# robertknight/ocrs

Hardware: AMD Instinct MI355X
Metric: pages/sec end-to-end (1024x1024) (higher is better)
Workload: dtype f32

## Files before the change

ocrs_amd/csrc/common.cpp:

```cpp
#include "common.hpp"

#include <chrono>
#include <climits>
#include <cstdint>
#include <cstdlib>
#include <cstring>

#include <algorithm>
#include <atomic>
#include <condition_variable>
#include <deque>
#include <system_error>

namespace ocrs {

static thread_local std::string g_last_error;

void set_last_error(const std::string& msg) { g_last_error = msg; }
const std::string& last_error() { return g_last_error; }

namespace {
std::atomic<int> g_default_device{0};
thread_local DeviceContext* t_ctx = nullptr;
constexpr int kMaxDevices = 64;
// ... 240 lines not shown
            cached_ -= got;
            live_[p] = got;
            live_bytes_ += got;
            peak_live_ = std::max(peak_live_, live_bytes_);
            return p;
        }
    }
    void* p = nullptr;
    OCRS_HIP(hipHostMalloc(&p, sz, hipHostMallocPortable));
    std::lock_guard<std::mutex> g(mu_);
    live_[p] = sz;
    live_bytes_ += sz;
    peak_live_ = std::max(peak_live_, live_bytes_);
    allocs_++;
    return p;
}

void HostPool::release(void* p) {
    if (!p) return;
    std::vector<void*> drop;
    {
        std::lock_guard<std::mutex> g(mu_);
        auto it = live_.find(p);
        if (it == live_.end()) return;
        free_.emplace(it->second, p);
        cached_ += it->second;
        live_bytes_ -= it->second;
        live_.erase(it);
        while (cached_ > cap_ && !free_.empty()) {
            auto big = std::prev(free_.end());
            drop.push_back(big->second);
            cached_ -= big->first;
            free_.erase(big);
        }
    }
    for (void* q : drop) trimmer().give(-1, q, &frees_);
}

void HostPool::set_cap(uint64_t bytes) {
    std::lock_guard<std::mutex> g(mu_);
    cap_ = bytes;
}

PoolStats HostPool::stats() {
    std::lock_guard<std::mutex> g(mu_);
    PoolStats st;
    st.live = live_bytes_; st.cached = cached_; st.cap = cap_; st.peak_live = peak_live_; st.driver_allocs = allocs_; st.driver_frees = frees_;
    return st;
}

hipStream_t DeviceContext::heavy_stream() {
    std::lock_guard<std::mutex> g(lazy_mu_);
    if (!heavy_) {
        DeviceScope bind(device);
        int least = 0, greatest = 0;
        OCRS_HIP(hipDeviceGetStreamPriorityRange(&least, &greatest));
        OCRS_HIP(hipStreamCreateWithPriority(&heavy_, hipStreamNonBlocking, greatest));
    }
    return heavy_;
}

hipStream_t DeviceContext::recurrent_stream(int mode) {
    if (mode == MODE_SERIAL) return heavy_stream();
    std::lock_guard<std::mutex> g(lazy_mu_);
    if (!recurrent_) {
        DeviceScope bind(device);
        int least = 0, greatest = 0;
        OCRS_HIP(hipDeviceGetStreamPriorityRange(&least, &greatest));
        OCRS_HIP(hipStreamCreateWithPriority(&recurrent_, hipStreamNonBlocking, greatest));
    }
    return recurrent_;
}

static thread_local int t_lease_depth[kMaxDevices] = {0};

template <class F> void DeviceContext::switch_isolation(F&& change) {
    if (t_lease_depth[device] > 0) fail(OCRS_ERR_INVALID_ARGUMENT, "the isolation regime of device %d cannot change from inside one of its requests", device);
    std::unique_lock<std::mutex> lk(iso_mu_);
    iso_cv_.wait(lk, [&] { return !switching_; });
    const Mode before = mode_locked();
    switching_ = true;
    struct Done { DeviceContext* c; ~Done() { c->switching_ = false; c->iso_cv_.notify_all(); } } done{this};
    const Isolation p0 = policy_;
    const int r0 = relaxed_;
    change();
    if (mode_locked() == before) return;
    const Isolation p1 = policy_;
    const int r1 = relaxed_;
    policy_ = p0; relaxed_ = r0;
    iso_cv_.wait(lk, [&] { return leases_ == 0; });
    {
        DeviceScope bind(device);
        if (hipDeviceSynchronize() != hipSuccess) (void)hipGetLastError();
    }
    policy_ = p1; relaxed_ = r1;
}

DeviceContext::Mode DeviceContext::lease_begin() {
    std::unique_lock<std::mutex> lk(iso_mu_);
    if (t_lease_depth[device] == 0) iso_cv_.wait(lk, [&] { return !switching_; });
    t_lease_depth[device]++;
    leases_++;
    return mode_locked();
}

void DeviceContext::lease_end() {
    std::lock_guard<std::mutex> lk(iso_mu_);
    t_lease_depth[device]--;
    if (--leases_ == 0) iso_cv_.notify_all();
}

void DeviceContext::add_relaxed_engine(int delta) {
    switch_isolation([&] { relaxed_ += delta; });
}

void DeviceContext::set_isolation(Isolation policy) {
    switch_isolation([&] { policy_ = policy; });
}

DeviceContext::Mode DeviceContext::current_mode() {
    std::lock_guard<std::mutex> lk(iso_mu_);
    return mode_locked();
}

int DeviceContext::relaxed_engine_count() {
    std::lock_guard<std::mutex> lk(iso_mu_);
    return relaxed_;
}

int DeviceContext::cu_count() {
    std::lock_guard<std::mutex> g(lazy_mu_);
    if (!cus_) {
        hipDeviceProp_t prop;
        OCRS_HIP(hipGetDeviceProperties(&prop, device));
        cus_ = prop.multiProcessorCount;
    }
    return cus_;
}

namespace {
struct OptDef { const char* name; const char* env; long def; };
const OptDef kOptDefs[OPT_COUNT] = {
    {"gru_mode", "OCRS_GRU_MODE", GRU_PERSISTENT},
    {"gru_gates", "OCRS_GRU_GATES", 1},
    {"gru_local", "OCRS_GRU_LOCAL", 1},
    {"det_fuse", "OCRS_DET_FUSE", 1},
    {"det_stream", "OCRS_DET_STREAM", 1},
    {"det_rows", "OCRS_DET_ROWS", 1},
    {"ccl_quad", "OCRS_CCL_QUAD", 1},
    {"conv12_fuse", "OCRS_CONV12_FUSE", 1},
    {"conv_flat", "OCRS_CONV_FLAT", 1},
    {"beam_gpu", "OCRS_BEAM_GPU", 1},
    {"det_tile_batch", "OCRS_DET_TILE_BATCH", 16},
    {"numerics", nullptr, 0},
    {"coalesce", nullptr, 2},
    {"coalesce_pages", nullptr, 16},
    {"coalesce_window_us", nullptr, 300},
    {"layout_threads", nullptr, 0},
    {"rec_max_pixels", nullptr, 0},
};
struct OptRange { long lo, hi; long also[4]; };
const OptRange kOptRanges[OPT_COUNT] = {
    {0, 1, {}}, {0, 1, {}}, {0, 1, {}}, {0, 2, {}}, {0, 1, {8, 14, 32}}, {0, 1, {8, 14, 20, 32}}, {0, 1, {}}, {0, 1, {}}, {0, 1, {}}, {0, 1, {}},
    {1, 1024, {}},
    {0, 2, {}}, {0, 64, {}}, {1, 4096, {}}, {0, 10000000, {}}, {0, 4096, {}}, {0, INT64_MAX, {}},
};
bool in_range(int i, long v) {
    const OptRange& r = kOptRanges[i];
    if (v >= r.lo && v <= r.hi) return true;
    for (long a : r.also) if (a && v == a) return true;
    return false;
}
const char* const kRetired[] = {"det_heavy", "det_tail", "gru_waves", "gru_background", "gru_scatter", "gru_gates_pack", "conv_occupancy",
                                "gx_heavy", "gemm_nfast", "conv_a_lds", "gru_heavy", "heavy_priority", "det_mfma"};
std::atomic<long> g_opts[OPT_COUNT];
std::once_flag g_opts_once;
void init_options() {
    for (int i = 0; i < OPT_COUNT; i++) {
        const char* e = kOptDefs[i].env ? getenv(kOptDefs[i].env) : nullptr;
        const long v = e && *e ? strtol(e, nullptr, 10) : kOptDefs[i].def;
        g_opts[i].store(in_range(i, v) ? v : kOptDefs[i].def);
    }
}
int find_option(const char* name, int count = OPT_PUBLIC_COUNT) {
    for (int i = 0; i < count; i++)
        if (name && i != OPT_NUMERICS && strcmp(name, kOptDefs[i].name) == 0) return i;
    return -1;
}
thread_local const Tuning* t_tuning = nullptr;
}

TuningScope::TuningScope(const Tuning* t) : prev_(t_tuning) { t_tuning = t; }
TuningScope::~TuningScope() { t_tuning = prev_; }
const Tuning* current_tuning() { return t_tuning; }

long option_long(Option o) {
    if (t_tuning) return __atomic_load_n(&t_tuning->v[o], __ATOMIC_RELAXED);
    std::call_once(g_opts_once, init_options);
    return g_opts[o].load(std::memory_order_relaxed);
}
int option(Option o) { return (int)option_long(o); }

Tuning default_tuning() {
    std::call_once(g_opts_once, init_options);
    Tuning t;
    for (int i = 0; i < OPT_COUNT; i++) t.v[i] = g_opts[i].load(std::memory_order_relaxed);
    return t;
}

const char* option_name(int i) { return i >= 0 && i < OPT_PUBLIC_COUNT ? kOptDefs[i].name : nullptr; }

int set_option(const char* name, long value) {
    std::call_once(g_opts_once, init_options);
    const int i = find_option(name);
    if (i < 0) {
        for (const char* r : kRetired) if (name && strcmp(name, r) == 0) return 0;
        return 1;
    }
    if (!in_range(i, value)) return 2;
    g_opts[i].store(value);
    return 0;
}

int set_option(Tuning& t, const char* name, long value) {
    const int i = find_option(name, OPT_COUNT);
    if (i < 0) return 1;
    if (!in_range(i, value)) return 2;
    __atomic_store_n(&t.v[i], value, __ATOMIC_RELAXED);
    return 0;
}

bool get_option(const Tuning& t, const char* name, long* value) {
    const int i = name && strcmp(name, "numerics") == 0 ? (int)OPT_NUMERICS : find_option(name, OPT_COUNT);
    if (i < 0) return false;
    *value = __atomic_load_n(&t.v[i], __ATOMIC_RELAXED);
    return true;
}

StreamLease::StreamLease(bool high_priority) : ctx_(&ctx()), high_(high_priority) {
    high_ = true;
    mode_ = ctx_->lease_begin();
    try {
        if (mode_ == DeviceContext::MODE_SERIAL) {
            s_ = ctx_->heavy_stream();
            shared_ = true;
            OCRS_HIP(hipEventCreateWithFlags(&done_, hipEventBlockingSync | hipEventDisableTiming));
            return;
        }
        {
            std::lock_guard<std::mutex> g(ctx_->stream_mu);
            auto& v = ctx_->streams;
            if (!v.empty()) {
                s_ = v.back().first;
                done_ = v.back().second;
                v.pop_back();
                return;
            }
        }
        int least = 0, greatest = 0;
        OCRS_HIP(hipDeviceGetStreamPriorityRange(&least, &greatest));
        OCRS_HIP(hipStreamCreateWithPriority(&s_, hipStreamNonBlocking, greatest));
        OCRS_HIP(hipEventCreateWithFlags(&done_, hipEventBlockingSync | hipEventDisableTiming));
    } catch (...) {
        ctx_->lease_end();
        throw;
    }
}

StreamLease::~StreamLease() {
    if (shared_) {
        (void)hipEventDestroy(done_);
    } else {
        std::lock_guard<std::mutex> g(ctx_->stream_mu);
        ctx_->streams.emplace_back(s_, done_);
    }
    ctx_->lease_end();
}

std::vector<StageTimers::Pending>& StageTimers::pending() {
    static thread_local std::vector<Pending> p;
    return p;
}
std::map<int, std::vector<hipEvent_t>>& StageTimers::thread_events() {
    static thread_local std::map<int, std::vector<hipEvent_t>> f;
    return f;
}
std::vector<hipEvent_t>& StageTimers::free_events() { return thread_events()[ctx().device]; }

hipEvent_t StageTimers::get_event() {
    auto& fe = free_events();
    if (!fe.empty()) {
        hipEvent_t e = fe.back();
        fe.pop_back();
        return e;
    }
    hipEvent_t e;
    OCRS_HIP(hipEventCreate(&e));
    return e;
}

int StageTimers::begin(int stage, hipStream_t s, uint64_t n_launches) {
    if (!enabled) return -1;
    Pending p{stage, get_event(), get_event(), n_launches, false, 0.0, 0.0, 0.0};
    OCRS_HIP(hipEventRecord(p.a, s));
    pending().push_back(p);
    return (int)pending().size() - 1;
}

int StageTimers::kbegin(int cls, hipStream_t s, double flops, double bytes, double mfma_flops) {
    if (!enabled || !kernels_enabled || !((kernel_mask >> cls) & 1u)) return -1;
    if (mfma_flops < 0.0) mfma_flops = cls <= KC_GEMM_LINEAR ? flops : 0.0;
    Pending p{cls, get_event(), get_event(), 1, true, flops, bytes, mfma_flops};
    OCRS_HIP(hipEventRecord(p.a, s));
    pending().push_back(p);
    return (int)pending().size() - 1;
}

// ... 43 lines not shown
```

ocrs_amd/csrc/common.hpp:

```cpp
#pragma once
#include <atomic>
#include <hip/hip_runtime.h>

#include <cstdarg>
#include <cstdint>
#include <cstdio>
#include <cstdlib>
#include <chrono>
#include <condition_variable>
#include <cstring>
#include <map>
#include <mutex>
#include <stdexcept>
#include <string>
#include <thread>
#include <vector>

#include "../../include/ocrs_amd.h"

namespace ocrs {

struct Error : std::runtime_error {
    ocrs_status status;
    Error(ocrs_status s, const std::string& msg) : std::runtime_error(msg), status(s) {}
};

[[noreturn]] inline void fail(ocrs_status s, const char* fmt, ...) {
    char buf[512];
    va_list ap;
    va_start(ap, fmt);
    vsnprintf(buf, sizeof buf, fmt, ap);
    va_end(ap);
    throw Error(s, buf);
}

#define OCRS_HIP(expr)                                                                              \
    do {                                                                                            \
        hipError_t _e = (expr);                                                                     \
        if (_e != hipSuccess)                                                                       \
            ::ocrs::fail(OCRS_ERR_DEVICE, "HIP error %s at %s:%d (%s)", hipGetErrorString(_e), __FILE__, \
                         __LINE__, #expr);                                                          \
    } while (0)

void set_last_error(const std::string& msg);


struct PoolStats { uint64_t live = 0, cached = 0, cap = 0, peak_live = 0, driver_allocs = 0, driver_frees = 0; };
class DevicePool {
  public:
    explicit DevicePool(int device) : device_(device) {}
    ~DevicePool();
    void* alloc(size_t bytes);
    void release(void* p);
    void trim();
    void set_cap(uint64_t bytes);
    PoolStats stats();
    int device() const { return device_; }

  private:
    uint64_t cap_locked();
    const int device_;
    std::mutex mu_;
    std::multimap<size_t, void*> free_;
    std::map<void*, size_t> live_;
    uint64_t cached_ = 0, live_bytes_ = 0, peak_live_ = 0, cap_ = 0, allocs_ = 0;
    std::atomic<uint64_t> frees_{0};
};

class HostPool {
  public:
    void* alloc(size_t bytes);
    void release(void* p);
    void set_cap(uint64_t bytes);
    PoolStats stats();

  private:
    std::mutex mu_;
    std::multimap<size_t, void*> free_;
    std::map<void*, size_t> live_;
    uint64_t cached_ = 0, live_bytes_ = 0, peak_live_ = 0, cap_ = uint64_t(1) << 30, allocs_ = 0;
    std::atomic<uint64_t> frees_{0};
};

struct DeviceContext {
    const int device;
    DevicePool pool;
    HostPool host_pool;
    std::mutex heavy_phase, rec_phase;
    hipStream_t heavy_stream();
    hipStream_t recurrent_stream(int mode = 0);
    enum Isolation { ISO_AUTO = 0, ISO_NONE = 1 };
    enum Mode { MODE_FREE = 0, MODE_SERIAL = 1 };
    Mode lease_begin();
    void lease_end();
    void add_relaxed_engine(int delta);
    void set_isolation(Isolation policy);
    Mode current_mode();
    int relaxed_engine_count();
    int cu_count();
    std::vector<struct DevBuf> heavy_arena;
    std::mutex stream_mu;
    std::vector<std::pair<hipStream_t, hipEvent_t>> streams;

    explicit DeviceContext(int d) : device(d), pool(d) {}

  private:
    Mode mode_locked() const { return policy_ == ISO_NONE || relaxed_ <= 0 ? MODE_FREE : MODE_SERIAL; }
    template <class F> void switch_isolation(F&& change);
    std::mutex lazy_mu_;
    hipStream_t heavy_ = nullptr, recurrent_ = nullptr;
    int cus_ = 0;
    std::mutex iso_mu_;
    std::condition_variable iso_cv_;
    int leases_ = 0, relaxed_ = 0;
    bool switching_ = false;
    Isolation policy_ = ISO_AUTO;
    friend class StreamLease;
};

DeviceContext& device_context(int device);
int default_device();
void select_device(int device);
DeviceContext& ctx();

class DeviceScope {
  public:
    explicit DeviceScope(int device);
    ~DeviceScope();
    DeviceScope(const DeviceScope&) = delete;
    DeviceScope& operator=(const DeviceScope&) = delete;

  private:
    DeviceContext* prev_;
    int restore_ = -1;
};

inline DevicePool& pool() { return ctx().pool; }
inline HostPool& host_pool() { return ctx().host_pool; }
inline hipStream_t heavy_stream() { return ctx().heavy_stream(); }

enum Option { OPT_GRU_MODE = 0, OPT_GRU_GATES, OPT_GRU_LOCAL, OPT_DET_FUSE, OPT_DET_STREAM, OPT_DET_ROWS, OPT_CCL_QUAD,
              OPT_CONV12_FUSE, OPT_CONV_FLAT, OPT_BEAM_GPU, OPT_DET_TILE_BATCH, OPT_PUBLIC_COUNT,
              OPT_NUMERICS = OPT_PUBLIC_COUNT,
              OPT_COALESCE, OPT_COALESCE_PAGES, OPT_COALESCE_WINDOW_US,
              OPT_LAYOUT_THREADS, OPT_REC_MAX_PIXELS,
              OPT_COUNT };
struct Tuning { long v[OPT_COUNT]; };
Tuning default_tuning();
int set_option(const char* name, long value);
int set_option(Tuning& t, const char* name, long value);
bool get_option(const Tuning& t, const char* name, long* value);
const char* option_name(int i);
class TuningScope {
  public:
    explicit TuningScope(const Tuning* t);
    ~TuningScope();
    TuningScope(const TuningScope&) = delete;
    TuningScope& operator=(const TuningScope&) = delete;
  private:
    const Tuning* prev_;
};
const Tuning* current_tuning();
enum { GRU_PERSISTENT = 0, GRU_STEP = 1 };
int option(Option o);

inline void allow_dynamic_lds(const void* kernel, std::atomic<uint64_t>& done) {
    int dev = 0;
    (void)hipGetDevice(&dev);
    const uint64_t bit = 1ull << (dev & 63);
    if (done.load(std::memory_order_relaxed) & bit) return;
    (void)hipFuncSetAttribute(kernel, hipFuncAttributeMaxDynamicSharedMemorySize, 160 * 1024);
    done.fetch_or(bit, std::memory_order_relaxed);
}
long option_long(Option o);
inline int gru_mode() { return option(OPT_GRU_MODE); }

struct DevBuf {
    void* p = nullptr;
    size_t bytes = 0;
    DevicePool* owner = nullptr;
    DevBuf() = default;
    explicit DevBuf(size_t n) : bytes(n), owner(n ? &pool() : nullptr) { p = n ? owner->alloc(n) : nullptr; }
    DevBuf(const DevBuf&) = delete;
    DevBuf& operator=(const DevBuf&) = delete;
    DevBuf(DevBuf&& o) noexcept : p(o.p), bytes(o.bytes), owner(o.owner) { o.p = nullptr; o.bytes = 0; o.owner = nullptr; }
    DevBuf& operator=(DevBuf&& o) noexcept {
        if (this != &o) { reset(); p = o.p; bytes = o.bytes; owner = o.owner; o.p = nullptr; o.bytes = 0; o.owner = nullptr; }
        return *this;
    }
    ~DevBuf() { reset(); }
    void reset() { if (p && owner) owner->release(p); p = nullptr; bytes = 0; owner = nullptr; }
    int device() const { return owner ? owner->device() : -1; }
    template <class T> T* as() const { return static_cast<T*>(p); }
};

struct PinnedBuf {
    void* p = nullptr;
    size_t bytes = 0;
    PinnedBuf() = default;
    explicit PinnedBuf(size_t n) : bytes(n) { if (n) OCRS_HIP(hipHostMalloc(&p, n, hipHostMallocPortable)); }
    PinnedBuf(const PinnedBuf&) = delete;
    PinnedBuf& operator=(const PinnedBuf&) = delete;
    ~PinnedBuf() { if (p) (void)hipHostFree(p); }
    template <class T> T* as() const { return static_cast<T*>(p); }
};

class StreamLease {
  public:
    explicit StreamLease(bool high_priority = false);
    ~StreamLease();
    hipStream_t get() const { return s_; }
    hipError_t wait_done() const noexcept {
        hipError_t e = hipEventRecord(done_, s_);
        if (e != hipSuccess) return e;
        for (int i = 0;; i++) {
            e = hipEventQuery(done_);
            if (e != hipErrorNotReady) return e;
            if (i < 64) std::this_thread::yield();
            else std::this_thread::sleep_for(std::chrono::microseconds(i < 256 ? 20 : 100));
        }
    }
    void sync() const { OCRS_HIP(wait_done()); }
    hipError_t sync_noexcept() const noexcept { return wait_done(); }
    DeviceContext::Mode mode() const { return mode_; }
    bool serial() const { return mode_ == DeviceContext::MODE_SERIAL; }
    hipStream_t conv_stream() const { return ctx_->heavy_stream(); }
    hipStream_t recurrent_stream() const { return ctx_->recurrent_stream((int)mode_); }

  private:
    DeviceContext* ctx_;
    DeviceContext::Mode mode_ = DeviceContext::MODE_FREE;
    bool shared_ = false;
    hipStream_t s_;
    hipEvent_t done_;
    bool high_;
};

enum Stage {
    ST_PREPARE = 0,
    ST_RESIZE_IN,
    ST_DET_CNN,
    ST_RESIZE_THRESH,
    ST_CCL,
    ST_CONTOUR_RECTS,
    ST_LINE_CROP,
    ST_REC_CONV,
    ST_REC_GRU,
    ST_REC_HEAD,
    ST_CTC,
    ST_COUNT
};
extern const char* const kStageNames[ST_COUNT];

enum KernelClass {
    KC_GEMM_CONV3X3 = 0, KC_GEMM_POINTWISE, KC_GEMM_CONVT, KC_GEMM_GRU_INPUT, KC_GEMM_GRU_HIDDEN, KC_GEMM_LINEAR,
    KC_DWCONV3X3, KC_CONV_DIRECT, KC_POOL, KC_PADCAT, KC_CONV1X1_SIGMOID, KC_GRU_GATES, KC_LOGSOFTMAX_ARGMAX,
    KC_OTHER, KC_DET_BLOCK, KC_DET_STREAM_WAVE, KC_DET_STREAM_ROWS, KC_COUNT
};
extern const char* const kKernelClassNames[KC_COUNT];

struct StageTimers {
    bool enabled = false;
    bool kernels_enabled = false;
    uint32_t kernel_mask = 0xffffffffu;
    std::mutex mu;
    double ms[ST_COUNT] = {0};
    uint64_t launches[ST_COUNT] = {0};
    double kms[KC_COUNT] = {0};
    uint64_t klaunches[KC_COUNT] = {0};
    double kflops[KC_COUNT] = {0};
    double kbytes[KC_COUNT] = {0};
    double kmfma[KC_COUNT] = {0};
    struct Pending { int stage; hipEvent_t a, b; uint64_t n; bool kernel; double flops, bytes, mfma; };
    static std::vector<Pending>& pending();
    int begin(int stage, hipStream_t s, uint64_t n_launches);
    int kbegin(int cls, hipStream_t s, double flops, double bytes, double mfma_flops = -1.0);
    void end(int token, hipStream_t s);
    void collect();
    void reset();
    static void release_thread_events();
  private:
    static std::vector<hipEvent_t>& free_events();
    static std::map<int, std::vector<hipEvent_t>>& thread_events();
    hipEvent_t get_event();
};

inline int ceil_div(int64_t a, int64_t b) { return (int)((a + b - 1) / b); }

struct StageScope {
    StageTimers* t; int token; hipStream_t s;
    StageScope(StageTimers* timers, int stage, hipStream_t stream, uint64_t n_launches = 1)
        : t(timers), token(timers ? timers->begin(stage, stream, n_launches) : -1), s(stream) {}
    ~StageScope() { if (t && token >= 0) t->end(token, s); }
};

struct Workspace {
    StreamLease stream;
    HostPool& hpool = host_pool();
    std::vector<DevBuf> bufs;
    std::vector<hipEvent_t> events;
    hipEvent_t make_event() {
        hipEvent_t e;
        OCRS_HIP(hipEventCreateWithFlags(&e, hipEventDisableTiming));
        events.push_back(e);
        return e;
    }
    Workspace() = default;
    explicit Workspace(bool high_priority) : stream(high_priority) {}
    std::vector<void*> upload_staging;
    void upload(void* d_dst, const void* h_src, size_t bytes) {
        if (!bytes) return;
        void* pin = hpool.alloc(bytes);
        memcpy(pin, h_src, bytes);
        upload_staging.push_back(pin);
        OCRS_HIP(hipMemcpyAsync(d_dst, pin, bytes, hipMemcpyHostToDevice, stream.get()));
    }
// ... 41 lines not shown
```

ocrs_amd/csrc/kernels.hpp:

```cpp
#pragma once
#include <vector>
#include <hip/hip_runtime.h>

#include <cstdint>

namespace ocrs {
namespace jpeg { struct Coefficients; }
namespace k {

void prepare_image(const void* d_pixels, bool is_u8, bool chans_last, int h, int w, int chans, float* d_out,
                   hipStream_t s);
void resize_pages_to_model(const float* const* d_src_ptrs, int n, int sh, int sw, int vh, int vw, float* d_dst,
                           int dh, int dw, hipStream_t s);
bool resize_threshold(const float* d_prob, int n, int mh, int mw, int sh, int sw, float thr, uint8_t* d_mask,
                      float* d_map, int h, int w, hipStream_t s, int32_t* d_labels = nullptr, int32_t* d_zero_a = nullptr,
                      int32_t* d_zero_b = nullptr);
void threshold_only(const float* d_prob, float thr, uint8_t* d_mask, int64_t count, hipStream_t s);

struct CclBuffers {
    int32_t* labels;
    int32_t* row_counts;
    int32_t* row_offsets;
    int32_t* n_roots;
    int32_t* roots;
    int32_t* lengths;
    int32_t* offsets;
    int32_t* overflow;
    uint32_t* pts;
    uint32_t* tmp;
    uint8_t* keep;
    float* rects;
    uint8_t* valid;
    uint32_t* score_pixels;
    unsigned long long* score_sums;
};
void ccl_label(const uint8_t* d_mask, int n, int h, int w, const CclBuffers& b, int max_comp, hipStream_t s, bool prepared = false);
void contour_rects(const uint8_t* d_mask, int n, int h, int w, const CclBuffers& b, int max_comp, int64_t arena,
                   float expand, float min_area, float eps, hipStream_t s, bool prepared = false);

void component_scores(const uint8_t* d_mask, const float* d_map, int n, int h, int w, const CclBuffers& b, int max_comp,
                      hipStream_t s);

struct TileDesc {
    const float* page;
    uint8_t* mask;
    float* map;
    int32_t h, w;
    int32_t oy, ox;
    int32_t y0, y1, x0, x1;
};
void gather_tiles(const TileDesc* d_tiles, int n_tiles, float* d_dst, int mh, int mw, hipStream_t s);
void stitch_threshold(const TileDesc* d_tiles, int n_tiles, const float* d_prob, int mh, int mw, float thr, hipStream_t s);

struct GemmDesc {
    const float* A; int lda;
    const float* B; int ldb;
    const float* bias;
    float* C; int ldc;
    int M, N, K;
    int relu;
    int im2col; int H, W, Cin;
    int convt; int Cout;
    int batch; int64_t strideA, strideB, strideBias, strideC;
    int nfast = 0, nx = 0, ny = 0;
    const uint16_t* Bsplit = nullptr; int64_t strideBsplit = 0;
};
void gemm(const GemmDesc& d, hipStream_t s);
void conv_direct(const float* x, int n, int h, int w, int cin, const float* wt, const float* bias, int kh, int kw,
                 int cout, int relu, float* y, hipStream_t s);
void dwconv3x3(const float* x, int n, int h, int w, int c, const float* wt, const float* bias, int relu, float* y,
               hipStream_t s);
bool dwpw_fused_supported(int cin, int cout);
void dwpw_fused(const float* x, int n, int h, int w, int cin, const float* wdw, const float* bdw, int relu_dw, int cout,
                const float* wpw, const float* bpw, int relu_pw, float* y, hipStream_t s);
bool dwconv3x3_cat(const float* skip, int n, int h, int w, int cs, const float* up, int uh, int uw, int cu, const float* wt,
                   const float* bias, int relu, float* y, hipStream_t s);
struct DoubleConvArgs {
    const float* skip;
    const float* x1;
    const float *wt, *bt;
    const float *wd1, *bd1;
    const float *wp1, *bp1;
    const float *wd2, *bd2;
    const float *wp2, *bp2;
    const float *wf, *bf;
    float* y;
    float* ypool;
    int n, h, w, h1, w1;
    int relu_d1, relu_p1, relu_d2, relu_p2, sigmoid;
    int tiles_x, tiles_y;
    const float* tape = nullptr;
    int tape_len = 0;
    const float* rtape = nullptr;
    int rtape_len = 0;
};
struct StreamWeights {
    const float *wt, *bt, *wd1, *bd1, *wp1, *bp1, *wd2, *bd2, *wp2, *bp2, *wf, *bf;
};
bool double_conv_fused(const DoubleConvArgs& a, int cs, int cx, int cmid, int cout, bool pool, bool final_conv,
                       bool launch, hipStream_t s, bool* on_mfma = nullptr, int* path = nullptr);
bool double_conv_stream(const DoubleConvArgs& a, int cs, int cx, int cmid, int cout, bool pool, bool final_conv, bool launch, hipStream_t s,
                        const StreamWeights* hw = nullptr, std::vector<float>* tape_out = nullptr, int* tape_len = nullptr);
bool double_conv_rows(const DoubleConvArgs& a, int cs, int cx, int cmid, int cout, bool pool, bool final_conv, bool launch, hipStream_t s,
                      const StreamWeights* hw = nullptr, std::vector<float>* tape_out = nullptr, int* tape_len = nullptr);
bool double_conv_rows_takes(const DoubleConvArgs& a, int cx);
void maxpool(const float* x, int n, int h, int w, int c, int kh, int kw, float* y, hipStream_t s);
void avgpool(const float* x, int n, int h, int w, int c, int kh, int kw, float* y, hipStream_t s);
void padcat(const float* skip, int n, int sh, int sw, int cs, const float* x, int h, int w, int cx, float* y,
            hipStream_t s);
void sigmoid(const float* x, float* y, int64_t count, hipStream_t s);
void conv1x1_cout1(const float* x, int64_t pixels, int cin, const float* wt, const float* bias, int relu, int do_sigmoid,
                   float* y, hipStream_t s);
void to_seq(const float* x, int n, int w, int c, float* y, hipStream_t s);
void gru_gates(const float* gx, const float* gh, float* h, float* y, int T, int N, int H, int step, hipStream_t s);
bool log_softmax_argmax(const float* logits, int64_t rows, int c, const uint8_t* d_excluded ,
                        float* logp, int32_t* labels, hipStream_t s, float* maxlp = nullptr);
void to_seq_packed(const float* x, int n, int T, int c, const int32_t* d_pos, const int32_t* d_off, float* y,
                   hipStream_t s);
void gru_gates_packed(const float* gx, const float* gh, float* h, float* y, const int32_t* d_Tm, const int32_t* d_off,
                      int64_t R, int Mcap, int active, int H, int step, hipStream_t s);
bool gru_step_fused(const float* gx, const float* wh, const float* bh, const float* hT_in, float* hT_out, float* y,
                    const int32_t* d_Tm, const int32_t* d_off, int64_t R, int Mcap, int active, int H, int step,
                    hipStream_t s);
size_t gru_persistent_sync_words(int M);
size_t gru_persistent_exchange_bytes(const int32_t* h_Tm, int M, int H);
bool gru_persistent_supported(const int32_t* h_Tm, int M, int Tmax, int64_t R, int H);
bool gru_tile_plan(const int32_t* h_Tm, int M, int H, int* ncl, int* waves, int16_t* tiles );
hipError_t gru_persistent_prepare(float* hx, const int32_t* h_Tm, int M, int H, hipStream_t s);
bool gru_persistent(const float* gx, const float* wh, const float* bh, float* y, float* hx, const int32_t* d_Tm, const int32_t* d_off,
                    const int32_t* h_Tm, int64_t R, int M, int Tmax, int H, uint32_t* d_sync, hipStream_t s);
bool gru_general_tile_plan(const int32_t* h_Tm, int M, int Tmax, int H, int cap, int* ncl, int16_t* tiles , int kernel );
size_t gru_split_exchange_bytes(const int32_t* h_Tm, int M, int H, int np);
bool gru_split_supported(const int32_t* h_Tm, int M, int Tmax, int64_t R, int H, int np);
hipError_t gru_split_prepare(uint16_t* hx, const int32_t* h_Tm, int M, int H, int np, hipStream_t s);
bool gru_persistent_split(const float* gx, const float* wh, const float* bh, float* y, uint16_t* hx, const int32_t* d_Tm, const int32_t* d_off,
                          const int32_t* h_Tm, int64_t R, int M, int Tmax, int H, int np, uint32_t* d_sync, hipStream_t s);
void ctc_collapse_packed(const int32_t* labels, const int32_t* d_Tm, const int32_t* d_off, int M, int Tmax,
                         uint32_t* out_labels, uint32_t* out_pos, int32_t* out_count, hipStream_t s);
void ctc_collapse_scored_packed(const int32_t* labels, const float* maxlp, const int32_t* d_Tm, const int32_t* d_off, int M,
                                int Tmax, uint32_t* out_labels, uint32_t* out_pos, float* out_logp, int32_t* out_count,
                                double* out_score, hipStream_t s);
void argmax_rows(const float* x, int64_t rows, int c, const uint8_t* d_excluded, int32_t* labels, hipStream_t s);
bool ctc_beam_supported(int C, int width);
size_t ctc_beam_arena_entries(int Tmax, int width);
bool ctc_beam_packed(const float* logp, const int32_t* d_Tm, const int32_t* d_off, int M, int Tmax, int C, int width,
                     const uint8_t* d_excluded, int2* d_nodes, int2* d_posn, uint32_t* out_labels, uint32_t* out_pos,
                     int32_t* out_count, hipStream_t s, double* out_score = nullptr, float* out_logp = nullptr);
void ctc_collapse(const int32_t* labels, int T, int N, uint32_t* out_labels, uint32_t* out_pos, int32_t* out_count,
                  hipStream_t s);

struct RaggedView {
    int G;
    int H;
    const int32_t* W;
    const int32_t* n;
    const int64_t* poff;
    const int32_t* toff128;
    const int32_t* toff256;
    const int32_t* loff;
    int ntiles128, ntiles256;
    const int32_t* toff2d;
    int ntiles2d, tw;
    const int32_t* toff2d_flat;
    const int32_t* toff2d_flat2;
    int ntiles2d_flat, ntiles2d_flat2;
    const int32_t* toff2d_gap;
    int ntiles2d_gap;
    int64_t max_tile_px_;
    int min_w;
    int64_t pixels;
    int max_w;
};
void conv1_relu_pool_ragged(const float* x, const RaggedView& in, const float* wt, const float* bias, int cout,
                            float* y, const RaggedView& out, hipStream_t s);
void pool_ragged(const float* x, const RaggedView& in, int c, int kh, int kw, bool avg, float* y, const RaggedView& out,
                 hipStream_t s);
void to_seq_packed_ragged(const float* x, const RaggedView& in, int c, const int32_t* d_pos, const int32_t* d_off,
                          float* y, hipStream_t s);
void avgpool_to_seq_ragged(const float* x, const RaggedView& in, const RaggedView& seq, int c, const int32_t* d_pos,
                           const int32_t* d_off, float* y, hipStream_t s);
bool conv12_fused_ragged(const float* x, const RaggedView& in0, const RaggedView& mid, const float* w1, const float* b1,
                         int c1, const float* w2, const float* b2, int c2, float* y, const RaggedView& out, hipStream_t s,
                         const uint16_t* w2split = nullptr);
void conv12_split_weights(const float* w2_host , std::vector<uint16_t>* out);
bool conv3x3_ragged(const float* x, const RaggedView& rv, int cin, const float* wt, const float* bias, int cout, int relu,
                    int ph, int pw, float* y, const RaggedView& out, hipStream_t s, const uint16_t* wsplit = nullptr);
void split_weights(const float* w_host, int K, int N, int ldw, std::vector<uint16_t>* out);

struct LineDesc {
    int32_t page;
    int32_t poly_off;
    int32_t poly_n;
    int32_t top, left, bh, bw;
    int32_t resized_w;
    int32_t out_w;
    int64_t out_off;
};
void crop_lines(const float* const* d_pages, const int32_t* d_page_hw , const LineDesc* d_lines,
                const int32_t* d_poly , int n_lines, int out_h, float* d_out, hipStream_t s);

struct RectLineDesc {
    int32_t page;
    int32_t mode;
    int32_t range_off;
    int32_t range_n;
    int32_t resized_w;
    int32_t out_w;
    int64_t out_off;
    float x0, ax, bx, y0, ay, by;
};
void rectify_lines(const float* const* d_pages, const int32_t* d_page_hw , const RectLineDesc* d_lines,
                   const int32_t* d_ranges, int n_lines, int max_out_w, int out_h, float* d_out, hipStream_t s);

void measure_peaks(double* mfma_tflops, double* copy_gbps);


size_t jpeg_sample_bytes(const jpeg::Coefficients& c);
void jpeg_decode(const jpeg::Coefficients& c, const uint64_t* d_mask, const uint32_t* d_offset, const int16_t* d_values,
                 const uint16_t* d_quant, uint8_t* d_samples, uint8_t* d_rgb, hipStream_t s);

}
}
```

ocrs_amd/csrc/kernels_lines.hip:

```cpp
#include "kernels.hpp"

namespace ocrs {
namespace k {

constexpr int MAX_LDS_EDGES = 512;

__device__ __forceinline__ void resize_axis(int o, int in_len, int out_len, int& i0, int& i1, float& wgt) {
    float scale = (float)in_len / (float)out_len;
    float c = ((float)o + 0.5f) * scale - 0.5f;
    float hi = (float)(in_len - 1);
    c = c < 0.0f ? 0.0f : c;
    c = c > hi ? hi : c;
    int a = (int)c;
    i0 = a;
    i1 = a + 1 < in_len ? a + 1 : in_len - 1;
    wgt = c - (float)a;
}

__device__ __forceinline__ int edge_x_at(int xa, int ya, int xb, int yb, int y) {
    float t = (float)(y - ya) * ((float)(xb - xa) / (float)(yb - ya));
    return xa + (int)roundf(t);
}

__global__ void __launch_bounds__(256)
crop_lines_kernel(const float* const* __restrict__ pages, const int32_t* __restrict__ page_hw,
                  const LineDesc* __restrict__ lines, const int32_t* __restrict__ poly, int out_h,
                  float* __restrict__ batch) {
    __shared__ int xs[2][MAX_LDS_EDGES];
    __shared__ int cnt[2];
    const LineDesc ln = lines[blockIdx.y];
    const int oy = blockIdx.x;
    const int out_w = ln.out_w;
    float* __restrict__ dst = batch + ln.out_off + (int64_t)oy * out_w;
    const float fill = -0.5f;
    if (ln.bh <= 0 || ln.bw <= 0) {
        for (int ox = threadIdx.x; ox < out_w; ox += blockDim.x) dst[ox] = fill;
        return;
    }
    const float* __restrict__ page = pages[ln.page];
    const int ph = page_hw[2 * ln.page], pw = page_hw[2 * ln.page + 1];
    int r0, r1;
    float wy;
    resize_axis(oy, ln.bh, out_h, r0, r1, wy);
    if (threadIdx.x < 2) cnt[threadIdx.x] = 0;
    __syncthreads();
    const int32_t* pv = poly + 2 * (int64_t)ln.poly_off;
    for (int i = threadIdx.x; i < 2 * ln.poly_n; i += blockDim.x) {
        const int which = i / ln.poly_n, e = i - which * ln.poly_n;
        const int y = ln.top + (which ? r1 : r0);
        int ya = pv[2 * e], xa = pv[2 * e + 1];
        const int e2 = e + 1 == ln.poly_n ? 0 : e + 1;
        int yb = pv[2 * e2], xb = pv[2 * e2 + 1];
        if (ya == yb) continue;
        if (ya > yb) { int t = ya; ya = yb; yb = t; t = xa; xa = xb; xb = t; }
        if (y < ya || y >= yb) continue;
        int slot = atomicAdd(&cnt[which], 1);
        if (slot < MAX_LDS_EDGES) xs[which][slot] = edge_x_at(xa, ya, xb, yb, y);
    }
    __syncthreads();
    const int m0 = cnt[0], m1 = cnt[1];
    auto crossings_direct = [&](int which, int x) {
        const int y = ln.top + (which ? r1 : r0);
        int c = 0;
        for (int e = 0; e < ln.poly_n; e++) {
            int ya = pv[2 * e], xa = pv[2 * e + 1];
            const int e2 = e + 1 == ln.poly_n ? 0 : e + 1;
            int yb = pv[2 * e2], xb = pv[2 * e2 + 1];
            if (ya == yb) continue;
            if (ya > yb) { int t = ya; ya = yb; yb = t; t = xa; xa = xb; xb = t; }
            if (y < ya || y >= yb) continue;
            c += edge_x_at(xa, ya, xb, yb, y) <= x ? 1 : 0;
        }
        return c;
    };
    for (int ox = threadIdx.x; ox < out_w; ox += blockDim.x) {
        float v = fill;
        if (ox < ln.resized_w) {
            int c0, c1;
            float wx;
            resize_axis(ox, ln.bw, ln.resized_w, c0, c1, wx);
            float tap[4];
#pragma unroll
            for (int q = 0; q < 4; q++) {
                const int which = q >> 1;
                const int r = which ? r1 : r0;
                const int c = (q & 1) ? c1 : c0;
                const int y = ln.top + r, x = ln.left + c;
                const int m = which ? m1 : m0;
                int crossings = 0;
                if (m <= MAX_LDS_EDGES)
                    for (int kk = 0; kk < m; kk++) crossings += xs[which][kk] <= x ? 1 : 0;
                else
                    crossings = crossings_direct(which, x);
                float t = fill;
                if ((crossings & 1) && y >= 0 && y <= ph - 1 && x >= 0 && x <= pw - 1 && r <= ph - 1 && c <= pw - 1)
                    t = page[(int64_t)y * pw + x];
                tap[q] = t;
            }
            float top = (1.0f - wx) * tap[0] + wx * tap[1];
            float bot = (1.0f - wx) * tap[2] + wx * tap[3];
            v = (1.0f - wy) * top + wy * bot;
        }
        dst[ox] = v;
    }
}

void crop_lines(const float* const* d_pages, const int32_t* d_page_hw, const LineDesc* d_lines, const int32_t* d_poly,
                int n_lines, int out_h, float* d_out, hipStream_t s) {
    if (n_lines <= 0) return;
    hipLaunchKernelGGL(crop_lines_kernel, dim3(out_h, n_lines), dim3(256), 0, s, d_pages, d_page_hw, d_lines, d_poly,
                       out_h, d_out);
}

}
}
```

ocrs_amd/csrc/kernels_nn.hip:

```cpp
#include "common.hpp"
#include "kernels.hpp"
#include "split_mfma.hpp"
#include "spec_math.hpp"

namespace ocrs {
namespace k {

typedef float f32x16 __attribute__((ext_vector_type(16)));

constexpr int GEMM_BK = 32;

template <int NT, bool IM2COL, bool CONVT>
__global__ void __launch_bounds__(256) gemm_mfma_kernel(GemmDesc d) {
    extern __shared__ __attribute__((aligned(16))) float lds_b[];
    constexpr int BN = 32 * NT;
    const int tid = threadIdx.x;
    const int lane = tid & 63;
    const int wave = tid >> 6;
    const int half = lane >> 5;
    const int l31 = lane & 31;
    const int z = blockIdx.z;
    const float* __restrict__ A = d.A + (int64_t)z * d.strideA;
    const float* __restrict__ B = d.B + (int64_t)z * d.strideB;
    const float* __restrict__ bias = d.bias ? d.bias + (int64_t)z * d.strideBias : nullptr;
    float* __restrict__ C = d.C + (int64_t)z * d.strideC;

    const int n0 = blockIdx.y * BN;
    const int64_t row = (int64_t)blockIdx.x * 128 + wave * 32 + l31;
    const bool row_ok = row < d.M;
    const int64_t rowc = row_ok ? row : (int64_t)d.M - 1;

    int py = 0, px = 0;
    int64_t img_base = 0;
    if (IM2COL) {
        int64_t hw = (int64_t)d.H * d.W;
        int64_t img = rowc / hw;
        int rem = (int)(rowc - img * hw);
        py = rem / d.W;
        px = rem - py * d.W;
        img_base = img * hw * d.Cin;
    }

    f32x16 acc[NT];
#pragma unroll
    for (int t = 0; t < NT; t++) {
        int col = n0 + t * 32 + l31;
        float bv = (bias && col < d.N) ? bias[col] : 0.0f;
#pragma unroll
        for (int r = 0; r < 16; r++) acc[t][r] = bv;
    }

    for (int k0 = 0; k0 < d.K; k0 += GEMM_BK) {
        const int kc = min(GEMM_BK, d.K - k0);
        __syncthreads();
        for (int i = tid; i < GEMM_BK * BN / 4; i += 256) {
            int kk = (i * 4) / BN;
            int nn = (i * 4) % BN;
            float4 v = make_float4(0.f, 0.f, 0.f, 0.f);
            if (kk < kc) {
                const float* src = B + (int64_t)(k0 + kk) * d.ldb + n0 + nn;
                if (n0 + nn + 3 < d.N && ((d.ldb & 3) == 0) && (((uintptr_t)B & 15) == 0)) {
                    v = *reinterpret_cast<const float4*>(src);
                } else {
                    if (n0 + nn + 0 < d.N) v.x = src[0];
                    if (n0 + nn + 1 < d.N) v.y = src[1];
                    if (n0 + nn + 2 < d.N) v.z = src[2];
                    if (n0 + nn + 3 < d.N) v.w = src[3];
                }
            }
            *reinterpret_cast<float4*>(&lds_b[kk * BN + nn]) = v;
        }
        __syncthreads();

        const float* arow;
        bool a_ok = true;
        if (IM2COL) {
            int tap = k0 / d.Cin;
            int ci0 = k0 - tap * d.Cin;
            int ky = tap / 3, kx = tap - ky * 3;
            int iy = py + ky - 1, ix = px + kx - 1;
            a_ok = (unsigned)iy < (unsigned)d.H && (unsigned)ix < (unsigned)d.W;
            arow = A + img_base + ((int64_t)(a_ok ? iy : 0) * d.W + (a_ok ? ix : 0)) * d.Cin + ci0;
        } else {
            arow = A + rowc * d.lda + k0;
        }

        for (int kk = 0; kk < kc; kk += 4) {
            float4 av = make_float4(0.f, 0.f, 0.f, 0.f);
            if (a_ok) {
                if (kk + 4 <= kc) {
                    av = *reinterpret_cast<const float4*>(arow + kk);
                } else {
                    av.x = arow[kk];
                    if (kk + 1 < kc) av.y = arow[kk + 1];
                    if (kk + 2 < kc) av.z = arow[kk + 2];
                }
            }
            const float a0 = half ? av.y : av.x;
            const float a1 = half ? av.w : av.z;
            const float* b0p = &lds_b[(kk + half) * BN + l31];
            const float* b1p = &lds_b[(kk + 2 + half) * BN + l31];
#pragma unroll
            for (int t = 0; t < NT; t++)
                acc[t] = __builtin_amdgcn_mfma_f32_32x32x2f32(a0, b0p[t * 32], acc[t], 0, 0, 0);
#pragma unroll
            for (int t = 0; t < NT; t++)
                acc[t] = __builtin_amdgcn_mfma_f32_32x32x2f32(a1, b1p[t * 32], acc[t], 0, 0, 0);
        }
    }

    const int64_t row_base = (int64_t)blockIdx.x * 128 + wave * 32;
#pragma unroll
    for (int t = 0; t < NT; t++) {
        const int col = n0 + t * 32 + l31;
        if (col >= d.N) continue;
#pragma unroll
        for (int r = 0; r < 16; r++) {
            const int64_t rr = row_base + (r & 3) + 8 * (r >> 2) + 4 * half;
            if (rr >= d.M) continue;
            float v = acc[t][r];
            if (d.relu) v = v > 0.0f ? v : 0.0f;
            if (CONVT) {
                int64_t hw = (int64_t)d.H * d.W;
                int64_t img = rr / hw;
                int rem = (int)(rr - img * hw);
                int y = rem / d.W, x = rem - y * d.W;
                int q = col / d.Cout, co = col - q * d.Cout;
                int dy = q >> 1, dx = q & 1;
                C[((img * 2 * d.H + 2 * y + dy) * (2 * (int64_t)d.W) + 2 * x + dx) * d.Cout + co] = v;
            } else {
                C[rr * d.ldc + col] = v;
            }
        }
    }
}

constexpr int TG_BM = 128, TG_BK = 16, TG_LDA = TG_BM + 1;

typedef float f32x4v __attribute__((ext_vector_type(4)));

template <int NTW, class Acc>
__device__ __forceinline__ void store_tile_rows(const Acc (&acc)[2][NTW], float* stage, int lane, bool relu, float* __restrict__ C,
                                                int64_t row0, int64_t M, int ldc) {
    constexpr int WN = 32 * NTW, LPR = WN / 4, RPI = 64 / LPR;
    const int half = lane >> 5, l31 = lane & 31;
    const int srow = lane / LPR, sc4 = (lane % LPR) * 4;
#pragma unroll
    for (int i = 0; i < 2; i++) {
#pragma unroll
        for (int t = 0; t < NTW; t++)
#pragma unroll
            for (int r = 0; r < 16; r++) {
                float v = acc[i][t][r];
                if (relu) v = v > 0.0f ? v : 0.0f;
                stage[((r & 3) + 8 * (r >> 2) + 4 * half) * WN + t * 32 + l31] = v;
            }
        asm volatile("s_waitcnt lgkmcnt(0)" ::: "memory");
#pragma unroll
        for (int it = 0; it < 32 / RPI; it++) {
            const int row = it * RPI + srow;
            const f32x4v v = *reinterpret_cast<const f32x4v*>(&stage[row * WN + sc4]);
            const int64_t rr = row0 + i * 32 + row;
            if (rr < M) *reinterpret_cast<f32x4v*>(&C[rr * ldc + sc4]) = v;
        }
        asm volatile("s_waitcnt lgkmcnt(0)" ::: "memory");
    }
}

template <int BN, bool IM2COL, bool PAIR>
__global__ void __launch_bounds__(256, 4) gemm_tiled_kernel(GemmDesc d) {
    extern __shared__ __attribute__((aligned(16))) float lds[];
    constexpr int NTW = BN / 64;
    float* As = lds;
    float* Bs = lds + 2 * TG_BK * TG_LDA;
    const int tid = threadIdx.x, lane = tid & 63, wave = tid >> 6;
    const int half = lane >> 5, l31 = lane & 31;
    const int wm = wave >> 1, wn = wave & 1;
    const int z = blockIdx.z;
    const float* __restrict__ A = d.A + (int64_t)z * d.strideA;
    const float* __restrict__ B = d.B + (int64_t)z * d.strideB;
    const float* __restrict__ bias = d.bias ? d.bias + (int64_t)z * d.strideBias : nullptr;
    float* __restrict__ C = d.C + (int64_t)z * d.strideC;
    int mblk, nblk;
    if (d.nfast) {
        const int xcd = blockIdx.x & 7, q = blockIdx.x >> 3;
        nblk = q % d.ny;
        mblk = (q / d.ny) * 8 + xcd;
        if (mblk >= d.nx) return;
    } else {
        const int nwg = gridDim.x, xcd = blockIdx.x & 7, xq = nwg >> 3, xr = nwg & 7;
        mblk = (xcd < xr ? xcd * (xq + 1) : xr * (xq + 1) + (xcd - xr) * xq) + (blockIdx.x >> 3);
        nblk = blockIdx.y;
    }
    const int64_t m0 = (int64_t)mblk * TG_BM;
    const int n0 = nblk * BN;

    constexpr int AQ = TG_BK / 4, AROWS = 256 / AQ, AV = TG_BM / AROWS;
    const int ar = tid / AQ, akq = tid % AQ;
    const float* arow_ptr[AV];
    int apy[AV], apx[AV];
#pragma unroll
    for (int j = 0; j < AV; j++) {
        int64_t row = m0 + ar + AROWS * j;
        if (row >= d.M) row = d.M - 1;
        if (IM2COL) {
            const int64_t hw = (int64_t)d.H * d.W;
            const int64_t img = row / hw;
            const int rem = (int)(row - img * hw);
            apy[j] = rem / d.W;
            apx[j] = rem - apy[j] * d.W;
            arow_ptr[j] = A + img * hw * d.Cin;
        } else {
            apy[j] = apx[j] = 0;
            arow_ptr[j] = A + row * d.lda;
        }
    }
    constexpr int BV = TG_BK * BN / 4 / 256;
    const bool b_vec = ((d.ldb & 3) == 0) && (((uintptr_t)B & 15) == 0);

    int boff[BV];
#pragma unroll
    for (int j = 0; j < BV; j++) {
        const int idx = tid + 256 * j;
        const int kk = idx / (BN / 4), nn = (idx % (BN / 4)) * 4;
        boff[j] = kk * d.ldb + min(n0 + nn, d.N - 4);
    }
    f32x4v pa[AV], pa2[AV], pb[BV];
    auto prefetch_b_fast = [&](int k0) {
        const float* __restrict__ bk = B + (int64_t)k0 * d.ldb;
#pragma unroll
        for (int j = 0; j < BV; j++) pb[j] = *reinterpret_cast<const f32x4v*>(bk + boff[j]);
    };
    auto prefetch_a_pair = [&](int k0) {
#pragma unroll
        for (int j = 0; j < AV; j++) {
            const float* src = arow_ptr[j] + k0 + akq * 4;
            pa[j] = *reinterpret_cast<const f32x4v*>(src);
            pa2[j] = *reinterpret_cast<const f32x4v*>(src + TG_BK);
        }
    };
    auto prefetch = [&](int k0) {
        if (IM2COL) {
            const int tap = k0 / d.Cin;
            const int ci0 = k0 - tap * d.Cin;
            const int ky = tap / 3, kx = tap - ky * 3;
#pragma unroll
            for (int j = 0; j < AV; j++) {
                const int iy = apy[j] + ky - 1, ix = apx[j] + kx - 1;
                const bool ok = (unsigned)iy < (unsigned)d.H && (unsigned)ix < (unsigned)d.W;
                pa[j] = ok ? *reinterpret_cast<const f32x4v*>(arow_ptr[j] + ((int64_t)iy * d.W + ix) * d.Cin + ci0 + akq * 4)
                           : f32x4v{0.f, 0.f, 0.f, 0.f};
            }
        } else {
#pragma unroll
            for (int j = 0; j < AV; j++) pa[j] = *reinterpret_cast<const f32x4v*>(arow_ptr[j] + k0 + akq * 4);
        }
#pragma unroll
        for (int j = 0; j < BV; j++) {
            const int idx = tid + 256 * j;
            const int kk = idx / (BN / 4), nn = (idx % (BN / 4)) * 4;
            const float* src = B + (int64_t)(k0 + kk) * d.ldb + n0 + nn;
            f32x4v v = {0.f, 0.f, 0.f, 0.f};
            if (b_vec && n0 + nn + 3 < d.N) {
                v = *reinterpret_cast<const f32x4v*>(src);
            } else {
                if (n0 + nn + 0 < d.N) v.x = src[0];
                if (n0 + nn + 1 < d.N) v.y = src[1];
                if (n0 + nn + 2 < d.N) v.z = src[2];
                if (n0 + nn + 3 < d.N) v.w = src[3];
            }
            pb[j] = v;
        }
    };
    auto commit_from = [&](int buf, const f32x4v (&src)[AV]) {
        float* a = As + buf * TG_BK * TG_LDA;
#pragma unroll
        for (int j = 0; j < AV; j++) {
            const int r = ar + AROWS * j;
            a[(akq * 4 + 0) * TG_LDA + r] = src[j].x;
            a[(akq * 4 + 1) * TG_LDA + r] = src[j].y;
            a[(akq * 4 + 2) * TG_LDA + r] = src[j].z;
            a[(akq * 4 + 3) * TG_LDA + r] = src[j].w;
        }
        float* b = Bs + buf * TG_BK * BN;
#pragma unroll
        for (int j = 0; j < BV; j++) {
            const int idx = tid + 256 * j;
            const int kk = idx / (BN / 4), nn = (idx % (BN / 4)) * 4;
            *reinterpret_cast<f32x4v*>(&b[kk * BN + nn]) = pb[j];
        }
    };
    auto commit = [&](int buf) { commit_from(buf, pa); };

    f32x16 acc[2][NTW];
#pragma unroll
    for (int t = 0; t < NTW; t++) {
        const int col = n0 + wn * (BN / 2) + t * 32 + l31;
        const float bv = (bias && col < d.N) ? bias[col] : 0.0f;
#pragma unroll
        for (int r = 0; r < 16; r++) { acc[0][t][r] = bv; acc[1][t][r] = bv; }
    }

    const int nchunks = d.K / TG_BK;
    auto compute = [&](int buf) {
        const float* a = As + buf * TG_BK * TG_LDA + wm * 64 + l31;
        const float* b = Bs + buf * TG_BK * BN + wn * (BN / 2) + l31;
#pragma unroll
        for (int kp = 0; kp < TG_BK / 2; kp++) {
            const int kr = 2 * kp + half;
            const float a0 = a[kr * TG_LDA], a1 = a[kr * TG_LDA + 32];
#pragma unroll
            for (int t = 0; t < NTW; t++) {
                const float bt = b[kr * BN + t * 32];
                acc[0][t] = __builtin_amdgcn_mfma_f32_32x32x2f32(a0, bt, acc[0][t], 0, 0, 0);
                acc[1][t] = __builtin_amdgcn_mfma_f32_32x32x2f32(a1, bt, acc[1][t], 0, 0, 0);
            }
        }
    };
    if (PAIR) {
        prefetch_a_pair(0);
        prefetch_b_fast(0);
        commit_from(0, pa);
        __syncthreads();
        for (int c = 0; c < nchunks; c += 2) {
            prefetch_b_fast((c + 1) * TG_BK);
            compute(0);
            commit_from(1, pa2);
            __syncthreads();
            const bool more = c + 2 < nchunks;
            if (more) {
                prefetch_a_pair((c + 2) * TG_BK);
                prefetch_b_fast((c + 2) * TG_BK);
            }
            compute(1);
            if (more) commit_from(0, pa);
            __syncthreads();
        }
    } else {
        prefetch(0);
        commit(0);
        __syncthreads();
        for (int c = 0; c < nchunks; c++) {
            const int buf = c & 1;
            if (c + 1 < nchunks) prefetch((c + 1) * TG_BK);
            compute(buf);
            if (c + 1 < nchunks) commit(buf ^ 1);
            __syncthreads();
        }
    }

    if (n0 + BN <= d.N && (d.ldc & 3) == 0 && (((uintptr_t)C) & 15) == 0) {
        static_assert(4 * 32 * (BN / 2) <= 2 * TG_BK * TG_LDA + 2 * TG_BK * BN, "staging must fit the operand tiles");
        store_tile_rows<NTW>(acc, lds + wave * (32 * (BN / 2)), lane, d.relu != 0, C + n0 + wn * (BN / 2), m0 + wm * 64, d.M, d.ldc);
        return;
    }
#pragma unroll
    for (int i = 0; i < 2; i++)
#pragma unroll
        for (int t = 0; t < NTW; t++) {
            const int col = n0 + wn * (BN / 2) + t * 32 + l31;
            if (col >= d.N) continue;
#pragma unroll
            for (int r = 0; r < 16; r++) {
                const int64_t rr = m0 + wm * 64 + i * 32 + (r & 3) + 8 * (r >> 2) + 4 * half;
                if (rr >= d.M) continue;
                float v = acc[i][t][r];
                if (d.relu) v = v > 0.0f ? v : 0.0f;
                C[rr * d.ldc + col] = v;
            }
        }
}

template <int BN>
static void launch_gemm_tiled(const GemmDesc& d, hipStream_t s) {
    dim3 grid((unsigned)((d.M + TG_BM - 1) / TG_BM), (unsigned)((d.N + BN - 1) / BN), (unsigned)(d.batch > 0 ? d.batch : 1));
    size_t lds = (size_t)(2 * TG_BK * TG_LDA + 2 * TG_BK * BN) * sizeof(float);
    const bool pair = !d.im2col && (d.K % (2 * TG_BK)) == 0 && (d.ldb & 3) == 0 && (((uintptr_t)d.B) & 15) == 0 &&
                      (d.strideB & 3) == 0 && (d.N & 3) == 0 && d.N >= 4;
    if (d.im2col) hipLaunchKernelGGL((gemm_tiled_kernel<BN, true, false>), grid, dim3(256), lds, s, d);
    else if (pair && grid.y > 1) {
        GemmDesc e = d;
        e.nfast = 1; e.nx = (int)grid.x; e.ny = (int)grid.y;
        const dim3 g1((unsigned)((grid.x + 7) / 8 * 8 * grid.y), 1, grid.z);
        hipLaunchKernelGGL((gemm_tiled_kernel<BN, false, true>), g1, dim3(256), lds, s, e);
    } else if (pair) hipLaunchKernelGGL((gemm_tiled_kernel<BN, false, true>), grid, dim3(256), lds, s, d);
    else hipLaunchKernelGGL((gemm_tiled_kernel<BN, false, false>), grid, dim3(256), lds, s, d);
}

template <int NP>
__global__ void __launch_bounds__(256, NP == 3 ? 2 : 3) gemm_split_kernel(GemmDesc d) {
    extern __shared__ __attribute__((aligned(16))) float lds[];
    constexpr int PL = split::PLANE;
    float* As = lds;
    float* Bs = lds + 2 * NP * PL;
    const int tid = threadIdx.x, lane = tid & 63, wave = tid >> 6;
    const int half = lane >> 5, l31 = lane & 31;
    const int wm = wave >> 1, wn = wave & 1;
    const int z = blockIdx.z;
    const float* __restrict__ A = d.A + (int64_t)z * d.strideA;
    const float* __restrict__ bias = d.bias ? d.bias + (int64_t)z * d.strideBias : nullptr;
    float* __restrict__ C = d.C + (int64_t)z * d.strideC;
    const int xcd = blockIdx.x & 7, q = blockIdx.x >> 3;
    const int nblk = q % d.ny;
    const int mblk = (q / d.ny) * 8 + xcd;
    if (mblk >= d.nx) return;
    const int64_t m0 = (int64_t)mblk * split::BM;
    const int n0 = nblk * split::BN;
    const int nchunks = d.K / split::BK;
    const float* __restrict__ img = reinterpret_cast<const float*>(d.Bsplit + (int64_t)z * d.strideBsplit) +
                                    (int64_t)nblk * nchunks * split::image_floats;
    const int ar = tid >> 2, akq = tid & 3;
    const float* arow[2];
#pragma unroll
    for (int j = 0; j < 2; j++) {
        int64_t row = m0 + ar + 64 * j;
        if (row >= d.M) row = d.M - 1;
        arow[j] = A + row * d.lda + akq * 4;
    }
    split::f32x16s acc[2][2];
#pragma unroll
    for (int t = 0; t < 2; t++) {
        const int col = n0 + wn * 64 + t * 32 + l31;
        const float bv = bias ? bias[col] : 0.0f;
#pragma unroll
        for (int r = 0; r < 16; r++) { acc[0][t][r] = bv; acc[1][t][r] = bv; }
    }
    split::pipeline<NP>(nchunks,
        [&](int k0, split::f32x4s (&d0)[2], split::f32x4s (&d1)[2]) {
#pragma unroll
            for (int j = 0; j < 2; j++) {
                d0[j] = *reinterpret_cast<const split::f32x4s*>(arow[j] + k0);
                d1[j] = *reinterpret_cast<const split::f32x4s*>(arow[j] + k0 + split::BK);
            }
        },
        [&](int k0, int ring) { split::load_weights<NP>(img + (int64_t)(k0 / split::BK) * split::image_floats, Bs + ring * NP * PL, wave, lane); },
        [&](int abuf, const split::f32x4s (&v)[2]) {
            char* base = reinterpret_cast<char*>(As + abuf * NP * PL);
#pragma unroll
            for (int j = 0; j < 2; j++) split::commit4<NP>(base, ar + 64 * j, akq, v[j][0], v[j][1], v[j][2], v[j][3]);
        },
        [&](int abuf, int ring) {
            split::mma_chunk<NP>(reinterpret_cast<const char*>(As + abuf * NP * PL), reinterpret_cast<const char*>(Bs + ring * NP * PL),
                                 wm, wn, l31, half, acc);
        });
    if ((d.ldc & 3) == 0 && (((uintptr_t)C) & 15) == 0) {
        store_tile_rows<2>(acc, lds + wave * (32 * 64), lane, d.relu != 0, C + n0 + wn * 64, m0 + wm * 64, d.M, d.ldc);
        return;
    }
#pragma unroll
    for (int i = 0; i < 2; i++)
#pragma unroll
        for (int t = 0; t < 2; t++) {
            const int col = n0 + wn * 64 + t * 32 + l31;
#pragma unroll
            for (int r = 0; r < 16; r++) {
                const int64_t rr = m0 + wm * 64 + i * 32 + (r & 3) + 8 * (r >> 2) + 4 * half;
                if (rr >= d.M) continue;
                float v = acc[i][t][r];
                if (d.relu) v = v > 0.0f ? v : 0.0f;
                C[rr * d.ldc + col] = v;
            }
        }
}

static bool launch_gemm_split(const GemmDesc& d, int numerics, hipStream_t s) {
    if (!d.Bsplit || d.im2col || d.convt || (d.K % 64) != 0 || (d.N % 128) != 0 || (d.lda & 3) != 0 || (((uintptr_t)d.A) & 15) != 0 ||
        (d.strideA & 3) != 0 || d.M < 1) return false;
    GemmDesc e = d;
    e.nx = (int)((d.M + split::BM - 1) / split::BM);
    e.ny = d.N / split::BN;
    const dim3 grid((unsigned)((e.nx + 7) / 8 * 8 * e.ny), 1, (unsigned)(d.batch > 0 ? d.batch : 1));
    static std::atomic<uint64_t> ok3{0}, ok2{0};
    if (numerics == 2) {
        allow_dynamic_lds(reinterpret_cast<const void*>(&gemm_split_kernel<2>), ok2);
        hipLaunchKernelGGL((gemm_split_kernel<2>), grid, dim3(256), split::lds_bytes(2), s, e);
    } else {
        allow_dynamic_lds(reinterpret_cast<const void*>(&gemm_split_kernel<3>), ok3);
        hipLaunchKernelGGL((gemm_split_kernel<3>), grid, dim3(256), split::lds_bytes(3), s, e);
    }
    return true;
}

template <int NT>
static void launch_gemm(const GemmDesc& d, hipStream_t s) {
    dim3 grid((unsigned)((d.M + 127) / 128), (unsigned)((d.N + 32 * NT - 1) / (32 * NT)), (unsigned)(d.batch > 0 ? d.batch : 1));
    size_t lds = (size_t)GEMM_BK * 32 * NT * sizeof(float);
    if (d.im2col)
        hipLaunchKernelGGL((gemm_mfma_kernel<NT, true, false>), grid, dim3(256), lds, s, d);
    else if (d.convt)
        hipLaunchKernelGGL((gemm_mfma_kernel<NT, false, true>), grid, dim3(256), lds, s, d);
    else
        hipLaunchKernelGGL((gemm_mfma_kernel<NT, false, false>), grid, dim3(256), lds, s, d);
}

constexpr int GS_KC = 128;

template <bool CONVT>
__global__ void __launch_bounds__(256) gemm_small_kernel(GemmDesc d) {
    extern __shared__ __attribute__((aligned(16))) float lds_b[];
    const int tid = threadIdx.x, lane = tid & 63, wave = tid >> 6;
    const int half = lane >> 5, l31 = lane & 31;
    const float* __restrict__ A = d.A;
    const float* __restrict__ B = d.B;
// ... 358 lines not shown
        const int ch = (int)(i % c);
        const int64_t pix = i / c;
        const int ox = (int)(pix % ow);
        const int oy = (int)((pix / ow) % oh);
        const int64_t img = pix / ((int64_t)ow * oh);
        const float* xp = x + ((img * h + (int64_t)oy * kh) * w + (int64_t)ox * kw) * c + ch;
        float acc = AVG ? 0.0f : xp[0];
        for (int ky = 0; ky < kh; ky++)
            for (int kx = 0; kx < kw; kx++) {
                float v = xp[((int64_t)ky * w + kx) * c];
                if (AVG) acc = acc + v;
                else acc = v > acc ? v : acc;
            }
        y[i] = AVG ? acc * inv : acc;
    }
}

void maxpool(const float* x, int n, int h, int w, int c, int kh, int kw, float* y, hipStream_t s) {
    int64_t total = (int64_t)n * (h / kh) * (w / kw) * c;
    int grid = (int)((total + 255) / 256 < 16384 ? (total + 255) / 256 : 16384);
    if (grid < 1) grid = 1;
    hipLaunchKernelGGL((pool_kernel<false>), dim3(grid), dim3(256), 0, s, x, n, h, w, c, kh, kw, y);
}

void avgpool(const float* x, int n, int h, int w, int c, int kh, int kw, float* y, hipStream_t s) {
    int64_t total = (int64_t)n * (h / kh) * (w / kw) * c;
    int grid = (int)((total + 255) / 256 < 16384 ? (total + 255) / 256 : 16384);
    if (grid < 1) grid = 1;
    hipLaunchKernelGGL((pool_kernel<true>), dim3(grid), dim3(256), 0, s, x, n, h, w, c, kh, kw, y);
}

__global__ void __launch_bounds__(256)
padcat_kernel(const float* __restrict__ skip, int n, int sh, int sw, int cs, const float* __restrict__ x, int h,
              int w, int cx, float* __restrict__ y) {
    const int ct = cs + cx;
    const int py = (sh - h) / 2, px = (sw - w) / 2;
    const int64_t total = (int64_t)n * sh * sw * ct;
    for (int64_t i = (int64_t)blockIdx.x * blockDim.x + threadIdx.x; i < total; i += (int64_t)gridDim.x * blockDim.x) {
        const int ch = (int)(i % ct);
        const int64_t pix = i / ct;
        float v;
        if (ch < cs) {
            v = skip[pix * cs + ch];
        } else {
            const int ox = (int)(pix % sw);
            const int oy = (int)((pix / sw) % sh);
            const int64_t img = pix / ((int64_t)sw * sh);
            const int iy = oy - py, ix = ox - px;
            v = ((unsigned)iy < (unsigned)h && (unsigned)ix < (unsigned)w) ? x[((img * h + iy) * w + ix) * cx + (ch - cs)] : 0.0f;
        }
        y[i] = v;
    }
}

void padcat(const float* skip, int n, int sh, int sw, int cs, const float* x, int h, int w, int cx, float* y,
            hipStream_t s) {
    int64_t total = (int64_t)n * sh * sw * (cs + cx);
    int grid = (int)((total + 255) / 256 < 16384 ? (total + 255) / 256 : 16384);
    if (grid < 1) grid = 1;
    hipLaunchKernelGGL(padcat_kernel, dim3(grid), dim3(256), 0, s, skip, n, sh, sw, cs, x, h, w, cx, y);
}

__global__ void __launch_bounds__(256) sigmoid_kernel(const float* __restrict__ x, float* __restrict__ y, int64_t count) {
    for (int64_t i = (int64_t)blockIdx.x * blockDim.x + threadIdx.x; i < count; i += (int64_t)gridDim.x * blockDim.x)
        y[i] = spec_sigmoidf(x[i]);
}

void sigmoid(const float* x, float* y, int64_t count, hipStream_t s) {
    int grid = (int)((count + 255) / 256 < 16384 ? (count + 255) / 256 : 16384);
    if (grid < 1) grid = 1;
    hipLaunchKernelGGL(sigmoid_kernel, dim3(grid), dim3(256), 0, s, x, y, count);
}

__global__ void __launch_bounds__(256)
conv1x1_cout1_kernel(const float* __restrict__ x, int64_t pixels, int cin, const float* __restrict__ wt,
                     const float* __restrict__ bias, int relu, int do_sigmoid, float* __restrict__ y) {
    for (int64_t p = (int64_t)blockIdx.x * blockDim.x + threadIdx.x; p < pixels; p += (int64_t)gridDim.x * blockDim.x) {
        float acc = bias[0];
        const float* xp = x + p * cin;
        if ((cin & 3) == 0) {
            for (int c = 0; c < cin; c += 4) {
                float4 v = *reinterpret_cast<const float4*>(xp + c);
                acc = fmaf(v.x, wt[c], acc);
                acc = fmaf(v.y, wt[c + 1], acc);
                acc = fmaf(v.z, wt[c + 2], acc);
                acc = fmaf(v.w, wt[c + 3], acc);
            }
        } else {
            for (int c = 0; c < cin; c++) acc = fmaf(xp[c], wt[c], acc);
        }
        if (relu) acc = acc > 0.0f ? acc : 0.0f;
        y[p] = do_sigmoid ? spec_sigmoidf(acc) : acc;
    }
}

void conv1x1_cout1(const float* x, int64_t pixels, int cin, const float* wt, const float* bias, int relu, int do_sigmoid,
                   float* y, hipStream_t s) {
    int grid = (int)((pixels + 255) / 256 < 16384 ? (pixels + 255) / 256 : 16384);
    if (grid < 1) grid = 1;
    hipLaunchKernelGGL(conv1x1_cout1_kernel, dim3(grid), dim3(256), 0, s, x, pixels, cin, wt, bias, relu, do_sigmoid, y);
}

__global__ void __launch_bounds__(256) to_seq_kernel(const float* __restrict__ x, int n, int w, int c, float* __restrict__ y) {
    const int64_t total = (int64_t)n * w * c;
    for (int64_t i = (int64_t)blockIdx.x * blockDim.x + threadIdx.x; i < total; i += (int64_t)gridDim.x * blockDim.x) {
        const int ch = (int)(i % c);
        const int64_t r = i / c;
        const int b = (int)(r % n);
        const int t = (int)(r / n);
        y[i] = x[((int64_t)b * w + t) * c + ch];
    }
}

void to_seq(const float* x, int n, int w, int c, float* y, hipStream_t s) {
    int64_t total = (int64_t)n * w * c;
    int grid = (int)((total + 255) / 256 < 16384 ? (total + 255) / 256 : 16384);
    if (grid < 1) grid = 1;
    hipLaunchKernelGGL(to_seq_kernel, dim3(grid), dim3(256), 0, s, x, n, w, c, y);
}

__global__ void __launch_bounds__(256)
gru_gates_kernel(const float* __restrict__ gx, const float* __restrict__ gh, float* __restrict__ h,
                 float* __restrict__ y, int T, int N, int H, int step) {
    const int dir = blockIdx.y;
    const int t = dir ? T - 1 - step : step;
    const int64_t total = (int64_t)N * H;
    const float* gxp = gx + (int64_t)dir * T * N * 3 * H + (int64_t)t * N * 3 * H;
    const float* ghp = gh + (int64_t)dir * N * 3 * H;
    float* hp = h + (int64_t)dir * N * H;
    for (int64_t i = (int64_t)blockIdx.x * blockDim.x + threadIdx.x; i < total; i += (int64_t)gridDim.x * blockDim.x) {
        const int j = (int)(i % H);
        const int64_t b = i / H;
        const float* gxr = gxp + b * 3 * H;
        const float* ghr = ghp + b * 3 * H;
        float r = spec_sigmoidf(gxr[j] + ghr[j]);
        float z = spec_sigmoidf(gxr[H + j] + ghr[H + j]);
        float nn = spec_tanhf(fmaf(r, ghr[2 * H + j], gxr[2 * H + j]));
        float hprev = hp[i];
        float hn = fmaf(z, hprev - nn, nn);
        hp[i] = hn;
        y[((int64_t)t * N + b) * 2 * H + (int64_t)dir * H + j] = hn;
    }
}

void gru_gates(const float* gx, const float* gh, float* h, float* y, int T, int N, int H, int step, hipStream_t s) {
    int64_t total = (int64_t)N * H;
    int grid = (int)((total + 255) / 256 < 4096 ? (total + 255) / 256 : 4096);
    if (grid < 1) grid = 1;
    hipLaunchKernelGGL(gru_gates_kernel, dim3(grid, 2), dim3(256), 0, s, gx, gh, h, y, T, N, H, step);
}

constexpr int LSM_ROWS = 64;

__device__ __forceinline__ void log_softmax_argmax_body(const float* __restrict__ logits, int64_t rows, int c,
                                                        const uint8_t* __restrict__ excl, float* __restrict__ logp,
                                                        int32_t* __restrict__ labels, float* __restrict__ maxlp) {
    extern __shared__ float tile[];
    const int cp = (c & 1) ? c : c + 1;
    const int64_t r0 = (int64_t)blockIdx.x * LSM_ROWS;
    const int nrows = (int)min((int64_t)LSM_ROWS, rows - r0);
    for (int i = threadIdx.x; i < nrows * c; i += LSM_ROWS) {
        int rr = i / c, cc = i - rr * c;
        tile[rr * cp + cc] = logits[r0 * c + i];
    }
    __syncthreads();
    if ((int)threadIdx.x < nrows) {
        float* row = tile + threadIdx.x * cp;
        float m = row[0];
        for (int j = 1; j < c; j++) m = row[j] > m ? row[j] : m;
        float ssum = 0.0f;
        for (int j = 0; j < c; j++) ssum = ssum + spec_expf(row[j] - m);
        const float lse = m + spec_logf(ssum);
        const float ninf = -__builtin_huge_valf();
        int best = 0;
        float bv = row[0] - lse;
        row[0] = bv;
        if (excl && excl[0]) bv = ninf;
        for (int j = 1; j < c; j++) {
            float v = row[j] - lse;
            row[j] = v;
            if (excl && excl[j]) v = ninf;
            if (v > bv) { bv = v; best = j; }
        }
        if (labels) labels[r0 + threadIdx.x] = best;
        if (maxlp) maxlp[r0 + threadIdx.x] = bv;
    }
    __syncthreads();
    if (logp)
        for (int i = threadIdx.x; i < nrows * c; i += LSM_ROWS) {
            int rr = i / c, cc = i - rr * c;
            logp[r0 * c + i] = tile[rr * cp + cc];
        }
}

__global__ void __launch_bounds__(LSM_ROWS)
log_softmax_argmax_kernel(const float* __restrict__ logits, int64_t rows, int c, const uint8_t* __restrict__ excl,
                          float* __restrict__ logp, int32_t* __restrict__ labels) {
    log_softmax_argmax_body(logits, rows, c, excl, logp, labels, nullptr);
}

__global__ void __launch_bounds__(LSM_ROWS)
log_softmax_argmax_max_kernel(const float* __restrict__ logits, int64_t rows, int c, const uint8_t* __restrict__ excl,
                              float* __restrict__ logp, int32_t* __restrict__ labels, float* __restrict__ maxlp) {
    log_softmax_argmax_body(logits, rows, c, excl, logp, labels, maxlp);
}

bool log_softmax_argmax(const float* logits, int64_t rows, int c, const uint8_t* d_excluded, float* logp,
                        int32_t* labels, hipStream_t s, float* maxlp) {
    if (rows <= 0) return true;
    int cp = (c & 1) ? c : c + 1;
    size_t lds = (size_t)LSM_ROWS * cp * sizeof(float);
    if (lds > 160 * 1024) return false;
    if (lds > 64 * 1024) {
        static std::atomic<uint64_t> lds_ok{0}, lds_ok_max{0};
        if (maxlp) allow_dynamic_lds(reinterpret_cast<const void*>(&log_softmax_argmax_max_kernel), lds_ok_max);
        else allow_dynamic_lds(reinterpret_cast<const void*>(&log_softmax_argmax_kernel), lds_ok);
    }
    int grid = (int)((rows + LSM_ROWS - 1) / LSM_ROWS);
    if (maxlp)
        hipLaunchKernelGGL(log_softmax_argmax_max_kernel, dim3(grid), dim3(LSM_ROWS), lds, s, logits, rows, c, d_excluded,
                           logp, labels, maxlp);
    else
        hipLaunchKernelGGL(log_softmax_argmax_kernel, dim3(grid), dim3(LSM_ROWS), lds, s, logits, rows, c, d_excluded, logp,
                           labels);
    return true;
}

__global__ void __launch_bounds__(256)
to_seq_packed_kernel(const float* __restrict__ x, int n, int T, int c, const int32_t* __restrict__ pos,
                     const int32_t* __restrict__ off, float* __restrict__ y) {
    const int64_t total = (int64_t)n * T * c;
    for (int64_t i = (int64_t)blockIdx.x * blockDim.x + threadIdx.x; i < total; i += (int64_t)gridDim.x * blockDim.x) {
        const int ch = (int)(i % c);
        const int64_t r = i / c;
        const int t = (int)(r % T);
        const int line = (int)(r / T);
        y[((int64_t)off[t] + pos[line]) * c + ch] = x[i];
    }
}

void to_seq_packed(const float* x, int n, int T, int c, const int32_t* d_pos, const int32_t* d_off, float* y,
                   hipStream_t s) {
    int64_t total = (int64_t)n * T * c;
    if (total <= 0) return;
    int grid = (int)((total + 255) / 256 < 16384 ? (total + 255) / 256 : 16384);
    hipLaunchKernelGGL(to_seq_packed_kernel, dim3(grid), dim3(256), 0, s, x, n, T, c, d_pos, d_off, y);
}

__global__ void __launch_bounds__(256)
gru_gates_packed_kernel(const float* __restrict__ gx, const float* __restrict__ gh, float* __restrict__ h,
                        float* __restrict__ y, const int32_t* __restrict__ Tm, const int32_t* __restrict__ off,
                        int64_t R, int Mcap, int active, int H, int step) {
    const int dir = blockIdx.y;
    const int64_t total = (int64_t)active * H;
    const float* gxd = gx + (int64_t)dir * R * 3 * H;
    const float* ghd = gh + (int64_t)dir * Mcap * 3 * H;
    float* hd = h + (int64_t)dir * Mcap * H;
    for (int64_t i = (int64_t)blockIdx.x * blockDim.x + threadIdx.x; i < total; i += (int64_t)gridDim.x * blockDim.x) {
        const int j = (int)(i % H);
        const int m = (int)(i / H);
        const int t = dir ? Tm[m] - 1 - step : step;
        const int64_t row = (int64_t)off[t] + m;
        const float* gxr = gxd + row * 3 * H;
        const float* ghr = ghd + (int64_t)m * 3 * H;
        float r = spec_sigmoidf(gxr[j] + ghr[j]);
        float z = spec_sigmoidf(gxr[H + j] + ghr[H + j]);
        float nn = spec_tanhf(fmaf(r, ghr[2 * H + j], gxr[2 * H + j]));
        float hprev = hd[i];
        float hn = fmaf(z, hprev - nn, nn);
        hd[i] = hn;
        y[row * 2 * H + (int64_t)dir * H + j] = hn;
    }
}

typedef float f32x4 __attribute__((ext_vector_type(4)));

template <int H>
__global__ void __launch_bounds__(256)
gru_step_fused_kernel(const float* __restrict__ gx, const float* __restrict__ wh, const float* __restrict__ bh,
                      const float* __restrict__ hT_in, float* __restrict__ hT_out, float* __restrict__ y,
                      const int32_t* __restrict__ Tm, const int32_t* __restrict__ off, int64_t R, int Mcap, int active,
                      int step) {
    extern __shared__ __attribute__((aligned(16))) float lds_w[];
    const int dir = blockIdx.z;
    const int j0 = blockIdx.y * 16;
    const int tid = threadIdx.x;
    const int lane = tid & 63, wave = tid >> 6;
    const int row0 = blockIdx.x * 64 + wave * 16;
    const float* __restrict__ whd = wh + (int64_t)dir * H * 3 * H;
    const float* __restrict__ bhd = bh + (int64_t)dir * 3 * H;
    const float* __restrict__ hin = hT_in + (int64_t)dir * H * Mcap;
    float* __restrict__ hout = hT_out + (int64_t)dir * H * Mcap;
    const float* __restrict__ gxd = gx + (int64_t)dir * R * 3 * H;

    const int i16 = lane & 15, kq = lane >> 4;
    const bool wave_active = row0 < active;

    float areg[H / 4];
    const int arow = min(row0 + i16, Mcap - 1);
    if (wave_active) {
        const float* ap = hin + (int64_t)kq * Mcap + arow;
#pragma unroll
        for (int s4 = 0; s4 < H / 4; s4++) areg[s4] = ap[(int64_t)s4 * 4 * Mcap];
    }
    const int j = j0 + i16;
    const int mbase = row0 + kq * 4;
    float gxr_[4], gxz_[4], gxn_[4], hprev_[4];
    int64_t yrow[4];
    bool rok[4];
#pragma unroll
    for (int r = 0; r < 4; r++) {
        const int m = mbase + r;
        rok[r] = wave_active && m < active;
        gxr_[r] = gxz_[r] = gxn_[r] = hprev_[r] = 0.0f;
        yrow[r] = 0;
        if (rok[r]) {
            const int t = dir ? Tm[m] - 1 - step : step;
            const int64_t row = (int64_t)off[t] + m;
            const float* g = gxd + row * 3 * H;
            gxr_[r] = g[j];
            gxz_[r] = g[H + j];
            gxn_[r] = g[2 * H + j];
            hprev_[r] = hin[(int64_t)j * Mcap + m];
            yrow[r] = row;
        }
    }
    for (int i = tid; i < H * 12; i += 256) {
        const int k = i / 12, q = i - k * 12;
        const int g = q >> 2, c4 = (q & 3) * 4;
        const float4 v = *reinterpret_cast<const float4*>(whd + (int64_t)k * 3 * H + g * H + j0 + c4);
        *reinterpret_cast<float4*>(&lds_w[k * 48 + g * 16 + c4]) = v;
    }
    __syncthreads();
    if (!wave_active) return;

    f32x4 acc_r, acc_z, acc_n;
    {
        const float br = bhd[j0 + i16], bz = bhd[H + j0 + i16], bn = bhd[2 * H + j0 + i16];
        for (int r = 0; r < 4; r++) { acc_r[r] = br; acc_z[r] = bz; acc_n[r] = bn; }
    }
    const float* bp = &lds_w[kq * 48 + i16];
#pragma unroll
    for (int s4 = 0; s4 < H / 4; s4++) {
        const float a = areg[s4];
        const float* b = bp + s4 * 4 * 48;
        acc_r = __builtin_amdgcn_mfma_f32_16x16x4f32(a, b[0], acc_r, 0, 0, 0);
        acc_z = __builtin_amdgcn_mfma_f32_16x16x4f32(a, b[16], acc_z, 0, 0, 0);
        acc_n = __builtin_amdgcn_mfma_f32_16x16x4f32(a, b[32], acc_n, 0, 0, 0);
    }
    float hnew[4];
#pragma unroll
    for (int r = 0; r < 4; r++) {
        float hn = 0.0f;
        if (rok[r]) {
            const float rg = spec_sigmoidf(gxr_[r] + acc_r[r]);
            const float zg = spec_sigmoidf(gxz_[r] + acc_z[r]);
            const float ng = spec_tanhf(fmaf(rg, acc_n[r], gxn_[r]));
            hn = fmaf(zg, hprev_[r] - ng, ng);
            y[yrow[r] * 2 * H + (int64_t)dir * H + j] = hn;
        }
        hnew[r] = hn;
    }
    float* hp = hout + (int64_t)j * Mcap + mbase;
    if (mbase + 3 < Mcap) {
        *reinterpret_cast<float4*>(hp) = make_float4(hnew[0], hnew[1], hnew[2], hnew[3]);
    } else {
        for (int r = 0; r < 4 && mbase + r < Mcap; r++) hp[r] = hnew[r];
    }
}

bool gru_step_fused(const float* gx, const float* wh, const float* bh, const float* hT_in, float* hT_out, float* y,
                    const int32_t* d_Tm, const int32_t* d_off, int64_t R, int Mcap, int active, int H, int step,
                    hipStream_t s) {
    if (active <= 0) return true;
    dim3 grid((active + 63) / 64, H / 16, 2);
    size_t lds = (size_t)H * 48 * sizeof(float);
    if (H == 256)
        hipLaunchKernelGGL((gru_step_fused_kernel<256>), grid, dim3(256), lds, s, gx, wh, bh, hT_in, hT_out, y, d_Tm, d_off,
                           R, Mcap, active, step);
    else if (H == 128)
        hipLaunchKernelGGL((gru_step_fused_kernel<128>), grid, dim3(256), lds, s, gx, wh, bh, hT_in, hT_out, y, d_Tm, d_off,
                           R, Mcap, active, step);
    else if (H == 64)
        hipLaunchKernelGGL((gru_step_fused_kernel<64>), grid, dim3(256), lds, s, gx, wh, bh, hT_in, hT_out, y, d_Tm, d_off, R,
                           Mcap, active, step);
    else
        return false;
    return true;
}

void gru_gates_packed(const float* gx, const float* gh, float* h, float* y, const int32_t* d_Tm, const int32_t* d_off,
                      int64_t R, int Mcap, int active, int H, int step, hipStream_t s) {
    int64_t total = (int64_t)active * H;
    if (total <= 0) return;
    int grid = (int)((total + 255) / 256 < 4096 ? (total + 255) / 256 : 4096);
    hipLaunchKernelGGL(gru_gates_packed_kernel, dim3(grid, 2), dim3(256), 0, s, gx, gh, h, y, d_Tm, d_off, R, Mcap, active,
                       H, step);
}

__global__ void __launch_bounds__(64)
ctc_collapse_packed_kernel(const int32_t* __restrict__ labels, const int32_t* __restrict__ Tm,
                           const int32_t* __restrict__ off, int M, int Tmax, uint32_t* __restrict__ out_labels,
                           uint32_t* __restrict__ out_pos, int32_t* __restrict__ out_count) {
    const int m = blockIdx.x * blockDim.x + threadIdx.x;
    if (m >= M) return;
    const int T = Tm[m];
    int last = 0, cnt = 0;
    for (int t = 0; t < T; t++) {
        int l = labels[(int64_t)off[t] + m];
        if (l == last) continue;
        last = l;
        if (l > 0) {
            out_labels[(int64_t)m * Tmax + cnt] = (uint32_t)l;
            out_pos[(int64_t)m * Tmax + cnt] = (uint32_t)t;
            cnt++;
        }
    }
    out_count[m] = cnt;
}

void ctc_collapse_packed(const int32_t* labels, const int32_t* d_Tm, const int32_t* d_off, int M, int Tmax,
                         uint32_t* out_labels, uint32_t* out_pos, int32_t* out_count, hipStream_t s) {
    if (M <= 0) return;
    hipLaunchKernelGGL(ctc_collapse_packed_kernel, dim3((M + 63) / 64), dim3(64), 0, s, labels, d_Tm, d_off, M, Tmax,
                       out_labels, out_pos, out_count);
}

constexpr int CTC_U = 16;

__global__ void __launch_bounds__(64)
ctc_collapse_scored_packed_kernel(const int32_t* __restrict__ labels, const float* __restrict__ maxlp,
                                  const int32_t* __restrict__ Tm, const int32_t* __restrict__ off, int M, int Tmax,
                                  uint32_t* __restrict__ out_labels, uint32_t* __restrict__ out_pos,
                                  float* __restrict__ out_logp, int32_t* __restrict__ out_count,
                                  double* __restrict__ out_score) {
    const int m = blockIdx.x * blockDim.x + threadIdx.x;
    const int T = m < M ? Tm[m] : 0;
    int Tw = T;
#pragma unroll
    for (int d = 32; d >= 1; d >>= 1) Tw = max(Tw, __shfl_xor(Tw, d));
    int last = 0, cnt = 0;
    double s = 0.0;
    const int64_t base = (int64_t)m * Tmax;
    for (int t0 = 0; t0 < Tw; t0 += CTC_U) {
        int l[CTC_U];
        float v[CTC_U];
#pragma unroll
        for (int u = 0; u < CTC_U; u++) {
            const int t = t0 + u;
            l[u] = 0;
            v[u] = 0.0f;
            if (t < T) {
                const int64_t r = (int64_t)off[t] + m;
                l[u] = labels[r];
                v[u] = maxlp[r];
            }
        }
#pragma unroll
        for (int u = 0; u < CTC_U; u++) {
            const int t = t0 + u;
            if (t >= T) break;
            s += (double)v[u];
            if (l[u] == last) continue;
            last = l[u];
            if (l[u] > 0) {
                out_labels[base + cnt] = (uint32_t)l[u];
                out_pos[base + cnt] = (uint32_t)t;
                out_logp[base + cnt] = v[u];
                cnt++;
            }
        }
    }
    if (m < M) {
        out_count[m] = cnt;
        out_score[m] = s;
    }
}

void ctc_collapse_scored_packed(const int32_t* labels, const float* maxlp, const int32_t* d_Tm, const int32_t* d_off, int M,
                                int Tmax, uint32_t* out_labels, uint32_t* out_pos, float* out_logp, int32_t* out_count,
                                double* out_score, hipStream_t s) {
    if (M <= 0) return;
    hipLaunchKernelGGL(ctc_collapse_scored_packed_kernel, dim3((M + 63) / 64), dim3(64), 0, s, labels, maxlp, d_Tm, d_off, M,
                       Tmax, out_labels, out_pos, out_logp, out_count, out_score);
}

__global__ void __launch_bounds__(256)
argmax_rows_kernel(const float* __restrict__ x, int64_t rows, int c, const uint8_t* __restrict__ excl,
                   int32_t* __restrict__ labels) {
    for (int64_t r = (int64_t)blockIdx.x * blockDim.x + threadIdx.x; r < rows; r += (int64_t)gridDim.x * blockDim.x) {
        const float* row = x + r * c;
        const float ninf = -__builtin_huge_valf();
        int best = 0;
        float bv = (excl && excl[0]) ? ninf : row[0];
        for (int j = 1; j < c; j++) {
            float v = (excl && excl[j]) ? ninf : row[j];
            if (v > bv) { bv = v; best = j; }
        }
        labels[r] = best;
    }
}

void argmax_rows(const float* x, int64_t rows, int c, const uint8_t* d_excluded, int32_t* labels, hipStream_t s) {
    if (rows <= 0) return;
    int grid = (int)((rows + 255) / 256 < 4096 ? (rows + 255) / 256 : 4096);
    hipLaunchKernelGGL(argmax_rows_kernel, dim3(grid), dim3(256), 0, s, x, rows, c, d_excluded, labels);
}

__global__ void __launch_bounds__(64)
ctc_collapse_kernel(const int32_t* __restrict__ labels, int T, int N, uint32_t* __restrict__ out_labels,
                    uint32_t* __restrict__ out_pos, int32_t* __restrict__ out_count) {
    const int b = blockIdx.x * blockDim.x + threadIdx.x;
    if (b >= N) return;
    int last = 0, cnt = 0;
    for (int t = 0; t < T; t++) {
        int l = labels[(int64_t)t * N + b];
        if (l == last) continue;
        last = l;
        if (l > 0) {
            out_labels[(int64_t)b * T + cnt] = (uint32_t)l;
            out_pos[(int64_t)b * T + cnt] = (uint32_t)t;
            cnt++;
        }
    }
    out_count[b] = cnt;
}

void ctc_collapse(const int32_t* labels, int T, int N, uint32_t* out_labels, uint32_t* out_pos, int32_t* out_count,
                  hipStream_t s) {
    if (N <= 0) return;
    hipLaunchKernelGGL(ctc_collapse_kernel, dim3((N + 63) / 64), dim3(64), 0, s, labels, T, N, out_labels, out_pos,
                       out_count);
}

}
}
```

ocrs_amd/csrc/kernels_rec.hip:

```cpp
#include <algorithm>

#include "common.hpp"
#include "kernels.hpp"
#include "split_mfma.hpp"

namespace ocrs {
namespace k {

typedef float f32x16 __attribute__((ext_vector_type(16)));
typedef unsigned u32x4 __attribute__((ext_vector_type(4)));
typedef float f32x4 __attribute__((ext_vector_type(4)));
typedef float f32x2 __attribute__((ext_vector_type(2)));
typedef unsigned u32x2 __attribute__((ext_vector_type(2)));
typedef __bf16 bf16x8 __attribute__((ext_vector_type(8)));
typedef __bf16 bf16x2 __attribute__((ext_vector_type(2)));

__device__ __forceinline__ int xcd_remap(int b, int nwg) {
    const int xcd = b & 7, q = nwg >> 3, r = nwg & 7;
    return (xcd < r ? xcd * (q + 1) : r * (q + 1) + (xcd - r) * q) + (b >> 3);
}

__device__ __forceinline__ int find_group(const int32_t* __restrict__ toff, int G, int tile) {
    int lo = 0, hi = G;
    while (hi - lo > 1) {
// ... 43 lines not shown
        if (iy0 >= 0 && iy0 + 3 < ih && ix0 >= 0 && ix0 + 3 < iw) {
            const float* pp = xi + (int64_t)iy0 * iw + ix0;
#pragma unroll
            for (int a = 0; a < 4; a++)
#pragma unroll
                for (int b = 0; b < 4; b++) p[a][b] = pp[a * iw + b];
        } else {
#pragma unroll
            for (int a = 0; a < 4; a++)
#pragma unroll
                for (int b = 0; b < 4; b++) {
                    const int iy = iy0 + a, ix = ix0 + b;
                    p[a][b] = ((unsigned)iy < (unsigned)ih && (unsigned)ix < (unsigned)iw) ? xi[(int64_t)iy * iw + ix] : 0.0f;
                }
        }
        float m[4];
#pragma unroll
        for (int py = 0; py < 2; py++)
#pragma unroll
            for (int px = 0; px < 2; px++) {
                float acc[4];
#pragma unroll
                for (int c = 0; c < 4; c++) acc[c] = bq[c];
#pragma unroll
                for (int ky = 0; ky < 3; ky++)
#pragma unroll
                    for (int kx = 0; kx < 3; kx++) {
                        const float xv = p[py + ky][px + kx];
#pragma unroll
                        for (int c = 0; c < 4; c++) acc[c] = fmaf(xv, wq[ky * 3 + kx][c], acc[c]);
                    }
#pragma unroll
                for (int c = 0; c < 4; c++) {
                    float v = acc[c] > 0.0f ? acc[c] : 0.0f;
                    if (py == 0 && px == 0) m[c] = v;
                    else m[c] = v > m[c] ? v : m[c];
                }
            }
        *reinterpret_cast<float4*>(yg + r * cout + 4 * q) = make_float4(m[0], m[1], m[2], m[3]);
    }
}

void conv1_relu_pool_ragged(const float* x, const RaggedView& in, const float* wt, const float* bias, int cout,
                            float* y, const RaggedView& out, hipStream_t s) {
    if (out.ntiles256 <= 0) return;
    hipLaunchKernelGGL(conv1_relu_pool_ragged_kernel, dim3(out.ntiles256), dim3(256), 0, s, x, in, wt, bias, cout, y, out);
}

template <bool AVG>
__global__ void __launch_bounds__(256)
pool_ragged_kernel(const float* __restrict__ x, RaggedView in, int c, int kh, int kw, float* __restrict__ y,
                   RaggedView out) {
    const int g = find_group(out.toff256, out.G, blockIdx.x);
    const int tile = blockIdx.x - out.toff256[g];
    const int ow = out.W[g], oh = out.H, iw = in.W[g], ih = in.H;
    const int64_t rows = (int64_t)out.n[g] * oh * ow;
    const float* __restrict__ xg = x + in.poff[g] * c;
    float* __restrict__ yg = y + out.poff[g] * c;
    const int cq = c >> 2;
    const float inv = 1.0f / (float)(kh * kw);
    for (int i = threadIdx.x; i < 256 * cq; i += 256) {
        const int64_t r = (int64_t)tile * 256 + i / cq;
        if (r >= rows) break;
        const int q = i % cq;
        const int ox = (int)(r % ow);
        const int oy = (int)((r / ow) % oh);
        const int64_t img = r / ((int64_t)ow * oh);
        const float* xp = xg + ((img * ih + (int64_t)oy * kh) * iw + (int64_t)ox * kw) * c + 4 * q;
        float4 acc = AVG ? make_float4(0.f, 0.f, 0.f, 0.f) : *reinterpret_cast<const float4*>(xp);
        for (int ky = 0; ky < kh; ky++)
            for (int kx = 0; kx < kw; kx++) {
                const float4 v = *reinterpret_cast<const float4*>(xp + ((int64_t)ky * iw + kx) * c);
                if (AVG) { acc.x = acc.x + v.x; acc.y = acc.y + v.y; acc.z = acc.z + v.z; acc.w = acc.w + v.w; }
                else {
                    acc.x = v.x > acc.x ? v.x : acc.x; acc.y = v.y > acc.y ? v.y : acc.y;
                    acc.z = v.z > acc.z ? v.z : acc.z; acc.w = v.w > acc.w ? v.w : acc.w;
                }
            }
        if (AVG) { acc.x = acc.x * inv; acc.y = acc.y * inv; acc.z = acc.z * inv; acc.w = acc.w * inv; }
        *reinterpret_cast<float4*>(yg + r * c + 4 * q) = acc;
    }
}

void pool_ragged(const float* x, const RaggedView& in, int c, int kh, int kw, bool avg, float* y, const RaggedView& out,
                 hipStream_t s) {
    if (out.ntiles256 <= 0) return;
    if (avg) hipLaunchKernelGGL((pool_ragged_kernel<true>), dim3(out.ntiles256), dim3(256), 0, s, x, in, c, kh, kw, y, out);
    else hipLaunchKernelGGL((pool_ragged_kernel<false>), dim3(out.ntiles256), dim3(256), 0, s, x, in, c, kh, kw, y, out);
}

__global__ void __launch_bounds__(256)
to_seq_packed_ragged_kernel(const float* __restrict__ x, RaggedView in, int c, const int32_t* __restrict__ pos,
                            const int32_t* __restrict__ off, float* __restrict__ y) {
    const int g = find_group(in.toff256, in.G, blockIdx.x);
    const int tile = blockIdx.x - in.toff256[g];
    const int T = in.W[g];
    const int64_t rows = (int64_t)in.n[g] * T;
    const float* __restrict__ xg = x + in.poff[g] * c;
    const int32_t* __restrict__ posg = pos + in.loff[g];
    const int cq = c >> 2;
    for (int i = threadIdx.x; i < 256 * cq; i += 256) {
        const int64_t r = (int64_t)tile * 256 + i / cq;
        if (r >= rows) break;
        const int q = i % cq;
        const int t = (int)(r % T);
        const int line = (int)(r / T);
        const float4 v = *reinterpret_cast<const float4*>(xg + r * c + 4 * q);
        *reinterpret_cast<float4*>(y + ((int64_t)off[t] + posg[line]) * c + 4 * q) = v;
    }
}

__global__ void __launch_bounds__(256)
avgpool_to_seq_ragged_kernel(const float* __restrict__ x, RaggedView in, RaggedView seq, int c,
                             const int32_t* __restrict__ pos, const int32_t* __restrict__ off, float* __restrict__ y) {
    const int g = find_group(seq.toff256, seq.G, blockIdx.x);
    const int tile = blockIdx.x - seq.toff256[g];
    const int T = seq.W[g], ih = in.H;
    const int64_t rows = (int64_t)seq.n[g] * T;
    const float* __restrict__ xg = x + in.poff[g] * c;
    const int32_t* __restrict__ posg = pos + seq.loff[g];
    const int cq = c >> 2;
    const float inv = 1.0f / (float)ih;
    for (int i = threadIdx.x; i < 256 * cq; i += 256) {
        const int64_t r = (int64_t)tile * 256 + i / cq;
        if (r >= rows) break;
        const int q = i % cq;
        const int t = (int)(r % T);
        const int64_t line = r / T;
        const float* xp = xg + (line * ih * T + t) * c + 4 * q;
        float4 acc = make_float4(0.f, 0.f, 0.f, 0.f);
        for (int ky = 0; ky < ih; ky++) {
            const float4 v = *reinterpret_cast<const float4*>(xp + (int64_t)ky * T * c);
            acc.x = acc.x + v.x; acc.y = acc.y + v.y; acc.z = acc.z + v.z; acc.w = acc.w + v.w;
        }
        acc.x = acc.x * inv; acc.y = acc.y * inv; acc.z = acc.z * inv; acc.w = acc.w * inv;
        *reinterpret_cast<float4*>(y + ((int64_t)off[t] + posg[line]) * c + 4 * q) = acc;
    }
}

void avgpool_to_seq_ragged(const float* x, const RaggedView& in, const RaggedView& seq, int c, const int32_t* d_pos,
                           const int32_t* d_off, float* y, hipStream_t s) {
    if (seq.ntiles256 <= 0) return;
    hipLaunchKernelGGL(avgpool_to_seq_ragged_kernel, dim3(seq.ntiles256), dim3(256), 0, s, x, in, seq, c, d_pos, d_off, y);
}

void to_seq_packed_ragged(const float* x, const RaggedView& in, int c, const int32_t* d_pos, const int32_t* d_off,
                          float* y, hipStream_t s) {
    if (in.ntiles256 <= 0) return;
    hipLaunchKernelGGL(to_seq_packed_ragged_kernel, dim3(in.ntiles256), dim3(256), 0, s, x, in, c, d_pos, d_off, y);
}

constexpr int RG_BM = 128, RG_BK = 16, RG_LDA = RG_BM + 1;
constexpr int CONV_WAVES = 4;
template <int BN, int TW, int PH, int PW, bool FLAT, int SPLIT = 0>
__global__ void __launch_bounds__(256, SPLIT == 3 ? 2 : SPLIT == 2 ? 3 : CONV_WAVES)
conv3x3_ragged_kernel(const float* __restrict__ X, RaggedView rv, int cin, const float* __restrict__ Bw,
                      const float* __restrict__ bias, int cout, int relu, float* __restrict__ Y,
                      const int64_t* __restrict__ out_poff) {
    extern __shared__ __attribute__((aligned(16))) float lds[];
    constexpr int NTW = BN / 64;
    constexpr int TH = RG_BM / TW;
    static_assert(TW == 32 || TW == 16, "patch width");
    static_assert(!SPLIT || (BN == 128 && RG_BK == 16), "split mode: 128-column blocks, 16-deep chunks");
    constexpr int NP = SPLIT ? SPLIT : 1;
    constexpr int SP_PLANE = split::PLANE;
    float* As = lds;
    float* Bs = lds + (SPLIT ? 2 * NP * SP_PLANE : 2 * RG_BK * RG_LDA);
    const int tid = threadIdx.x, lane = tid & 63, wave = tid >> 6;
    const int half = lane >> 5, l31 = lane & 31;
    const int wm = wave >> 1, wn = wave & 1;
    const int gtile = xcd_remap(blockIdx.x, gridDim.x);
    const int32_t* __restrict__ toff = FLAT ? (PW == 2 ? rv.toff2d_flat2 : rv.toff2d_flat) : rv.toff2d;
    const int g = find_group(toff, rv.G, gtile);
    const int tile = gtile - toff[g];
    const int H = rv.H, W = rv.W[g];
    const int tiles_h = H / TH;
    const int Wp = FLAT ? (PW == 2 ? (W + 1) & ~1 : W) : W;
    const int nimg = FLAT ? rv.n[g] : 1;
    int rb, img, x0, span = 1;
    if (FLAT) {
        rb = tile % tiles_h;
        const int c0 = (tile / tiles_h) * TW;
        img = c0 / Wp;
        x0 = c0 - img * Wp;
        span = min(nimg - img, (x0 + TW - 1) / Wp + 1);
    } else {
        const int tiles_w = (W + TW - 1) / TW;
        const int cb = tile % tiles_w;
        const int t2 = tile / tiles_w;
        rb = t2 % tiles_h;
        img = t2 / tiles_h;
        x0 = cb * TW;
    }
    const int y0 = rb * TH;
    const int n0 = blockIdx.y * BN;
    const float* __restrict__ A = X + (rv.poff[g] + (int64_t)img * H * W) * cin;
    const int K = 9 * cin;

    constexpr int AQ = RG_BK / 4;
    constexpr int AROWS = 256 / AQ;
    constexpr int AV = RG_BM / AROWS;
    const int ar = tid / AQ, akq = tid % AQ;
    int aoff[AV];
    unsigned amask[AV];
#pragma unroll
    for (int j = 0; j < AV; j++) {
        const int m = ar + AROWS * j;
        const int py = y0 + m / TW;
        int px = x0 + m % TW, ir = 0;
        if (FLAT) {
#pragma unroll
            for (int q = 0; q < 3; q++) { const bool nx = px >= Wp; px -= nx ? Wp : 0; ir += nx; }
        }
        unsigned mk = 0;
        if (px < W && ir < span) {
#pragma unroll
            for (int t9 = 0; t9 < 9; t9++) {
                const int iy = py + t9 / 3 - 1, ix = px + t9 % 3 - 1;
                if ((unsigned)iy < (unsigned)H && (unsigned)ix < (unsigned)W) mk |= 1u << t9;
            }
        }
        amask[j] = mk;
        aoff[j] = ((min(ir, span - 1) * H + py) * W + min(px, W - 1)) * cin + akq * 4;
    }
    constexpr int BV = RG_BK * BN / 4 / 256;
    f32x4 pa0[AV], pa1[AV];
    const uint64_t a_addr = reinterpret_cast<uint64_t>(A);
    const float* a_uniform = reinterpret_cast<const float*>(((uint64_t)(uint32_t)__builtin_amdgcn_readfirstlane((int)(a_addr >> 32)) << 32) |
                                                            (uint32_t)__builtin_amdgcn_readfirstlane((int)a_addr));
    const __amdgpu_buffer_rsrc_t a_rsrc = __builtin_amdgcn_make_buffer_rsrc(
        const_cast<float*>(a_uniform),  0,
        __builtin_amdgcn_readfirstlane((int)((int64_t)span * H * W * cin * sizeof(float))), 0x00020000);
    constexpr int OOB = 0x40000000;
    auto load_a_into = [&](int k0, f32x4 (&d0)[AV], f32x4 (&d1)[AV]) {
        const int tap = k0 / cin;
        const int ci0 = k0 - tap * cin;
        const int ky = tap / 3, kx = tap - ky * 3;
        const int delta = ((ky - 1) * W + (kx - 1)) * cin + ci0;
#pragma unroll
        for (int j = 0; j < AV; j++) {
            const int voff = ((amask[j] >> tap) & 1u) ? (aoff[j] + delta) * 4 : OOB;
            const u32x4 v0 = __builtin_amdgcn_raw_buffer_load_b128(a_rsrc, voff, 0, 0);
            const u32x4 v1 = __builtin_amdgcn_raw_buffer_load_b128(a_rsrc, voff + RG_BK * 4, 0, 0);
            d0[j] = __builtin_bit_cast(f32x4, v0);
            d1[j] = __builtin_bit_cast(f32x4, v1);
        }
    };
    auto load_a_pair = [&](int k0) { load_a_into(k0, pa0, pa1); };
    int boff[BV];
#pragma unroll
    for (int j = 0; j < BV; j++) {
        const int idx = tid + 256 * j;
        const int kk = idx / (BN / 4), nn = (idx % (BN / 4)) * 4;
        boff[j] = kk * cout + min(n0 + nn, cout - 4);
    }
    auto load_b = [&](int k0, int buf) {
        if constexpr (SPLIT != 0) {
            split::load_weights<NP>(Bw + ((int64_t)blockIdx.y * (K / RG_BK) + k0 / RG_BK) * split::image_floats,
                                    Bs + buf * NP * SP_PLANE, wave, lane);
            return;
        }
        const float* __restrict__ bk = Bw + (int64_t)k0 * cout;
        float* bdst = Bs + buf * RG_BK * BN + wave * 256;
#pragma unroll
        for (int j = 0; j < BV; j++)
            __builtin_amdgcn_global_load_lds((const __attribute__((address_space(1))) void*)(bk + boff[j]),
                                             (__attribute__((address_space(3))) void*)(bdst + 1024 * j), 16, 0, 0);
    };
    auto commit = [&](int buf, const f32x4 (&pa)[AV]) {
        if constexpr (SPLIT != 0) {
            char* base = reinterpret_cast<char*>(As + buf * NP * SP_PLANE);
#pragma unroll
            for (int j = 0; j < AV; j++) split::commit4<NP>(base, ar + AROWS * j, akq, pa[j][0], pa[j][1], pa[j][2], pa[j][3]);
            return;
        }
        float* a = As + buf * RG_BK * RG_LDA;
#pragma unroll
        for (int j = 0; j < AV; j++) {
            const int r = ar + AROWS * j;
            a[(akq * 4 + 0) * RG_LDA + r] = pa[j].x;
            a[(akq * 4 + 1) * RG_LDA + r] = pa[j].y;
            a[(akq * 4 + 2) * RG_LDA + r] = pa[j].z;
            a[(akq * 4 + 3) * RG_LDA + r] = pa[j].w;
        }
    };

    f32x16 acc[2][NTW];
#pragma unroll
    for (int t = 0; t < NTW; t++) {
        const int col = n0 + wn * (BN / 2) + t * 32 + l31;
        const float bv = col < cout ? bias[col] : 0.0f;
#pragma unroll
        for (int r = 0; r < 16; r++) { acc[0][t][r] = bv; acc[1][t][r] = bv; }
    }
    auto compute = [&](int buf, int bbuf = -1) {
        if constexpr (SPLIT != 0) {
            split::mma_chunk<NP>(reinterpret_cast<const char*>(As + buf * NP * SP_PLANE),
                                 reinterpret_cast<const char*>(Bs + (bbuf < 0 ? buf : bbuf) * NP * SP_PLANE), wm, wn, l31, half, acc);
            return;
        }
        const float* a = As + buf * RG_BK * RG_LDA + wm * 64 + l31;
        const float* b = Bs + buf * RG_BK * BN + wn * (BN / 2) + l31;
#pragma unroll
        for (int kp = 0; kp < RG_BK / 2; kp++) {
            const int kr = 2 * kp + half;
            const float a0 = a[kr * RG_LDA], a1 = a[kr * RG_LDA + 32];
#pragma unroll
            for (int t = 0; t < NTW; t++) {
                const float bt = b[kr * BN + t * 32];
                acc[0][t] = __builtin_amdgcn_mfma_f32_32x32x2f32(a0, bt, acc[0][t], 0, 0, 0);
                acc[1][t] = __builtin_amdgcn_mfma_f32_32x32x2f32(a1, bt, acc[1][t], 0, 0, 0);
            }
        }
    };
    const int nchunks = K / RG_BK;
    if constexpr (SPLIT != 0) {
        static_assert(AV == 2, "split::pipeline counts four activation loads per chunk pair");
        split::pipeline<NP>(nchunks,
                            [&](int k0, f32x4 (&d0)[AV], f32x4 (&d1)[AV]) { load_a_into(k0, d0, d1); },
                            [&](int k0, int ring) { load_b(k0, ring); },
                            [&](int abuf, const f32x4 (&d)[AV]) { commit(abuf, d); },
                            [&](int abuf, int ring) { compute(abuf, ring); });
    } else {
    load_a_pair(0);
    load_b(0, 0);
    commit(0, pa0);
    __syncthreads();
    for (int c = 0; c < nchunks; c += 2) {
        load_b((c + 1) * RG_BK, 1);
        compute(0);
        commit(1, pa1);
        __syncthreads();
        const bool more = c + 2 < nchunks;
        if (more) {
            load_a_pair((c + 2) * RG_BK);
            load_b((c + 2) * RG_BK, 0);
        }
        compute(1);
        if (more) commit(0, pa0);
        __syncthreads();
    }
    }

    const int Ho = H / PH, Wo = W / PW;
    float* __restrict__ C = Y + (out_poff[g] + (int64_t)img * Ho * Wo) * cout;
    auto act = [&](float v) { return relu ? (v > 0.0f ? v : 0.0f) : v; };
    if (PH == 1 && PW == 1 && n0 + BN <= cout && (cout & 3) == 0 && (((uintptr_t)Y) & 15) == 0) {
        constexpr int WN = BN / 2, LPR = WN / 4, RPI = 64 / LPR, NIT = 32 / RPI;
        static_assert(SPLIT != 0 || 4 * 32 * WN <= 2 * RG_BK * RG_LDA + 2 * RG_BK * BN, "staging must fit the operand tiles");
        float* stage = lds + wave * (32 * WN);
        const int srow = lane / LPR, sc4 = (lane % LPR) * 4;
        int soff[NIT];
#pragma unroll
        for (int it = 0; it < NIT; it++) {
            const int q = it * RPI + srow;
            int x = x0 + (TW == 32 ? q : (q & 15)), ir = 0;
            if (FLAT) {
#pragma unroll
                for (int k = 0; k < 3; k++) { const bool nx = x >= Wp; x -= nx ? Wp : 0; ir += nx; }
            }
            soff[it] = (x < W && (!FLAT || ir < span)) ? ((FLAT ? ir * Ho * Wo : 0) + x) * cout + n0 + wn * WN + sc4 : -1;
        }
#pragma unroll
        for (int i = 0; i < 2; i++) {
#pragma unroll
            for (int t = 0; t < NTW; t++)
#pragma unroll
                for (int r = 0; r < 16; r++)
                    stage[((r & 3) + 8 * (r >> 2) + 4 * half) * WN + t * 32 + l31] = act(acc[i][t][r]);
            asm volatile("s_waitcnt lgkmcnt(0)" ::: "memory");
#pragma unroll
            for (int it = 0; it < NIT; it++) {
                const int q = it * RPI + srow;
                if (soff[it] < 0) continue;
                const int ty = TW == 32 ? 2 * wm + i : 4 * wm + 2 * i + (q >> 4);
                *reinterpret_cast<f32x4*>(&C[soff[it] + (y0 + ty) * Wo * cout]) = *reinterpret_cast<const f32x4*>(&stage[q * WN + sc4]);
            }
            asm volatile("s_waitcnt lgkmcnt(0)" ::: "memory");
        }
        return;
    }
    constexpr int NX = TW == 16 ? 8 : 16;
    int xo_off[FLAT ? NX : 1];
    if (FLAT) {
#pragma unroll
        for (int jx = 0; jx < NX; jx++) {
            if (PW == 2 && (jx & 1)) { xo_off[jx] = -1; continue; }
            const int q = (jx & 3) + 8 * (jx >> 2) + 4 * half;
            int x = x0 + (TW == 32 ? q : (q & 15)), ir = 0;
#pragma unroll
            for (int k = 0; k < 3; k++) { const bool nx = x >= Wp; x -= nx ? Wp : 0; ir += nx; }
            xo_off[jx] = (x + (PW - 1) < W && ir < span) ? (ir * Ho * Wo + x / PW) * cout : -1;
        }
    }
#pragma unroll
    for (int t = 0; t < NTW; t++) {
        const int col = n0 + wn * (BN / 2) + t * 32 + l31;
        if (col >= cout) continue;
#pragma unroll
        for (int i = 0; i < 2; i++) {
            if (PH == 2 && TW == 32 && i == 1) continue;
#pragma unroll
            for (int r = 0; r < 16; r++) {
                if (PH == 2 && TW == 16 && (r & 8)) continue;
                if (PW == 2 && (r & 1)) continue;
                const int q = (r & 3) + 8 * (r >> 2) + 4 * half;
                const int ty = TW == 32 ? 2 * wm + i : 4 * wm + 2 * i + (r >> 3);
                const int tx = TW == 32 ? q : (q & 15);
                const int x = x0 + tx;
                if (FLAT ? xo_off[TW == 16 ? (r & 7) : r] < 0 : x + (PW - 1) >= W) continue;
                constexpr int VI = (PH == 2 && TW == 32) ? 1 : 0;
                constexpr int VR = (PH == 2 && TW == 16) ? 8 : 0;
                float m = act(acc[i][t][r]);
                if (PW == 2) { const float v = act(acc[i][t][(r + 1) & 15]); m = v > m ? v : m; }
                if (PH == 2) {
                    { const float v = act(acc[(i + VI) & 1][t][(r + VR) & 15]); m = v > m ? v : m; }
                    if (PW == 2) { const float v = act(acc[(i + VI) & 1][t][(r + VR + 1) & 15]); m = v > m ? v : m; }
                }
                const int yo = (y0 + ty) / PH;
                if (FLAT) C[xo_off[TW == 16 ? (r & 7) : r] + yo * Wo * cout + col] = m;
                else C[((int64_t)yo * Wo + x / PW) * cout + col] = m;
            }
        }
    }
}

constexpr int F12_MID = 32, F12_COUT = 64, F12_TW = 16, F12_TH = 8, F12_HW = F12_TW + 2, F12_HH = F12_TH + 2;
constexpr int F12_NPOS = F12_HH * F12_HW;
constexpr int F12_LD = F12_MID + 1;
constexpr int F12_BK = 16;
constexpr size_t F12_LDS = (size_t)(F12_NPOS * F12_LD + 2 * F12_BK * F12_COUT) * sizeof(float);

__global__ void __launch_bounds__(256, CONV_WAVES)
conv12_fused_kernel(const float* __restrict__ X0, RaggedView in0, RaggedView mid, const float* __restrict__ w1,
                    const float* __restrict__ b1, const float* __restrict__ Bw, const float* __restrict__ bias,
                    float* __restrict__ Y, const int64_t* __restrict__ out_poff) {
    extern __shared__ __attribute__((aligned(16))) float lds[];
    constexpr int BN = F12_COUT, TW = F12_TW, TH = F12_TH, LD = F12_LD;
    float* T = lds;
    float* Bs = lds + F12_NPOS * LD;
    const int tid = threadIdx.x, lane = tid & 63, wave = tid >> 6;
    const int half = lane >> 5, l31 = lane & 31;
    const int wm = wave >> 1, wn = wave & 1;
    const int gtile = xcd_remap(blockIdx.x, gridDim.x);
    const int g = find_group(mid.toff2d_gap, mid.G, gtile);
    const int tile = gtile - mid.toff2d_gap[g];
    const int H = mid.H, W = mid.W[g];
    const int H0 = in0.H, W0 = in0.W[g];
    const int tiles_h = H / TH;
    const int Wg = (W + 2) & ~1;
    const int nimg = mid.n[g];
    const int rb = tile % tiles_h;
    const int c0 = (tile / tiles_h) * TW;
    const int img = c0 / Wg;
    const int x0 = c0 - img * Wg;
    const int span = min(nimg - img, (x0 + TW - 1) / Wg + 1);
    const int y0 = rb * TH;

    constexpr int BV = F12_BK * BN / 4 / 256;
    const int boff = (tid / (BN / 4)) * BN + (tid % (BN / 4)) * 4;
    auto load_b = [&](int k0, int buf) {
#pragma unroll
        for (int j = 0; j < BV; j++)
            __builtin_amdgcn_global_load_lds((const __attribute__((address_space(1))) void*)(Bw + (int64_t)(k0 + 16 * j) * BN + boff),
                                             (__attribute__((address_space(3))) void*)(Bs + buf * F12_BK * BN + wave * 256 + 1024 * j), 16, 0, 0);
    };
    load_b(0, 0);

    {
        const int q = tid & 7;
        f32x2 wq[9][2], bq[2];
#pragma unroll
        for (int t = 0; t < 9; t++)
#pragma unroll
            for (int c = 0; c < 2; c++) wq[t][c] = f32x2{w1[t * F12_MID + 4 * q + 2 * c], w1[t * F12_MID + 4 * q + 2 * c + 1]};
#pragma unroll
        for (int c = 0; c < 2; c++) bq[c] = f32x2{b1[4 * q + 2 * c], b1[4 * q + 2 * c + 1]};
        const float* __restrict__ xg = X0 + in0.poff[g];
        for (int p = tid >> 3; p < F12_NPOS; p += 32) {
            const int hy = p / F12_HW, hx = p - hy * F12_HW;
            const int y = y0 - 1 + hy;
            int x = x0 - 1 + hx, ir = 0;
#pragma unroll
            for (int k = 0; k < 3; k++) { const bool nx = x >= Wg; x -= nx ? Wg : 0; ir += nx; }
            f32x2 m[2] = {f32x2{0.0f, 0.0f}, f32x2{0.0f, 0.0f}};
            if ((unsigned)y < (unsigned)H && x >= 0 && x < W && ir < span) {
                const float* xi = xg + (int64_t)(img + ir) * H0 * W0;
                float pt[4][4];
                const int iy0 = 2 * y - 1, ix0 = 2 * x - 1;
                if (iy0 >= 0 && iy0 + 3 < H0 && ix0 >= 0 && ix0 + 3 < W0) {
                    const float* pp = xi + (int64_t)iy0 * W0 + ix0;
#pragma unroll
                    for (int a = 0; a < 4; a++)
#pragma unroll
                        for (int b = 0; b < 4; b++) pt[a][b] = pp[a * W0 + b];
                } else {
#pragma unroll
                    for (int a = 0; a < 4; a++)
#pragma unroll
// ... 198 lines not shown
            *reinterpret_cast<u32x2*>(T + off) = ph;
            *reinterpret_cast<u32x2*>(T + F12S_TILE + off) = pm;
            if (NP == 3) {
                u32x2 pl = {cut(r0 - lo_f(pm[0]), r1 - hi_f(pm[0])), cut(r2 - lo_f(pm[1]), r3 - hi_f(pm[1]))};
                *reinterpret_cast<u32x2*>(T + 2 * F12S_TILE + off) = pl;
            }
        }
    }

    f32x16 acc[2];
    {
        const float bv = bias[wn * 32 + l31];
#pragma unroll
        for (int r = 0; r < 16; r++) { acc[0][r] = bv; acc[1][r] = bv; }
    }
    const int mx = l31 & 15;
    int pos0[2];
#pragma unroll
    for (int i = 0; i < 2; i++) {
        const int m = wm * 64 + i * 32 + l31;
        pos0[i] = (m / TW) * F12S_RS + mx;
    }
    const int nb = wn * 32 + l31;
    const int boff = nb * 64, bsw = (nb >> 2) & 3;
    asm volatile("" ::: "memory");
    __builtin_amdgcn_s_waitcnt(0x0070);
    __builtin_amdgcn_s_barrier();
    asm volatile("" ::: "memory");
#pragma unroll
    for (int tap = 0; tap < 9; tap++) {
        if (tap + 2 < 9) load_b(tap + 2);
        const int ky = tap / 3, kx = tap % 3;
        const int asw = ((mx + kx) >> 2) & 3;
        const char* bb = Bs + (tap % 3) * NP * F12S_BTAP + boff;
#pragma unroll
        for (int s2 = 0; s2 < 2; s2++) {
            const int qa = (((2 * s2 + half) ^ asw) & 3) << 4, qb = (((2 * s2 + half) ^ bsw) & 3) << 4;
            bf16x8 af[2][3], bfr[3];
#pragma unroll
            for (int i = 0; i < 2; i++)
#pragma unroll
                for (int p = 0; p < NP; p++) af[i][p] = *reinterpret_cast<const bf16x8*>(T + p * F12S_TILE + (pos0[i] + ky * F12S_RS + kx) * 64 + qa);
#pragma unroll
            for (int p = 0; p < NP; p++) bfr[p] = *reinterpret_cast<const bf16x8*>(bb + p * F12S_BTAP + qb);
#define OCRS_TERM12(PA, PB)                                                                                   \
            OCRS_SPLIT_MMA(af[0][PA], bfr[PB], acc[0]);                                                       \
            OCRS_SPLIT_MMA(af[1][PA], bfr[PB], acc[1]);
            if (NP == 3) { OCRS_TERM12(NP - 1, 0) OCRS_TERM12(0, NP - 1) OCRS_TERM12(1, 1) }
            OCRS_TERM12(1, 0) OCRS_TERM12(0, 1) OCRS_TERM12(0, 0)
#undef OCRS_TERM12
        }
        asm volatile("" ::: "memory");
        if (tap + 2 < 9) __builtin_amdgcn_s_waitcnt(0x0070 | NP);
        else __builtin_amdgcn_s_waitcnt(0x0070);
        __builtin_amdgcn_s_barrier();
        asm volatile("" ::: "memory");
    }

    const int Ho = H / 2, Wo = W / 2;
    float* __restrict__ C = Y + (out_poff[g] + (int64_t)img * Ho * Wo) * BN;
    auto act = [&](float v) { return v > 0.0f ? v : 0.0f; };
    const int col = wn * 32 + l31;
    int xo_off[8];
#pragma unroll
    for (int jx = 0; jx < 8; jx++) {
        if (jx & 1) { xo_off[jx] = -1; continue; }
        int x = x0 + (jx & 3) + 8 * (jx >> 2) + 4 * half, ir = 0;
#pragma unroll
        for (int k = 0; k < 3; k++) { const bool nx = x >= Wg; x -= nx ? Wg : 0; ir += nx; }
        xo_off[jx] = (x + 1 < W && ir < span) ? (ir * Ho * Wo + x / 2) * BN : -1;
    }
#pragma unroll
    for (int i = 0; i < 2; i++)
#pragma unroll
        for (int r = 0; r < 8; r += 2) {
            if (xo_off[r & 7] < 0) continue;
            const float m = act(__builtin_fmaxf(__builtin_fmaxf(acc[i][r], acc[i][r + 1]), __builtin_fmaxf(acc[i][r + 8], acc[i][r + 9])));
            const int yo = (y0 + 4 * wm + 2 * i) / 2;
            C[xo_off[r & 7] + yo * Wo * BN + col] = m;
        }
}

void conv12_split_weights(const float* w, std::vector<uint16_t>* out) {
    out->assign((size_t)9 * 3 * F12_COUT * 32, 0);
    auto bits = [](float f) { uint32_t u; memcpy(&u, &f, 4); return u; };
    auto from = [](uint32_t u) { float f; memcpy(&f, &u, 4); return f; };
    auto rne = [&](float f) { const uint32_t u = bits(f); return (u + 0x7FFFu + ((u >> 16) & 1u)) >> 16; };
    for (int tap = 0; tap < 9; tap++)
        for (int n = 0; n < F12_COUT; n++)
            for (int k = 0; k < 32; k++) {
                const float x = w[(size_t)(tap * 32 + k) * F12_COUT + n];
                const uint32_t hb = rne(x);
                const float r1 = x - from(hb << 16);
                const uint32_t mb = rne(r1);
                const uint32_t lb = rne(r1 - from(mb << 16));
                const size_t e = (size_t)n * 32 + (size_t)((((k >> 3) ^ (n >> 2)) & 3) * 8) + (k & 7);
                uint16_t* img = out->data() + (size_t)tap * 3 * F12_COUT * 32;
                img[e] = (uint16_t)hb;
                img[F12_COUT * 32 + e] = (uint16_t)mb;
                img[2 * F12_COUT * 32 + e] = (uint16_t)lb;
            }
}

bool conv12_fused_ragged(const float* x, const RaggedView& in0, const RaggedView& mid, const float* w1, const float* b1,
                         int c1, const float* w2, const float* b2, int c2, float* y, const RaggedView& out, hipStream_t s,
                         const uint16_t* w2split) {
    if (option(OPT_CONV12_FUSE) == 0) return false;
    if (c1 != F12_MID || c2 != F12_COUT || mid.H % F12_TH != 0 || in0.H != 2 * mid.H || out.H * 2 != mid.H) return false;
    if (mid.min_w < 11 || mid.ntiles2d_gap <= 0) return false;
    if (mid.max_tile_px_ * 4 * (int64_t)sizeof(float) >= (int64_t)1 << 30 ||
        mid.max_tile_px_ * F12_COUT * (int64_t)sizeof(float) >= (int64_t)1 << 30) return false;
    if (!x) return true;
    const int numerics = option(OPT_NUMERICS);
    if (numerics != 0 && w2split) {
        static std::atomic<uint64_t> ok3{0}, ok2{0};
        if (numerics == 2) {
            allow_dynamic_lds(reinterpret_cast<const void*>(&conv12_fused_split_kernel<2>), ok2);
            hipLaunchKernelGGL((conv12_fused_split_kernel<2>), dim3(mid.ntiles2d_gap), dim3(256), f12s_lds(2), s, x, in0, mid, w1, b1, w2split, b2, y, out.poff);
        } else {
            allow_dynamic_lds(reinterpret_cast<const void*>(&conv12_fused_split_kernel<3>), ok3);
            hipLaunchKernelGGL((conv12_fused_split_kernel<3>), dim3(mid.ntiles2d_gap), dim3(256), f12s_lds(3), s, x, in0, mid, w1, b1, w2split, b2, y, out.poff);
        }
        return true;
    }
    hipLaunchKernelGGL(conv12_fused_kernel, dim3(mid.ntiles2d_gap), dim3(256), F12_LDS, s, x, in0, mid, w1, b1, w2, b2, y, out.poff);
    return true;
}

void split_weights(const float* w, int K, int N, int ldw, std::vector<uint16_t>* out) {
    const int nblk = N / 128, nch = K / 16;
    out->assign((size_t)nblk * nch * 3 * 128 * 16, 0);
    auto bits = [](float f) { uint32_t u; memcpy(&u, &f, 4); return u; };
    auto from = [](uint32_t u) { float f; memcpy(&f, &u, 4); return f; };
    auto rne = [&](float f) { const uint32_t u = bits(f); return (u + 0x7FFFu + ((u >> 16) & 1u)) >> 16; };
    for (int nb = 0; nb < nblk; nb++)
        for (int c = 0; c < nch; c++) {
            uint16_t* img = out->data() + ((size_t)nb * nch + c) * 3 * 128 * 16;
            for (int n = 0; n < 128; n++)
                for (int kl = 0; kl < 16; kl++) {
                    const float x = w[(size_t)(c * 16 + kl) * ldw + nb * 128 + n];
                    const uint32_t hb = rne(x);
                    const float r1 = x - from(hb << 16);
                    const uint32_t mb = rne(r1);
                    const uint32_t lb = rne(r1 - from(mb << 16));
                    const int half = kl >> 3, j = kl & 7;
                    const size_t e = (size_t)n * 16 + (size_t)(((half ^ (n >> 3)) & 1) * 8) + j;
                    img[e] = (uint16_t)hb;
                    img[128 * 16 + e] = (uint16_t)mb;
                    img[2 * 128 * 16 + e] = (uint16_t)lb;
                }
        }
}

bool conv3x3_ragged(const float* x, const RaggedView& rv, int cin, const float* wt, const float* bias, int cout, int relu,
                    int ph, int pw, float* y, const RaggedView& out, hipStream_t s, const uint16_t* wsplit) {
    if ((cin % (2 * RG_BK)) != 0 || (cout % 4) != 0 || cout < 64) return false;
    if (!((ph == 1 && pw == 1) || (ph == 2 && (pw == 1 || pw == 2)))) return false;
    if ((ph == 2 || pw == 2) && !relu) return false;
    if (rv.tw != 32 && rv.tw != 16) return false;
    if (rv.H % (RG_BM / rv.tw) != 0) return false;
    const bool flat = option(OPT_CONV_FLAT) != 0 && rv.min_w >= 11 &&
                      rv.max_tile_px_ * std::max(cin, cout) * (int64_t)sizeof(float) < (int64_t)1 << 30;
    if (!flat && (int64_t)rv.H * rv.max_w * cin * (int64_t)sizeof(float) >= (int64_t)1 << 30) return false;
    const int ntiles = flat ? (pw == 2 ? rv.ntiles2d_flat2 : rv.ntiles2d_flat) : rv.ntiles2d;
    if (ntiles <= 0) return true;
    const bool n64 = cout <= 64;
    const int numerics = option(OPT_NUMERICS);
    const bool split = wsplit && !n64 && (cout % 128) == 0 && (cin % 64) == 0 && numerics != 0;
    const size_t lds = split ? split::lds_bytes(numerics == 2 ? 2 : 3)
                             : (size_t)(2 * RG_BK * RG_LDA + 2 * RG_BK * (n64 ? 64 : 128)) * sizeof(float);
    const dim3 grid(ntiles, (cout + (n64 ? 63 : 127)) / (n64 ? 64 : 128));
#define OCRS_LAUNCH_SPLIT(TW_, PH_, PW_, FLAT_, NP_, SLOT_)                                                              \
    if (flat == FLAT_ && (numerics == 2 ? 2 : 3) == NP_) {                                                              \
        allow_dynamic_lds(reinterpret_cast<const void*>(&conv3x3_ragged_kernel<128, TW_, PH_, PW_, FLAT_, NP_>), ok_[SLOT_]);   \
        hipLaunchKernelGGL((conv3x3_ragged_kernel<128, TW_, PH_, PW_, FLAT_, NP_>), grid, dim3(256), lds, s, x, rv, cin, ws_, bias, \
                           cout, relu, y, out.poff);                                                                    \
    }
#define OCRS_LAUNCH_CONV(BN_, TW_, PH_, PW_)                                                                            \
    do {                                                                                                                \
        if (split && BN_ == 128) {                                                                                      \
            const float* ws_ = reinterpret_cast<const float*>(wsplit);                                                  \
            static std::atomic<uint64_t> ok_[4] = {};                                                                    \
            OCRS_LAUNCH_SPLIT(TW_, PH_, PW_, true, 3, 0) OCRS_LAUNCH_SPLIT(TW_, PH_, PW_, false, 3, 1)                     \
            OCRS_LAUNCH_SPLIT(TW_, PH_, PW_, true, 2, 2) OCRS_LAUNCH_SPLIT(TW_, PH_, PW_, false, 2, 3)                     \
        } else if (flat) hipLaunchKernelGGL((conv3x3_ragged_kernel<BN_, TW_, PH_, PW_, true>), grid, dim3(256), lds, s, x, rv, \
                                     cin, wt, bias, cout, relu, y, out.poff);                                           \
        else hipLaunchKernelGGL((conv3x3_ragged_kernel<BN_, TW_, PH_, PW_, false>), grid, dim3(256), lds, s, x, rv,     \
                                cin, wt, bias, cout, relu, y, out.poff);                                                \
    } while (0)
#define OCRS_DISPATCH_POOL(BN_, TW_)                              \
    do {                                                          \
        if (ph == 1) OCRS_LAUNCH_CONV(BN_, TW_, 1, 1);            \
        else if (pw == 1) OCRS_LAUNCH_CONV(BN_, TW_, 2, 1);       \
        else OCRS_LAUNCH_CONV(BN_, TW_, 2, 2);                    \
    } while (0)
    if (n64) {
        if (rv.tw == 32) OCRS_DISPATCH_POOL(64, 32); else OCRS_DISPATCH_POOL(64, 16);
    } else {
        if (rv.tw == 32) OCRS_DISPATCH_POOL(128, 32); else OCRS_DISPATCH_POOL(128, 16);
    }
#undef OCRS_DISPATCH_POOL
#undef OCRS_LAUNCH_CONV
#undef OCRS_LAUNCH_SPLIT
    return true;
}

}
}
```

ocrs_amd/csrc/model.cpp:

```cpp
#include "model.hpp"

#include <cstdio>
#include <functional>
#include <map>
#include <mutex>

#include "kernels.hpp"

namespace ocrs {

namespace {
#pragma pack(push, 1)
struct FileHeader {
    char magic[8];
    uint32_t version, kind;
    int64_t input_shape[4];
    uint32_t n_ops, n_slots, out_slot, reserved;
    uint64_t blob_floats;
};
struct FileOp {
    uint32_t type;
    int32_t in0, in1, out, relu, kh, kw, cin, cout, hidden;
    uint32_t n_w, reserved;
    struct { uint64_t off, cnt; } w[8];
// ... 37 lines not shown

    auto m = std::make_unique<HipModel>();
    m->kind = hd.kind;
    for (int i = 0; i < 4; i++) m->input_shape[i] = hd.input_shape[i];
    m->n_slots = hd.n_slots;
    m->out_slot = hd.out_slot;

    std::vector<float> slab(blob, blob + hd.blob_floats);
    auto pad16 = [&]() { while (slab.size() % 4) slab.push_back(0.f); };
    pad16();
    struct Fix { size_t op; int which; size_t off; };
    std::vector<Fix> fixes;
    std::vector<FileOp> fops(hd.n_ops);
    for (uint32_t i = 0; i < hd.n_ops; i++) {
        memcpy(&fops[i], static_cast<const char*>(data) + sizeof(FileHeader) + (size_t)i * sizeof(FileOp), sizeof(FileOp));
        const FileOp& f = fops[i];
        if (f.type >= OP_COUNT || f.n_w > 8) fail(OCRS_ERR_IO, "bad op record %u", i);
        for (uint32_t j = 0; j < f.n_w; j++)
            if (f.w[j].off > hd.blob_floats || f.w[j].cnt > hd.blob_floats - f.w[j].off)
                fail(OCRS_ERR_IO, "weight reference out of range in op %u", i);
        {
            const int64_t ns = hd.n_slots;
            const bool two_in = f.type == OP_PADCAT;
            if (f.in0 < 0 || f.in0 >= ns || f.out <= 0 || f.out >= ns || (two_in ? (f.in1 < 0 || f.in1 >= ns) : false) ||
                (!two_in && f.in1 >= ns))
                fail(OCRS_ERR_IO, "slot index out of range in op %u", i);
            auto want = [&](uint32_t j, int64_t cnt) {
                if (j >= f.n_w || cnt < 0 || (int64_t)f.w[j].cnt != cnt)
                    fail(OCRS_ERR_IO, "op %u (%s): weight tensor %u has %llu floats, the op's shape needs %lld", i,
                         kOpNames[f.type], j, j < f.n_w ? (unsigned long long)f.w[j].cnt : 0ull, (long long)cnt);
            };
            auto pos = [&](int64_t v, const char* what) {
                if (v <= 0 || v > (1 << 20)) fail(OCRS_ERR_IO, "op %u (%s): bad %s %lld", i, kOpNames[f.type], what, (long long)v);
            };
            switch (f.type) {
                case OP_CONV: pos(f.kh, "kh"); pos(f.kw, "kw"); pos(f.cin, "cin"); pos(f.cout, "cout");
                    want(0, (int64_t)f.kh * f.kw * f.cin * f.cout); want(1, f.cout); break;
                case OP_DWCONV3: pos(f.cin, "channels"); want(0, 9LL * f.cin); want(1, f.cin); break;
                case OP_MAXPOOL: case OP_AVGPOOL: pos(f.kh, "kh"); pos(f.kw, "kw"); break;
                case OP_CONVT2: pos(f.cin, "cin"); pos(f.cout, "cout"); want(0, 4LL * f.cin * f.cout); want(1, f.cout); break;
                case OP_GRU: pos(f.cin, "input size"); pos(f.hidden, "hidden size");
                    if (f.n_w != 8) fail(OCRS_ERR_IO, "GRU op %u needs 8 weight tensors", i);
                    for (uint32_t d = 0; d < 2; d++) {
                        want(4 * d + 0, 3LL * f.cin * f.hidden); want(4 * d + 1, 3LL * f.hidden);
                        want(4 * d + 2, 3LL * f.hidden * f.hidden); want(4 * d + 3, 3LL * f.hidden);
                    }
                    break;
                case OP_LINEAR: pos(f.cin, "cin"); pos(f.cout, "cout"); want(0, (int64_t)f.cin * f.cout); want(1, f.cout); break;
                default: break;
            }
        }
        GraphOp op{};
        op.type = f.type; op.in0 = f.in0; op.in1 = f.in1; op.out = f.out;
        op.relu = f.relu; op.kh = f.kh; op.kw = f.kw; op.cin = f.cin; op.cout = f.cout; op.hidden = f.hidden;
        for (uint32_t j = 0; j < f.n_w; j++) op.wcount[j] = f.w[j].cnt;
        if (f.type == OP_CONVT2) {
            const float* w = blob + f.w[0].off;
            const float* b = blob + f.w[1].off;
            fixes.push_back({i, 0, slab.size()});
            for (int ci = 0; ci < f.cin; ci++)
                for (int q = 0; q < 4; q++)
                    for (int co = 0; co < f.cout; co++) slab.push_back(w[((size_t)q * f.cin + ci) * f.cout + co]);
            pad16();
            fixes.push_back({i, 1, slab.size()});
            for (int q = 0; q < 4; q++)
                for (int co = 0; co < f.cout; co++) slab.push_back(b[co]);
            pad16();
        } else if (f.type == OP_GRU) {
            if (f.n_w != 8) fail(OCRS_ERR_IO, "GRU op %u needs 8 weight tensors", i);
            for (int part = 0; part < 4; part++) {
                fixes.push_back({i, part, slab.size()});
                for (int d = 0; d < 2; d++) {
                    const float* src = blob + f.w[4 * d + part].off;
                    slab.insert(slab.end(), src, src + f.w[4 * d + part].cnt);
                }
                pad16();
            }
        }
        m->ops.push_back(op);
    }
    {
        std::vector<int64_t> chans(hd.n_slots, -1);
        chans[0] = 1;
        for (uint32_t i = 0; i < hd.n_ops; i++) {
            const FileOp& f = fops[i];
            auto in = [&](int32_t sl) {
                if (chans[sl] < 0)
                    fail(OCRS_ERR_IO, "op %u (%s): input slot %d is not written by an earlier op", i, kOpNames[f.type], sl);
                return chans[sl];
            };
            const int64_t c0 = in(f.in0);
            auto need = [&](int64_t want, const char* what) {
                if (c0 != want)
                    fail(OCRS_ERR_IO, "op %u (%s): %s is %lld but input slot %d carries %lld channels", i, kOpNames[f.type], what,
                         (long long)want, f.in0, (long long)c0);
            };
            int64_t co = c0;
            switch (f.type) {
                case OP_CONV: case OP_CONVT2: case OP_LINEAR: need(f.cin, "cin"); co = f.cout; break;
                case OP_DWCONV3: need(f.cin, "channels"); break;
                case OP_GRU: need(f.cin, "input size"); co = 2LL * f.hidden; break;
                case OP_PADCAT: co = c0 + in(f.in1); break;
                default: break;
            }
            if (co > (1 << 24)) fail(OCRS_ERR_IO, "op %u (%s): %lld output channels", i, kOpNames[f.type], (long long)co);
            chans[f.out] = co;
        }
        if (chans[hd.out_slot] < 0) fail(OCRS_ERR_IO, "the output slot %u is not written by any op", hd.out_slot);
    }
    DeviceScope bind(device);
    m->device = ctx().device;
    m->weights = DevBuf(slab.size() * sizeof(float));
    OCRS_HIP(hipMemcpy(m->weights.p, slab.data(), slab.size() * sizeof(float), hipMemcpyHostToDevice));
    const float* base = m->weights.as<float>();
    for (uint32_t i = 0; i < hd.n_ops; i++)
        for (uint32_t j = 0; j < fops[i].n_w; j++) m->ops[i].w[j] = base + fops[i].w[j].off;
    for (const Fix& fx : fixes) {
        GraphOp& op = m->ops[fx.op];
        const float* p = base + fx.off;
        if (fx.which == 0) op.aux0 = p;
        else if (fx.which == 1) op.aux1 = p;
        else if (fx.which == 2) op.aux2 = p;
        else op.aux3 = p;
    }
    for (uint32_t i = 0; i < hd.n_ops; i++) {
        GraphOp& op = m->ops[i];
        if (m->kind == 1 && op.type == OP_CONV && op.kh == 3 && op.kw == 3 && (op.cin % 32) == 0 && (op.cout % 128) == 0) {
            std::vector<uint16_t> img;
            k::split_weights(slab.data() + fops[i].w[0].off, 9 * op.cin, op.cout, op.cout, &img);
            m->tapes.emplace_back(img.size() * sizeof(uint16_t));
            OCRS_HIP(hipMemcpy(m->tapes.back().p, img.data(), img.size() * sizeof(uint16_t), hipMemcpyHostToDevice));
            op.wsplit = m->tapes.back().as<uint16_t>();
        }
        if (m->kind == 1 && op.type == OP_CONV && op.kh == 3 && op.kw == 3 && op.cin == 32 && op.cout == 64) {
            std::vector<uint16_t> img;
            k::conv12_split_weights(slab.data() + fops[i].w[0].off, &img);
            m->tapes.emplace_back(img.size() * sizeof(uint16_t));
            OCRS_HIP(hipMemcpy(m->tapes.back().p, img.data(), img.size() * sizeof(uint16_t), hipMemcpyHostToDevice));
            op.wsplit = m->tapes.back().as<uint16_t>();
        }
    }
    for (const Fix& fx : fixes) {
        GraphOp& op = m->ops[fx.op];
        if (fx.which != 0 || op.type != OP_GRU || (op.cin % 64) != 0 || ((3 * op.hidden) % 128) != 0) continue;
        std::vector<uint16_t> both;
        for (int dir = 0; dir < 2; dir++) {
            std::vector<uint16_t> img;
            k::split_weights(slab.data() + fx.off + (size_t)dir * op.cin * 3 * op.hidden, op.cin, 3 * op.hidden, 3 * op.hidden, &img);
            both.insert(both.end(), img.begin(), img.end());
        }
        m->tapes.emplace_back(both.size() * sizeof(uint16_t));
        OCRS_HIP(hipMemcpy(m->tapes.back().p, both.data(), both.size() * sizeof(uint16_t), hipMemcpyHostToDevice));
        op.wsplit = m->tapes.back().as<uint16_t>();
    }
    for (size_t i = 0; i + 1 < m->ops.size(); i++) {
        GraphOp& a = m->ops[i];
        GraphOp& b = m->ops[i + 1];
        if (a.type == OP_CONV && a.cout == 1 && a.kh == 1 && a.kw == 1 && b.type == OP_SIGMOID && b.in0 == a.out) {
            bool other_use = false;
            for (size_t j = i + 2; j < m->ops.size(); j++)
                if (m->ops[j].in0 == a.out || m->ops[j].in1 == a.out) other_use = true;
            if (!other_use && (uint32_t)a.out != m->out_slot) b.fused_into_prev = true;
        }
    }
    for (size_t i = 0; i + 1 < m->ops.size(); i++) {
        GraphOp& a = m->ops[i];
        GraphOp& b = m->ops[i + 1];
        if (a.type == OP_DWCONV3 && b.type == OP_CONV && b.kh == 1 && b.kw == 1 && b.in0 == a.out && b.cin == a.cin &&
            k::dwpw_fused_supported(a.cin, b.cout) && (uint32_t)a.out != m->out_slot) {
            bool other_use = false;
            for (size_t j = i + 2; j < m->ops.size(); j++)
                if (m->ops[j].in0 == a.out || m->ops[j].in1 == a.out) other_use = true;
            if (!other_use) { a.fuse_next_pw = true; b.done_by_prev = true; }
        }
    }
    for (size_t i = 0; i + 1 < m->ops.size(); i++) {
        GraphOp& a = m->ops[i];
        GraphOp& b = m->ops[i + 1];
        if (a.type == OP_PADCAT && b.type == OP_DWCONV3 && b.in0 == a.out && (uint32_t)a.out != m->out_slot) {
            bool other_use = false;
            for (size_t j = i + 2; j < m->ops.size(); j++)
                if (m->ops[j].in0 == a.out || m->ops[j].in1 == a.out) other_use = true;
            if (!other_use) { a.cat_into_next = true; b.reads_cat = true; }
        }
    }
    {
        auto& ops = m->ops;
        const int n = (int)ops.size();
        auto uses = [&](int slot) {
            int u = 0;
            for (const GraphOp& o : ops) u += (o.in0 == slot) + (o.in1 == slot);
            return u + ((uint32_t)slot == m->out_slot ? 1 : 0);
        };
        auto pw11 = [](const GraphOp& o) { return o.type == OP_CONV && o.kh == 1 && o.kw == 1; };
        for (int i = 0; i + 3 < n; i++) {
            DcBlock b;
            int j = i;
            if (ops[j].type == OP_CONVT2 && j + 1 < n && ops[j + 1].type == OP_PADCAT && ops[j + 1].in1 == ops[j].out &&
                uses(ops[j].out) == 1 && uses(ops[j + 1].out) == 1) {
                b.convt = j; b.cat = j + 1;
                j += 2;
            }
            if (j + 3 >= n) continue;
            const GraphOp &d1 = ops[j], &p1 = ops[j + 1], &d2 = ops[j + 2], &p2 = ops[j + 3];
            if (d1.type != OP_DWCONV3 || !pw11(p1) || d2.type != OP_DWCONV3 || !pw11(p2)) continue;
            if (b.cat >= 0 && d1.in0 != ops[b.cat].out) continue;
            if (p1.in0 != d1.out || d2.in0 != p1.out || p2.in0 != d2.out) continue;
            if (uses(d1.out) != 1 || uses(p1.out) != 1 || uses(d2.out) != 1) continue;
            if (p1.cin != d1.cin || d2.cin != p1.cout || p2.cin != d2.cin) continue;
            b.dw1 = j; b.pw1 = j + 1; b.dw2 = j + 2; b.pw2 = j + 3;
            b.first = i; b.last = j + 3;
            b.cmid = p1.cout; b.cout = p2.cout;
            if (b.convt >= 0) {
                b.cx = ops[b.convt].cin;
                b.cs = d1.cin - ops[b.convt].cout;
                if (b.cs != ops[b.convt].cout) continue;
            } else {
                b.cs = d1.cin;
            }
            const int k = j + 4;
            if (k < n && ops[k].type == OP_MAXPOOL && ops[k].kh == 2 && ops[k].kw == 2 && ops[k].in0 == p2.out && b.convt < 0) {
                b.pool = k; b.last = k;
            } else if (k < n && pw11(ops[k]) && ops[k].cout == 1 && !ops[k].relu && ops[k].in0 == p2.out && uses(p2.out) == 1 && b.convt >= 0) {
                b.fin = k; b.last = k;
                if (k + 1 < n && ops[k + 1].type == OP_SIGMOID && ops[k + 1].fused_into_prev) { b.sig = k + 1; b.last = k + 1; }
                else if (uses(ops[k].out) == 0) continue;
            }
            k::DoubleConvArgs none{};
            if (!k::double_conv_fused(none, b.cs, b.cx, b.cmid, b.cout, b.pool >= 0, b.fin >= 0, false, nullptr)) continue;
            {
                auto host = [&](int op, int j) -> const float* { return op >= 0 ? slab.data() + fops[op].w[j].off : nullptr; };
                k::StreamWeights hw{host(b.convt, 0), host(b.convt, 1), host(b.dw1, 0), host(b.dw1, 1), host(b.pw1, 0), host(b.pw1, 1),
                                    host(b.dw2, 0), host(b.dw2, 1), host(b.pw2, 0), host(b.pw2, 1), host(b.fin, 0), host(b.fin, 1)};
                std::vector<float> tape;
                int tape_len = 0;
                if (k::double_conv_stream(none, b.cs, b.cx, b.cmid, b.cout, b.pool >= 0, b.fin >= 0, false, nullptr, &hw, &tape, &tape_len)) {
                    m->tapes.emplace_back(tape.size() * sizeof(float));
                    OCRS_HIP(hipMemcpy(m->tapes.back().p, tape.data(), tape.size() * sizeof(float), hipMemcpyHostToDevice));
                    b.tape = m->tapes.back().as<float>();
                    b.tape_len = tape_len;
                }
                if (k::double_conv_rows(none, b.cs, b.cx, b.cmid, b.cout, b.pool >= 0, b.fin >= 0, false, nullptr, &hw, &tape, &tape_len)) {
                    m->tapes.emplace_back(tape.size() * sizeof(float));
                    OCRS_HIP(hipMemcpy(m->tapes.back().p, tape.data(), tape.size() * sizeof(float), hipMemcpyHostToDevice));
                    b.rtape = m->tapes.back().as<float>();
                    b.rtape_len = tape_len;
                }
            }
            ops[i].dc_block = (int)m->dc_blocks.size();
            m->dc_blocks.push_back(b);
            i = b.last;
        }
    }
    return m;
}

TensorShape HipModel::infer(int n, int h, int w, std::vector<TensorShape>* slots_out) const {
    std::vector<TensorShape> s(n_slots);
    s[0] = TensorShape{n, h, w, 1, false};
    for (const GraphOp& op : ops) {
        const TensorShape a = s[op.in0];
        TensorShape o = a;
        switch (op.type) {
            case OP_CONV: o.c = op.cout; break;
            case OP_DWCONV3: break;
            case OP_MAXPOOL:
            case OP_AVGPOOL: o.h = a.h / op.kh; o.w = a.w / op.kw; break;
            case OP_CONVT2: o.h = 2 * a.h; o.w = 2 * a.w; o.c = op.cout; break;
            case OP_PADCAT: o.c = a.c + s[op.in1].c; break;
            case OP_SIGMOID:
            case OP_LOGSOFTMAX: break;
            case OP_TOSEQ: o = TensorShape{a.w, a.n, 1, a.c, true}; break;
            case OP_GRU: o.c = 2 * op.hidden; break;
            case OP_LINEAR: o.c = op.cout; break;
            default: fail(OCRS_ERR_IO, "bad op type %u", op.type);
        }
        s[op.out] = o;
    }
    TensorShape out = s[out_slot];
    if (slots_out) *slots_out = std::move(s);
    return out;
}

double HipModel::flops(int n, int h, int w) const {
    std::vector<TensorShape> s;
    infer(n, h, w, &s);
    double total = 0;
    for (const GraphOp& op : ops) {
        const TensorShape a = s[op.in0];
        const double px = (double)a.n * a.h * a.w;
        switch (op.type) {
            case OP_CONV: total += 2.0 * px * op.cout * op.cin * op.kh * op.kw; break;
            case OP_DWCONV3: total += 2.0 * px * a.c * 9; break;
            case OP_CONVT2: total += 2.0 * px * op.cin * op.cout * 4; break;
            case OP_GRU: total += 2.0 * 2.0 * px * 3 * op.hidden * (op.cin + op.hidden); break;
            case OP_LINEAR: total += 2.0 * px * op.cin * op.cout; break;
            default: break;
        }
    }
    return total;
}

float* HipModel::run_device(Workspace& ws, const float* d_in, int n, int h, int w, TensorShape* out_shape,
                            StageTimers* timers, const uint8_t* d_excluded, int32_t* d_labels, bool want_logp,
                            bool print_timing, int stop_before, hipStream_t exec) const {
    std::vector<TensorShape> shp;
// ... 380 lines not shown
    for (const PackedGroup& g : groups) geos[0].W.push_back(g.w);
    for (int i = 0; i < ts; i++) {
        Geo o = geos.back();
        if (ops[i].type == OP_MAXPOOL || ops[i].type == OP_AVGPOOL) {
            o.H /= ops[i].kh;
            for (auto& w : o.W) w /= ops[i].kw;
        }
        geos.push_back(std::move(o));
    }
    std::vector<int32_t> nvec;
    for (const PackedGroup& g : groups) nvec.push_back(g.n);
    std::vector<int32_t> meta32;
    std::vector<int64_t> meta64;
    struct GeoOff { size_t w, t128, t256, t32, t16, p, f32[2], f16[2], gap; int nt128, nt256, nt32, nt16, nf32[2], nf16[2], ngap; int64_t pixels; };
    std::vector<GeoOff> goff;
    const size_t n_at = 0;
    meta32.insert(meta32.end(), nvec.begin(), nvec.end());
    const size_t loff_at = meta32.size();
    {
        int32_t acc = 0;
        meta32.push_back(0);
        for (int g = 0; g < G; g++) { acc += nvec[g]; meta32.push_back(acc); }
    }
    for (const Geo& ge : geos) {
        GeoOff o{};
        o.w = meta32.size();
        meta32.insert(meta32.end(), ge.W.begin(), ge.W.end());
        o.t128 = meta32.size();
        int32_t a128 = 0, a256 = 0, a32 = 0, a16 = 0;
        int64_t px = 0;
        std::vector<int32_t> t256{0}, t32{0}, t16{0};
        std::vector<int32_t> f32[2] = {{0}, {0}}, f16[2] = {{0}, {0}};
        int32_t af32[2] = {0, 0}, af16[2] = {0, 0};
        std::vector<int32_t> tgap{0};
        int32_t agap = 0;
        std::vector<int64_t> pv{0};
        meta32.push_back(0);
        for (int g = 0; g < G; g++) {
            const int64_t rows = (int64_t)nvec[g] * ge.H * ge.W[g];
            a128 += (int32_t)((rows + 127) / 128);
            a256 += (int32_t)((rows + 255) / 256);
            a32 += nvec[g] * (ge.H / 4) * ((ge.W[g] + 31) / 32);
            a16 += nvec[g] * (ge.H / 8) * ((ge.W[g] + 15) / 16);
            agap += (int32_t)((ge.H / 8) * (((int64_t)nvec[g] * ((ge.W[g] + 2) & ~1) + 15) / 16));
            tgap.push_back(agap);
            for (int e = 0; e < 2; e++) {
                const int64_t cols = (int64_t)nvec[g] * (e ? (ge.W[g] + 1) & ~1 : ge.W[g]);
                af32[e] += (int32_t)((ge.H / 4) * ((cols + 31) / 32));
                af16[e] += (int32_t)((ge.H / 8) * ((cols + 15) / 16));
                f32[e].push_back(af32[e]);
                f16[e].push_back(af16[e]);
            }
            px += rows;
            meta32.push_back(a128);
            t256.push_back(a256);
            t32.push_back(a32);
            t16.push_back(a16);
            pv.push_back(px);
        }
        o.t256 = meta32.size();
        meta32.insert(meta32.end(), t256.begin(), t256.end());
        o.t32 = meta32.size();
        meta32.insert(meta32.end(), t32.begin(), t32.end());
        o.t16 = meta32.size();
        meta32.insert(meta32.end(), t16.begin(), t16.end());
        o.nt32 = a32; o.nt16 = a16;
        o.gap = meta32.size();
        meta32.insert(meta32.end(), tgap.begin(), tgap.end());
        o.ngap = agap;
        for (int e = 0; e < 2; e++) {
            o.f32[e] = meta32.size();
            meta32.insert(meta32.end(), f32[e].begin(), f32[e].end());
            o.f16[e] = meta32.size();
            meta32.insert(meta32.end(), f16[e].begin(), f16[e].end());
            o.nf32[e] = af32[e]; o.nf16[e] = af16[e];
        }
        o.p = meta64.size();
        meta64.insert(meta64.end(), pv.begin(), pv.end());
        o.nt128 = a128; o.nt256 = a256; o.pixels = px;
        goff.push_back(o);
    }
    int64_t* d64 = ws.alloc_n<int64_t>(meta64.size());
    int32_t* d32 = ws.alloc_n<int32_t>(meta32.size());
    ws.upload(d64, meta64.data(), meta64.size() * sizeof(int64_t));
    ws.upload(d32, meta32.data(), meta32.size() * sizeof(int32_t));
    if (before_launch) before_launch();
    if (exec != ws.s()) {
        hipEvent_t ready = ws.make_event();
        OCRS_HIP(hipEventRecord(ready, ws.s()));
        OCRS_HIP(hipStreamWaitEvent(exec, ready, 0));
    }
    auto view = [&](size_t gi) {
        k::RaggedView v{};
        v.G = G; v.H = geos[gi].H;
        v.W = d32 + goff[gi].w; v.n = d32 + n_at; v.poff = d64 + goff[gi].p;
        v.toff128 = d32 + goff[gi].t128; v.toff256 = d32 + goff[gi].t256; v.loff = d32 + loff_at;
        v.ntiles128 = goff[gi].nt128; v.ntiles256 = goff[gi].nt256; v.pixels = goff[gi].pixels;
        v.max_w = 0;
        for (int32_t w : geos[gi].W) v.max_w = std::max(v.max_w, (int)w);
        const bool use16 = geos[gi].H % 8 == 0 && (geos[gi].H % 4 != 0 || goff[gi].nt16 < goff[gi].nt32);
        v.tw = use16 ? 16 : 32;
        v.toff2d = d32 + (use16 ? goff[gi].t16 : goff[gi].t32);
        v.ntiles2d = use16 ? goff[gi].nt16 : goff[gi].nt32;
        v.toff2d_flat = d32 + (use16 ? goff[gi].f16[0] : goff[gi].f32[0]);
        v.toff2d_flat2 = d32 + (use16 ? goff[gi].f16[1] : goff[gi].f32[1]);
        v.ntiles2d_flat = use16 ? goff[gi].nf16[0] : goff[gi].nf32[0];
        v.ntiles2d_flat2 = use16 ? goff[gi].nf16[1] : goff[gi].nf32[1];
        v.toff2d_gap = d32 + goff[gi].gap;
        v.ntiles2d_gap = geos[gi].H % 8 == 0 ? goff[gi].ngap : 0;
        v.max_tile_px_ = 0;
        v.min_w = INT32_MAX;
        for (int g = 0; g < G; g++) {
            const int64_t w = geos[gi].W[g], span = std::min<int64_t>(nvec[g], (v.tw - 1 + w - 1) / w + 1);
            v.max_tile_px_ = std::max(v.max_tile_px_, span * geos[gi].H * w);
            v.min_w = std::min(v.min_w, (int)w);
        }
        return v;
    };

    int tok = timers ? timers->begin(ST_REC_CONV, st, 0) : -1;
    const float* cur = groups[0].d_batch;
    int curC = 1;
    float* prev_buf = nullptr;
    std::vector<std::pair<float*, size_t>> spare;
    const bool shared_arena = exec != ws.s() || (ws.stream.serial() && before_launch);
    std::vector<char> arena_taken;
    auto get = [&](size_t floats) -> float* {
        const size_t bytes = floats * sizeof(float);
        for (size_t i = 0; i < spare.size(); i++)
            if (spare[i].second >= bytes) { float* p = spare[i].first; spare.erase(spare.begin() + i); return p; }
        if (!shared_arena) return static_cast<float*>(ws.alloc(bytes));
        auto& arena = ctx().heavy_arena;
        arena_taken.resize(arena.size(), 0);
        size_t best = arena.size();
        for (size_t i = 0; i < arena.size(); i++)
            if (!arena_taken[i] && arena[i].bytes >= bytes && (best == arena.size() || arena[i].bytes < arena[best].bytes)) best = i;
        if (best == arena.size()) {
            arena.emplace_back(bytes + bytes / 8);
            arena_taken.push_back(0);
        }
        arena_taken[best] = 1;
        return arena[best].as<float>();
    };
    size_t prev_bytes = 0;
    const int first = range ? range->first : 0, last = range ? range->last : ts;
    auto launches = [&](int i, int j) {
        if (i < first && j >= first)
            fail(OCRS_ERR_INVALID_ARGUMENT, "op range: op %d lies inside the fused launch of ops %d..%d (a range starts at %d)", first, i, j, i);
        if (i <= last && j > last)
            fail(OCRS_ERR_INVALID_ARGUMENT, "op range: op %d lies inside the fused launch of ops %d..%d (a range ends at %d)", last, i, j, j);
        return i >= first;
    };
    int at = ts;
    for (int i = 0; i < ts; i++) {
        const GraphOp& op = ops[i];
        const k::RaggedView vin = view(i);
        float* y = nullptr;
        size_t ybytes = 0;
        bool run = false;
        if (op.type == OP_CONV && op.cin == 1 && i + 3 < ts && ops[i + 2].type == OP_CONV && ops[i + 2].cin == op.cout &&
            ops[i + 2].relu && ops[i + 3].type == OP_MAXPOOL && ops[i + 3].kh == 2 && ops[i + 3].kw == 2) {
            const GraphOp& op2 = ops[i + 2];
            const k::RaggedView vmid = view(i + 2), vout = view(i + 4);
            bool ok = k::conv12_fused_ragged(nullptr, vin, vmid, nullptr, nullptr, op.cout, nullptr, nullptr, op2.cout, nullptr, vout, st);
            if (ok && launches(i, i + 3)) {
                float* y2 = get((size_t)vout.pixels * op2.cout);
                timed(KC_GEMM_CONV3X3, 2.0 * vmid.pixels * 9.0 * op2.cin * op2.cout,
                      4.0 * (vin.pixels + vout.pixels * op2.cout) + 4.0 * op2.wcount[0],
                      [&] { k::conv12_fused_ragged(cur, vin, vmid, op.w[0], op.w[1], op.cout, op2.w[0], op2.w[1], op2.cout, y2, vout, st, op2.wsplit); });
                y = y2;
                ybytes = (size_t)vout.pixels * op2.cout * sizeof(float);
                if (prev_buf) spare.emplace_back(prev_buf, prev_bytes);
                prev_buf = y;
                prev_bytes = ybytes;
                cur = y;
            }
            if (ok) {
                curC = op2.cout;
                i += 3;
                if (i >= last) { at = i; break; }
                continue;
            }
        }
        if (op.type == OP_CONV && op.cin == 1) {
            const k::RaggedView vout = view(i + 2);
            if ((run = launches(i, i + 1))) {
                ybytes = (size_t)vout.pixels * op.cout * sizeof(float);
                y = get((size_t)vout.pixels * op.cout);
                timed(KC_CONV_DIRECT, 2.0 * vin.pixels * 9 * op.cout, 4.0 * vin.pixels + 4.0 * vout.pixels * op.cout,
                      [&] { k::conv1_relu_pool_ragged(cur, vin, op.w[0], op.w[1], op.cout, y, vout, st); });
            }
            curC = op.cout;
            i += 1;
        } else if (op.type == OP_CONV) {
            const bool fuse = i + 1 < ts && ops[i + 1].type == OP_MAXPOOL && ops[i + 1].kh == 2 &&
                              (ops[i + 1].kw == 1 || ops[i + 1].kw == 2) && vin.H % 2 == 0;
            const int ph = fuse ? 2 : 1, pw = fuse ? ops[i + 1].kw : 1;
            const k::RaggedView vout = view(fuse ? i + 2 : i + 1);
            if ((run = launches(i, fuse ? i + 1 : i))) {
                ybytes = (size_t)vout.pixels * op.cout * sizeof(float);
                y = get((size_t)vout.pixels * op.cout);
                bool ok = false;
                timed(KC_GEMM_CONV3X3, 2.0 * vin.pixels * 9.0 * op.cin * op.cout,
                      4.0 * (vin.pixels * op.cin + vout.pixels * op.cout) + 4.0 * op.wcount[0],
                      [&] { ok = k::conv3x3_ragged(cur, vin, op.cin, op.w[0], op.w[1], op.cout, op.relu, ph, pw, y, vout, st, op.wsplit); });
                if (!ok) fail(OCRS_ERR_RUN_FAILED, "model run failed: ragged conv %d->%d at height %d not supported", op.cin, op.cout, vin.H);
            }
            curC = op.cout;
            if (fuse) i += 1;
        } else if (op.type == OP_AVGPOOL && i + 1 == ts && op.kw == 1 && op.kh == vin.H && (curC & 3) == 0) {
            launches(i, ts);
            break;
        } else if ((run = launches(i, i))) {
            const k::RaggedView vout = view(i + 1);
            ybytes = (size_t)vout.pixels * curC * sizeof(float);
            y = get((size_t)vout.pixels * curC);
            timed(KC_POOL, 0, 4.0 * curC * (vin.pixels + vout.pixels),
                  [&] { k::pool_ragged(cur, vin, curC, op.kh, op.kw, op.type == OP_AVGPOOL, y, vout, st); });
        }
        if (run) {
            if (prev_buf) spare.emplace_back(prev_buf, prev_bytes);
            prev_buf = y;
            prev_bytes = ybytes;
            cur = y;
        }
        if (i >= last) { at = i; break; }
    }
    float* X = nullptr;
    if (at < ts) {
        X = ws.alloc_n<float>(prev_bytes / sizeof(float));
        OCRS_HIP(hipMemcpyAsync(X, prev_buf, prev_bytes, hipMemcpyDeviceToDevice, st));
    } else {
        const k::RaggedView vf = view(ts);
        if (vf.H != 1) fail(OCRS_ERR_RUN_FAILED, "model run failed: TOSEQ expects height 1, got %d", vf.H);
        X = ws.alloc_n<float>((size_t)plan.R * curC);
        const bool pool_here = ts >= 1 && ops[ts - 1].type == OP_AVGPOOL && ops[ts - 1].kw == 1 && (curC & 3) == 0 &&
                               ops[ts - 1].kh == view(ts - 1).H;
        if (pool_here) {
            const k::RaggedView vp = view(ts - 1);
            timed(KC_POOL, 0, 4.0 * curC * (vp.pixels + vf.pixels),
                  [&] { k::avgpool_to_seq_ragged(cur, vp, vf, curC, groups[0].d_pos, plan.d_off, X, st); });
        } else {
            launches(ts, ts);
            timed(KC_OTHER, 0, 8.0 * vf.pixels * curC,
                  [&] { k::to_seq_packed_ragged(cur, vf, curC, groups[0].d_pos, plan.d_off, X, st); });
        }
    }
    if (tok >= 0) timers->end(tok, st);
    if (exec != ws.s()) {
        hipEvent_t done = ws.make_event();
        OCRS_HIP(hipEventRecord(done, exec));
        OCRS_HIP(hipStreamWaitEvent(ws.s(), done, 0));
    }
    *feat_c = curC;
    return X;
}

const int32_t* HipModel::make_packed_plan(Workspace& ws, const std::vector<int32_t>& T, PackedPlan* plan,
                                          std::vector<size_t>* order) {
    order->clear();
    for (size_t i = 0; i < T.size(); i++)
        if (T[i] > 0) order->push_back(i);
    std::stable_sort(order->begin(), order->end(), [&](size_t a, size_t b) { return T[a] > T[b]; });
    const int M = (int)order->size();
    if (M == 0) return nullptr;
    plan->M = M;
    plan->Tmax = T[(*order)[0]];
    plan->active.assign(plan->Tmax, 0);
    std::vector<int32_t> hTm(M), hoff(plan->Tmax + 1, 0), hpos(T.size(), 0);
    for (int m = 0; m < M; m++) {
        hTm[m] = T[(*order)[m]];
        hpos[(*order)[m]] = m;
        for (int t = 0; t < hTm[m]; t++) plan->active[t]++;
    }
    for (int t = 0; t < plan->Tmax; t++) hoff[t + 1] = hoff[t] + plan->active[t];
    plan->R = hoff[plan->Tmax];
    std::vector<int32_t> meta(hTm);
    meta.insert(meta.end(), hoff.begin(), hoff.end());
    meta.insert(meta.end(), hpos.begin(), hpos.end());
    int32_t* d_meta = ws.alloc_n<int32_t>(meta.size());
    ws.upload(d_meta, meta.data(), meta.size() * sizeof(int32_t));
    plan->d_Tm = d_meta;
    plan->d_off = d_meta + M;
    plan->h_Tm = std::move(hTm);
    plan->h_off = std::move(hoff);
    return d_meta + M + plan->Tmax + 1;
}

int HipModel::packed_split() const {
    int ts = -1;
    for (size_t i = 0; i < ops.size(); i++)
        if (ops[i].type == OP_TOSEQ) { ts = (int)i; break; }
    if (ts < 0 || (size_t)ts + 3 > ops.size()) return -1;
    int prev_out = ops[ts].out;
    for (size_t i = ts + 1; i < ops.size(); i++) {
        const GraphOp& op = ops[i];
        const bool last = i + 1 == ops.size(), second_last = i + 2 == ops.size();
        if (op.in0 != prev_out) return -1;
        if (last) { if (op.type != OP_LOGSOFTMAX || (uint32_t)op.out != out_slot) return -1; }
        else if (second_last) { if (op.type != OP_LINEAR) return -1; }
        else if (op.type != OP_GRU) return -1;
        prev_out = op.out;
    }
    for (int i = 0; i < ts; i++)
        if (ops[i].type == OP_GRU || ops[i].type == OP_LINEAR || ops[i].type == OP_LOGSOFTMAX || ops[i].type == OP_TOSEQ)
            return -1;
    return ts;
}

int HipModel::run_recognition_packed(Workspace& ws, const std::vector<PackedGroup>& groups, const PackedPlan& plan, int h,
                                     StageTimers* timers, const uint8_t* d_excluded, int32_t* d_labels,
                                     float** d_logp, float* d_maxlp, OpRange* range) const {
    const int ts = packed_split();
    if (ts < 0) fail(OCRS_ERR_RUN_FAILED, "model run failed: graph is not <conv stack> TOSEQ GRU* LINEAR LOGSOFTMAX");
    const int first = range ? range->first : 0, last = range ? range->last : (int)ops.size() - 1;
    hipStream_t st = ws.s();
    auto timed = [&](int cls, double flops, double bytes, auto&& launch) {
        int tok = timers ? timers->kbegin(cls, st, flops, bytes) : -1;
        launch();
        if (tok >= 0) timers->end(tok, st);
    };
    const int64_t R = plan.R;
    const int M = plan.M;

    float* X = nullptr;
    int C0 = 0;
    if (first <= ts) {
        std::unique_lock<std::mutex> heavy(ctx().heavy_phase, std::defer_lock);
        const hipStream_t conv = ws.stream.conv_stream();
        try {
            X = run_prefix_ragged(ws, conv, groups, plan, h, ts, timers, &C0, [&] { heavy.lock(); }, range);
        } catch (...) {
            hipEvent_t e = nullptr;
            if (hipEventCreateWithFlags(&e, hipEventDisableTiming) == hipSuccess) {
                ws.events.push_back(e);
                if (hipEventRecord(e, conv) != hipSuccess || hipStreamWaitEvent(ws.s(), e, 0) != hipSuccess)
                    (void)hipStreamSynchronize(conv);
            } else {
                (void)hipStreamSynchronize(conv);
            }
            throw;
        }
    }
    if (range && first <= ts) {
        if (!X) fail(OCRS_ERR_INVALID_ARGUMENT, "op range: this model's conv stack has no ragged form");
        if (last < ts) {
            range->out = X;
            range->out_c = C0;
            return 0;
        }
    }
    if (!X && first <= ts)
    for (const PackedGroup& g : groups) {
        TensorShape fs;
        float* feat = run_device(ws, g.d_batch, g.n, h, g.w, &fs, timers, nullptr, nullptr, true, false, ts);
        if (fs.h != 1) fail(OCRS_ERR_RUN_FAILED, "model run failed: TOSEQ expects height 1, got %d", fs.h);
        if (!X) {
            C0 = fs.c;
            X = ws.alloc_n<float>((size_t)R * C0);
        }
        int tok = timers ? timers->begin(ST_REC_CONV, st, 0) : -1;
        timed(KC_OTHER, 0, 8.0 * fs.count(), [&] { k::to_seq_packed(feat, g.n, fs.w, fs.c, g.d_pos, plan.d_off, X, st); });
        if (tok >= 0) timers->end(tok, st);
    }
    if (!X && first <= ts) return 0;

    const float* cur = first <= ts ? X : range->seq_in;
    int curC = first <= ts ? C0 : range->in_c;
    int classes = 0;
    int gru_layer = 0;
    float* gx_buf = nullptr;
    size_t gx_cap = 0;
    void* hx_buf = nullptr;
    size_t hx_cap = 0;
    for (int i = std::max(ts + 1, first); i <= last; i++) {
        const GraphOp& op = ops[i];
        if (op.type == OP_GRU) {
            const int H = op.hidden, I = op.cin;
            if (I != curC) fail(OCRS_ERR_RUN_FAILED, "model run failed: GRU input size %d != %d", I, curC);
            int tok = timers ? timers->begin(ST_REC_GRU, st, 0) : -1;
            const size_t gx_floats = (size_t)2 * R * 3 * H;
            if (gx_floats > gx_cap) { gx_buf = ws.alloc_n<float>(gx_floats); gx_cap = gx_floats; }
            float* gx = gx_buf;
            float* y = ws.alloc_n<float>((size_t)R * 2 * H);
            const bool fused = (H == 256 || H == 128 || H == 64);
            const bool persistent = fused && gru_mode() == GRU_PERSISTENT && k::gru_persistent_supported(plan.h_Tm.data(), M, plan.Tmax, R, H);
            const int np = option(OPT_NUMERICS) == 1 ? 3 : option(OPT_NUMERICS) == 2 ? 2 : 0;
            const bool split = persistent && np != 0 && k::gru_split_supported(plan.h_Tm.data(), M, plan.Tmax, R, H, np);
            const size_t hx_bytes = split ? k::gru_split_exchange_bytes(plan.h_Tm.data(), M, H, np) : persistent ? k::gru_persistent_exchange_bytes(plan.h_Tm.data(), M, H) : 0;
            if (hx_bytes > hx_cap) { hx_buf = ws.alloc(hx_bytes); hx_cap = hx_bytes; }
            uint16_t* hx = split ? static_cast<uint16_t*>(hx_buf) : nullptr;
            float* hxf = persistent && !split ? static_cast<float*>(hx_buf) : nullptr;
            if (split) OCRS_HIP(k::gru_split_prepare(hx, plan.h_Tm.data(), M, H, np, st));
            else if (persistent) OCRS_HIP(k::gru_persistent_prepare(hxf, plan.h_Tm.data(), M, H, st));
            k::GemmDesc d{};
            d.A = cur; d.lda = I; d.B = op.aux0; d.ldb = 3 * H; d.bias = op.aux1; d.C = gx; d.ldc = 3 * H;
            d.M = (int)R; d.N = 3 * H; d.K = I; d.batch = 2;
            d.strideA = 0; d.strideB = (int64_t)I * 3 * H; d.strideBias = 3 * H; d.strideC = R * 3 * H;
            d.Bsplit = op.wsplit; d.strideBsplit = (int64_t)(3 * H / 128) * (I / 16) * 3 * 128 * 16;
            const double gx_flops = 2.0 * 2 * R * (double)d.N * d.K, gx_bytes = 4.0 * ((double)R * I + 2.0 * R * d.N + 2.0 * d.K * d.N);
            timed(KC_GEMM_GRU_INPUT, gx_flops, gx_bytes, [&] { k::gemm(d, st); });
            if (range && range->gx_only && i == last) {
                range->out = gx;
                range->out_c = 3 * H;
                return 0;
            }
            bool ran_persistent = false;
            if (persistent) {
                uint32_t* d_sync = ws.alloc_n<uint32_t>(k::gru_persistent_sync_words(M));
                double fl = 0.0;
                for (int step = 0; step < plan.Tmax; step++) fl += 2.0 * 2 * plan.active[step] * 3.0 * H * H;
                {
                    DeviceContext& dc = ctx();
                    std::lock_guard<std::mutex> g(dc.rec_phase);
                    hipStream_t rs = ws.stream.recurrent_stream();
                    hipEvent_t ready = ws.make_event(), done = ws.make_event();
                    OCRS_HIP(hipEventRecord(ready, st));
                    OCRS_HIP(hipStreamWaitEvent(rs, ready, 0));
                    int ktok = timers ? timers->kbegin(KC_GEMM_GRU_HIDDEN, rs, fl, 4.0 * ((double)R * (2.0 * 3 * H + 2.0 * 2 * H) + 2.0 * 3 * H * H)) : -1;
                    ran_persistent = split ? k::gru_persistent_split(gx, op.aux2, op.aux3, y, hx, plan.d_Tm, plan.d_off, plan.h_Tm.data(), R, M, plan.Tmax, H, np, d_sync, rs)
                                           : k::gru_persistent(gx, op.aux2, op.aux3, y, hxf, plan.d_Tm, plan.d_off, plan.h_Tm.data(), R, M, plan.Tmax, H, d_sync, rs);
                    if (ktok >= 0) timers->end(ktok, rs);
                    if (ran_persistent && plan.h_status && gru_layer < 8)
                        ws.download(plan.h_status + gru_layer, d_sync + k::gru_persistent_sync_words(M) - 1, sizeof(uint32_t), rs);
                    OCRS_HIP(hipEventRecord(done, rs));
                    OCRS_HIP(hipStreamWaitEvent(st, done, 0));
                }
            }
            if (ran_persistent) {
            } else if (fused) {
                const int Mcap = (M + 3) & ~3;
                float* hT0 = ws.alloc_n<float>((size_t)2 * H * Mcap);
                float* hT1 = ws.alloc_n<float>((size_t)2 * H * Mcap);
                OCRS_HIP(hipMemsetAsync(hT0, 0, (size_t)2 * H * Mcap * sizeof(float), st));
                for (int step = 0; step < plan.Tmax; step++) {
                    const int act = plan.active[step];
                    if (act <= 0) break;
                    const float* hin = (step & 1) ? hT1 : hT0;
                    float* hout = (step & 1) ? hT0 : hT1;
                    timed(KC_GEMM_GRU_HIDDEN, 2.0 * 2 * act * 3.0 * H * H,
                          4.0 * 2 * ((double)act * H * 2 + (double)act * 3 * H + 3.0 * H * H + (double)act * H), [&] {
                              if (!k::gru_step_fused(gx, op.aux2, op.aux3, hin, hout, y, plan.d_Tm, plan.d_off, R, Mcap, act, H, step, st))
                                  fail(OCRS_ERR_RUN_FAILED, "model run failed: no fused GRU step kernel for hidden size %d", H);
                          });
                }
            } else {
                float* gh = ws.alloc_n<float>((size_t)2 * M * 3 * H);
                float* hs = ws.alloc_n<float>((size_t)2 * M * H);
                OCRS_HIP(hipMemsetAsync(hs, 0, (size_t)2 * M * H * sizeof(float), st));
                k::GemmDesc r{};
                r.A = hs; r.lda = H; r.B = op.aux2; r.ldb = 3 * H; r.bias = op.aux3; r.C = gh; r.ldc = 3 * H;
                r.N = 3 * H; r.K = H; r.batch = 2;
                r.strideA = (int64_t)M * H; r.strideB = (int64_t)H * 3 * H; r.strideBias = 3 * H; r.strideC = (int64_t)M * 3 * H;
                for (int step = 0; step < plan.Tmax; step++) {
                    const int act = plan.active[step];
                    if (act <= 0) break;
                    r.M = act;
                    timed(KC_GEMM_GRU_HIDDEN, 2.0 * 2 * act * (double)r.N * r.K,
                          4.0 * 2 * ((double)act * r.K + (double)act * r.N + (double)r.K * r.N), [&] { k::gemm(r, st); });
                    timed(KC_GRU_GATES, 0, 4.0 * 2 * act * (double)H * 9, [&] {
                        k::gru_gates_packed(gx, gh, hs, y, plan.d_Tm, plan.d_off, R, M, act, H, step, st);
                    });
                }
            }
            if (tok >= 0) timers->end(tok, st);
            gru_layer++;
            cur = y;
            curC = 2 * H;
        } else if (op.type == OP_LINEAR) {
            if (op.cin != curC) fail(OCRS_ERR_RUN_FAILED, "model run failed: Linear input size %d != %d", op.cin, curC);
            int tok = timers ? timers->begin(ST_REC_HEAD, st, 0) : -1;
            float* y = ws.alloc_n<float>((size_t)R * op.cout);
            k::GemmDesc d{};
            d.A = cur; d.lda = op.cin; d.B = op.w[0]; d.ldb = op.cout; d.bias = op.w[1];
            d.C = y; d.ldc = op.cout; d.M = (int)R; d.N = op.cout; d.K = op.cin; d.relu = op.relu;
            timed(KC_GEMM_LINEAR, 2.0 * R * (double)d.N * d.K, 4.0 * ((double)R * (op.cin + op.cout)) + 4.0 * op.wcount[0],
                  [&] { k::gemm(d, st); });
            if (tok >= 0) timers->end(tok, st);
            cur = y;
            curC = op.cout;
        } else {
            int tok = timers ? timers->begin(ST_REC_HEAD, st, 0) : -1;
            float* lp = nullptr;
            if (d_logp || range) {
                lp = ws.alloc_n<float>((size_t)R * curC);
                if (d_logp) *d_logp = lp;
            }
            timed(KC_LOGSOFTMAX_ARGMAX, 0, 4.0 * R * curC * (lp ? 2.0 : 1.0),
                  [&] {
                      if (!k::log_softmax_argmax(cur, R, curC, d_excluded, lp, d_labels, st, d_maxlp))
                          fail(OCRS_ERR_CAPACITY, "LogSoftmax over %d classes exceeds the kernel's LDS staging (max ~630)", curC);
                  });
            if (tok >= 0) timers->end(tok, st);
            classes = curC;
            if (range) cur = lp;
        }
    }
    if (range) {
        range->out = cur;
        range->out_c = curC;
    }
    OCRS_HIP(hipGetLastError());
    return classes;
}

}
```

Before: 271.9.

## Fuse recognition tail: linear+logsoftmax head, conv+pool+seq, sorted crop edges, blocked CTC

Adds a REC_TAIL option bitmask that enables several recognition-tail optimizations. The final linear layer is fused with log-softmax/argmax inside the tiled GEMM epilogue, using weights padded to 128 columns. The last conv3x3 is fused with the maxpool, avgpool and to-sequence packing. Crop_lines sorts polygon edge crossings in LDS and binary-searches them. CTC collapse batches its label loads in blocks of 16. Together these aim to cut kernel launches and intermediate memory traffic. The cost is added code complexity, plus a single wave doing the per-row softmax inside the GEMM block.

```diff
diff --git a/ocrs_amd/csrc/common.cpp b/ocrs_amd/csrc/common.cpp
--- a/ocrs_amd/csrc/common.cpp
+++ b/ocrs_amd/csrc/common.cpp
@@ -416,6 +416,7 @@
     {"conv_flat", "OCRS_CONV_FLAT", 1},
     {"beam_gpu", "OCRS_BEAM_GPU", 1},
     {"det_tile_batch", "OCRS_DET_TILE_BATCH", 16},
+    {"rec_tail", "OCRS_REC_TAIL", REC_TAIL_ALL},
     {"numerics", nullptr, 0},
     {"coalesce", nullptr, 2},
     {"coalesce_pages", nullptr, 16},
@@ -426,7 +427,7 @@
 struct OptRange { long lo, hi; long also[4]; };
 const OptRange kOptRanges[OPT_COUNT] = {
     {0, 1, {}}, {0, 1, {}}, {0, 1, {}}, {0, 2, {}}, {0, 1, {8, 14, 32}}, {0, 1, {8, 14, 20, 32}}, {0, 1, {}}, {0, 1, {}}, {0, 1, {}}, {0, 1, {}},
-    {1, 1024, {}},
+    {1, 1024, {}}, {0, REC_TAIL_ALL, {}},
     {0, 2, {}}, {0, 64, {}}, {1, 4096, {}}, {0, 10000000, {}}, {0, 4096, {}}, {0, INT64_MAX, {}},
 };
 bool in_range(int i, long v) {
diff --git a/ocrs_amd/csrc/common.hpp b/ocrs_amd/csrc/common.hpp
--- a/ocrs_amd/csrc/common.hpp
+++ b/ocrs_amd/csrc/common.hpp
@@ -140,7 +140,7 @@
 inline hipStream_t heavy_stream() { return ctx().heavy_stream(); }
 
 enum Option { OPT_GRU_MODE = 0, OPT_GRU_GATES, OPT_GRU_LOCAL, OPT_DET_FUSE, OPT_DET_STREAM, OPT_DET_ROWS, OPT_CCL_QUAD,
-              OPT_CONV12_FUSE, OPT_CONV_FLAT, OPT_BEAM_GPU, OPT_DET_TILE_BATCH, OPT_PUBLIC_COUNT,
+              OPT_CONV12_FUSE, OPT_CONV_FLAT, OPT_BEAM_GPU, OPT_DET_TILE_BATCH, OPT_REC_TAIL, OPT_PUBLIC_COUNT,
               OPT_NUMERICS = OPT_PUBLIC_COUNT,
               OPT_COALESCE, OPT_COALESCE_PAGES, OPT_COALESCE_WINDOW_US,
               OPT_LAYOUT_THREADS, OPT_REC_MAX_PIXELS,
@@ -162,6 +162,11 @@
 };
 const Tuning* current_tuning();
 enum { GRU_PERSISTENT = 0, GRU_STEP = 1 };
+enum { REC_TAIL_HEAD = 1,
+       REC_TAIL_CROP = 2,
+       REC_TAIL_CTC = 4,
+       REC_TAIL_SEQ = 8,
+       REC_TAIL_ALL = 15 };
 int option(Option o);
 
 inline void allow_dynamic_lds(const void* kernel, std::atomic<uint64_t>& done) {
diff --git a/ocrs_amd/csrc/kernels.hpp b/ocrs_amd/csrc/kernels.hpp
--- a/ocrs_amd/csrc/kernels.hpp
+++ b/ocrs_amd/csrc/kernels.hpp
@@ -64,6 +64,7 @@
     int batch; int64_t strideA, strideB, strideBias, strideC;
     int nfast = 0, nx = 0, ny = 0;
     const uint16_t* Bsplit = nullptr; int64_t strideBsplit = 0;
+    int head_c = 0; const uint8_t* head_excl = nullptr; int32_t* head_labels = nullptr; float* head_maxlp = nullptr; float* head_logp = nullptr;
 };
 void gemm(const GemmDesc& d, hipStream_t s);
 void conv_direct(const float* x, int n, int h, int w, int cin, const float* wt, const float* bias, int kh, int kw,
@@ -115,6 +116,8 @@
 void gru_gates(const float* gx, const float* gh, float* h, float* y, int T, int N, int H, int step, hipStream_t s);
 bool log_softmax_argmax(const float* logits, int64_t rows, int c, const uint8_t* d_excluded ,
                         float* logp, int32_t* labels, hipStream_t s, float* maxlp = nullptr);
+bool linear_log_softmax_argmax(const float* a, int lda, const float* w128, const float* b128, int64_t rows, int k, int c,
+                               const uint8_t* d_excluded, float* logp, int32_t* labels, float* maxlp, hipStream_t s);
 void to_seq_packed(const float* x, int n, int T, int c, const int32_t* d_pos, const int32_t* d_off, float* y,
                    hipStream_t s);
 void gru_gates_packed(const float* gx, const float* gh, float* h, float* y, const int32_t* d_Tm, const int32_t* d_off,
@@ -185,6 +188,8 @@
 void conv12_split_weights(const float* w2_host , std::vector<uint16_t>* out);
 bool conv3x3_ragged(const float* x, const RaggedView& rv, int cin, const float* wt, const float* bias, int cout, int relu,
                     int ph, int pw, float* y, const RaggedView& out, hipStream_t s, const uint16_t* wsplit = nullptr);
+bool conv3x3_pool_avg_seq_ragged(const float* x, const RaggedView& rv, int cin, const float* wt, const float* bias, int cout,
+                                 int relu, const int32_t* d_pos, const int32_t* d_off, float* y, hipStream_t s);
 void split_weights(const float* w_host, int K, int N, int ldw, std::vector<uint16_t>* out);
 
 struct LineDesc {
diff --git a/ocrs_amd/csrc/kernels_lines.hip b/ocrs_amd/csrc/kernels_lines.hip
--- a/ocrs_amd/csrc/kernels_lines.hip
+++ b/ocrs_amd/csrc/kernels_lines.hip
@@ -1,3 +1,4 @@
+#include "common.hpp"
 #include "kernels.hpp"
 
 namespace ocrs {
@@ -22,11 +23,13 @@
     return xa + (int)roundf(t);
 }
 
+template <bool SORTED>
 __global__ void __launch_bounds__(256)
 crop_lines_kernel(const float* const* __restrict__ pages, const int32_t* __restrict__ page_hw,
                   const LineDesc* __restrict__ lines, const int32_t* __restrict__ poly, int out_h,
                   float* __restrict__ batch) {
     __shared__ int xs[2][MAX_LDS_EDGES];
+    __shared__ int xo[SORTED ? 2 : 1][SORTED ? MAX_LDS_EDGES : 1];
     __shared__ int cnt[2];
     const LineDesc ln = lines[blockIdx.y];
     const int oy = blockIdx.x;
@@ -59,6 +62,30 @@
     }
     __syncthreads();
     const int m0 = cnt[0], m1 = cnt[1];
+    if (SORTED) {
+        const int n0 = m0 <= MAX_LDS_EDGES ? m0 : 0, n1 = m1 <= MAX_LDS_EDGES ? m1 : 0;
+        for (int i = threadIdx.x; i < n0 + n1; i += blockDim.x) {
+            const int which = i >= n0 ? 1 : 0, e = i - (which ? n0 : 0);
+            const int m = which ? n1 : n0;
+            const int v = xs[which][e];
+            int rank = 0;
+            for (int j = 0; j < m; j++) {
+                const int u = xs[which][j];
+                rank += (u < v || (u == v && j < e)) ? 1 : 0;
+            }
+            xo[which][rank] = v;
+        }
+        __syncthreads();
+    }
+    auto crossings_sorted = [&](int which, int m, int x) {
+        int lo = 0, hi = m;
+        while (lo < hi) {
+            const int mid = (lo + hi) >> 1;
+            if (xo[which][mid] <= x) lo = mid + 1;
+            else hi = mid;
+        }
+        return lo;
+    };
     auto crossings_direct = [&](int which, int x) {
         const int y = ln.top + (which ? r1 : r0);
         int c = 0;
@@ -80,6 +107,18 @@
             float wx;
             resize_axis(ox, ln.bw, ln.resized_w, c0, c1, wx);
             float tap[4];
+            int cross[4] = {0, 0, 0, 0};
+            if (SORTED) {
+#pragma unroll
+                for (int which = 0; which < 2; which++) {
+                    const int m = which ? m1 : m0;
+                    if (m > MAX_LDS_EDGES) continue;
+                    int a = crossings_sorted(which, m, ln.left + c0);
+                    cross[2 * which] = a;
+                    while (a < m && xo[which][a] <= ln.left + c1) a++;
+                    cross[2 * which + 1] = a;
+                }
+            }
 #pragma unroll
             for (int q = 0; q < 4; q++) {
                 const int which = q >> 1;
@@ -88,9 +127,11 @@
                 const int y = ln.top + r, x = ln.left + c;
                 const int m = which ? m1 : m0;
                 int crossings = 0;
-                if (m <= MAX_LDS_EDGES)
-                    for (int kk = 0; kk < m; kk++) crossings += xs[which][kk] <= x ? 1 : 0;
-                else
+                if (m <= MAX_LDS_EDGES) {
+                    if (SORTED) crossings = cross[q];
+                    else
+                        for (int kk = 0; kk < m; kk++) crossings += xs[which][kk] <= x ? 1 : 0;
+                } else
                     crossings = crossings_direct(which, x);
                 float t = fill;
                 if ((crossings & 1) && y >= 0 && y <= ph - 1 && x >= 0 && x <= pw - 1 && r <= ph - 1 && c <= pw - 1)
@@ -108,8 +149,12 @@
 void crop_lines(const float* const* d_pages, const int32_t* d_page_hw, const LineDesc* d_lines, const int32_t* d_poly,
                 int n_lines, int out_h, float* d_out, hipStream_t s) {
     if (n_lines <= 0) return;
-    hipLaunchKernelGGL(crop_lines_kernel, dim3(out_h, n_lines), dim3(256), 0, s, d_pages, d_page_hw, d_lines, d_poly,
-                       out_h, d_out);
+    if (option(OPT_REC_TAIL) & REC_TAIL_CROP)
+        hipLaunchKernelGGL(crop_lines_kernel<true>, dim3(out_h, n_lines), dim3(256), 0, s, d_pages, d_page_hw, d_lines, d_poly,
+                           out_h, d_out);
+    else
+        hipLaunchKernelGGL(crop_lines_kernel<false>, dim3(out_h, n_lines), dim3(256), 0, s, d_pages, d_page_hw, d_lines, d_poly,
+                           out_h, d_out);
 }
 
 }
diff --git a/ocrs_amd/csrc/kernels_nn.hip b/ocrs_amd/csrc/kernels_nn.hip
--- a/ocrs_amd/csrc/kernels_nn.hip
+++ b/ocrs_amd/csrc/kernels_nn.hip
@@ -167,7 +167,9 @@
     }
 }
 
-template <int BN, bool IM2COL, bool PAIR>
+__device__ __forceinline__ void log_softmax_argmax_row(float* row, int c, const uint8_t* __restrict__ excl, int& best, float& bv);
+
+template <int BN, bool IM2COL, bool PAIR, bool HEAD = false>
 __global__ void __launch_bounds__(256, 4) gemm_tiled_kernel(GemmDesc d) {
     extern __shared__ __attribute__((aligned(16))) float lds[];
     constexpr int NTW = BN / 64;
@@ -349,6 +351,60 @@
         }
     }
 
+    if constexpr (HEAD) {
+        const int c = d.head_c, cp = (c & 1) ? c : c + 1;
+        float* tile = lds;
+        auto stage = [&] {
+#pragma unroll
+            for (int i = 0; i < 2; i++)
+#pragma unroll
+                for (int t = 0; t < NTW; t++) {
+                    const int col = wn * (BN / 2) + t * 32 + l31;
+                    if (col >= c) continue;
+#pragma unroll
+                    for (int r = 0; r < 16; r++)
+                        tile[(i * 32 + (r & 3) + 8 * (r >> 2) + 4 * half) * cp + col] = acc[i][t][r];
+                }
+        };
+        auto walk = [&](int pass) {
+            const int64_t rr = m0 + pass * 64 + lane;
+            if (wave != 0 || rr >= d.M) return;
+            int best;
+            float bv;
+            log_softmax_argmax_row(tile + lane * cp, c, d.head_excl, best, bv);
+            d.head_labels[rr] = best;
+            if (d.head_maxlp) d.head_maxlp[rr] = bv;
+        };
+        const bool want_logp = d.head_logp != nullptr;
+        auto copy_out = [&](int pass) {
+            if (want_logp) {
+                __syncthreads();
+                const int64_t r0 = m0 + pass * 64;
+                const int nrows = (int)min((int64_t)64, (int64_t)d.M - r0);
+                for (int i = tid; i < nrows * c; i += 256) {
+                    const int rr = i / c, cc = i - rr * c;
+                    d.head_logp[r0 * c + i] = tile[rr * cp + cc];
+                }
+            }
+            __syncthreads();
+        };
+        if (__builtin_amdgcn_readfirstlane(wm) == 0) {
+            stage();
+            __syncthreads();
+            walk(0);
+            copy_out(0);
+            __syncthreads();
+            walk(1);
+            copy_out(1);
+        } else {
+            __syncthreads();
+            copy_out(0);
+            stage();
+            __syncthreads();
+            copy_out(1);
+        }
+        return;
+    }
     if (n0 + BN <= d.N && (d.ldc & 3) == 0 && (((uintptr_t)C) & 15) == 0) {
         static_assert(4 * 32 * (BN / 2) <= 2 * TG_BK * TG_LDA + 2 * TG_BK * BN, "staging must fit the operand tiles");
         store_tile_rows<NTW>(acc, lds + wave * (32 * (BN / 2)), lane, d.relu != 0, C + n0 + wn * (BN / 2), m0 + wm * 64, d.M, d.ldc);
@@ -1013,6 +1069,25 @@
 
 constexpr int LSM_ROWS = 64;
 
+__device__ __forceinline__ void log_softmax_argmax_row(float* row, int c, const uint8_t* __restrict__ excl, int& best, float& bv) {
+    float m = row[0];
+    for (int j = 1; j < c; j++) m = row[j] > m ? row[j] : m;
+    float ssum = 0.0f;
+    for (int j = 0; j < c; j++) ssum = ssum + spec_expf(row[j] - m);
+    const float lse = m + spec_logf(ssum);
+    const float ninf = -__builtin_huge_valf();
+    best = 0;
+    bv = row[0] - lse;
+    row[0] = bv;
+    if (excl && excl[0]) bv = ninf;
+    for (int j = 1; j < c; j++) {
+        float v = row[j] - lse;
+        row[j] = v;
+        if (excl && excl[j]) v = ninf;
+        if (v > bv) { bv = v; best = j; }
+    }
+}
+
 __device__ __forceinline__ void log_softmax_argmax_body(const float* __restrict__ logits, int64_t rows, int c,
                                                         const uint8_t* __restrict__ excl, float* __restrict__ logp,
                                                         int32_t* __restrict__ labels, float* __restrict__ maxlp) {
@@ -1026,23 +1101,9 @@
     }
     __syncthreads();
     if ((int)threadIdx.x < nrows) {
-        float* row = tile + threadIdx.x * cp;
-        float m = row[0];
-        for (int j = 1; j < c; j++) m = row[j] > m ? row[j] : m;
-        float ssum = 0.0f;
-        for (int j = 0; j < c; j++) ssum = ssum + spec_expf(row[j] - m);
-        const float lse = m + spec_logf(ssum);
-        const float ninf = -__builtin_huge_valf();
-        int best = 0;
-        float bv = row[0] - lse;
-        row[0] = bv;
-        if (excl && excl[0]) bv = ninf;
-        for (int j = 1; j < c; j++) {
-            float v = row[j] - lse;
-            row[j] = v;
-            if (excl && excl[j]) v = ninf;
-            if (v > bv) { bv = v; best = j; }
-        }
+        int best;
+        float bv;
+        log_softmax_argmax_row(tile + threadIdx.x * cp, c, excl, best, bv);
         if (labels) labels[r0 + threadIdx.x] = best;
         if (maxlp) maxlp[r0 + threadIdx.x] = bv;
     }
@@ -1084,6 +1145,21 @@
     else
         hipLaunchKernelGGL(log_softmax_argmax_kernel, dim3(grid), dim3(LSM_ROWS), lds, s, logits, rows, c, d_excluded, logp,
                            labels);
+    return true;
+}
+
+bool linear_log_softmax_argmax(const float* a, int lda, const float* w128, const float* b128, int64_t rows, int k, int c,
+                               const uint8_t* d_excluded, float* logp, int32_t* labels, float* maxlp, hipStream_t s) {
+    if (c < 1 || c > 128 || k <= 0 || (k % (2 * TG_BK)) != 0 || (lda & 3) != 0 || (((uintptr_t)a) & 15) != 0 ||
+        (((uintptr_t)w128) & 15) != 0 || !labels || rows > INT32_MAX)
+        return false;
+    if (rows <= 0) return true;
+    GemmDesc d{};
+    d.A = a; d.lda = lda; d.B = w128; d.ldb = 128; d.bias = b128; d.M = (int)rows; d.N = 128; d.K = k;
+    d.head_c = c; d.head_excl = d_excluded; d.head_labels = labels; d.head_maxlp = maxlp; d.head_logp = logp;
+    const int cp = (c & 1) ? c : c + 1;
+    const size_t lds = std::max((size_t)(2 * TG_BK * TG_LDA + 2 * TG_BK * 128), (size_t)64 * cp) * sizeof(float);
+    hipLaunchKernelGGL((gemm_tiled_kernel<128, false, true, true>), dim3((unsigned)((rows + TG_BM - 1) / TG_BM)), dim3(256), lds, s, d);
     return true;
 }
 
@@ -1259,35 +1335,72 @@
                        H, step);
 }
 
+constexpr int CTC_U = 16;
+
+template <bool BLOCKED>
 __global__ void __launch_bounds__(64)
 ctc_collapse_packed_kernel(const int32_t* __restrict__ labels, const int32_t* __restrict__ Tm,
                            const int32_t* __restrict__ off, int M, int Tmax, uint32_t* __restrict__ out_labels,
                            uint32_t* __restrict__ out_pos, int32_t* __restrict__ out_count) {
     const int m = blockIdx.x * blockDim.x + threadIdx.x;
-    if (m >= M) return;
-    const int T = Tm[m];
+    if (!BLOCKED) {
+        if (m >= M) return;
+        const int T = Tm[m];
+        int last = 0, cnt = 0;
+        for (int t = 0; t < T; t++) {
+            int l = labels[(int64_t)off[t] + m];
+            if (l == last) continue;
+            last = l;
+            if (l > 0) {
+                out_labels[(int64_t)m * Tmax + cnt] = (uint32_t)l;
+                out_pos[(int64_t)m * Tmax + cnt] = (uint32_t)t;
+                cnt++;
+            }
+        }
+        out_count[m] = cnt;
+        return;
+    }
+    const int T = m < M ? Tm[m] : 0;
+    int Tw = T;
+#pragma unroll
+    for (int d = 32; d >= 1; d >>= 1) Tw = max(Tw, __shfl_xor(Tw, d));
     int last = 0, cnt = 0;
-    for (int t = 0; t < T; t++) {
-        int l = labels[(int64_t)off[t] + m];
-        if (l == last) continue;
-        last = l;
-        if (l > 0) {
-            out_labels[(int64_t)m * Tmax + cnt] = (uint32_t)l;
-            out_pos[(int64_t)m * Tmax + cnt] = (uint32_t)t;
-            cnt++;
-        }
-    }
-    out_count[m] = cnt;
+    const int64_t base = (int64_t)m * Tmax;
+    for (int t0 = 0; t0 < Tw; t0 += CTC_U) {
+        int l[CTC_U];
+#pragma unroll
+        for (int u = 0; u < CTC_U; u++) {
+            const int t = t0 + u;
+            l[u] = 0;
+            if (t < T) l[u] = labels[(int64_t)off[t] + m];
+        }
+#pragma unroll
+        for (int u = 0; u < CTC_U; u++) {
+            const int t = t0 + u;
+            if (t >= T) break;
+            if (l[u] == last) continue;
+            last = l[u];
+            if (l[u] > 0) {
+                out_labels[base + cnt] = (uint32_t)l[u];
+                out_pos[base + cnt] = (uint32_t)t;
+                cnt++;
+            }
+        }
+    }
+    if (m < M) out_count[m] = cnt;
 }
 
 void ctc_collapse_packed(const int32_t* labels, const int32_t* d_Tm, const int32_t* d_off, int M, int Tmax,
                          uint32_t* out_labels, uint32_t* out_pos, int32_t* out_count, hipStream_t s) {
     if (M <= 0) return;
-    hipLaunchKernelGGL(ctc_collapse_packed_kernel, dim3((M + 63) / 64), dim3(64), 0, s, labels, d_Tm, d_off, M, Tmax,
-                       out_labels, out_pos, out_count);
-}
-
-constexpr int CTC_U = 16;
+    if (option(OPT_REC_TAIL) & REC_TAIL_CTC)
+        hipLaunchKernelGGL(ctc_collapse_packed_kernel<true>, dim3((M + 63) / 64), dim3(64), 0, s, labels, d_Tm, d_off, M, Tmax,
+                           out_labels, out_pos, out_count);
+    else
+        hipLaunchKernelGGL(ctc_collapse_packed_kernel<false>, dim3((M + 63) / 64), dim3(64), 0, s, labels, d_Tm, d_off, M, Tmax,
+                           out_labels, out_pos, out_count);
+}
+
 
 __global__ void __launch_bounds__(64)
 ctc_collapse_scored_packed_kernel(const int32_t* __restrict__ labels, const float* __restrict__ maxlp,
diff --git a/ocrs_amd/csrc/kernels_rec.hip b/ocrs_amd/csrc/kernels_rec.hip
--- a/ocrs_amd/csrc/kernels_rec.hip
+++ b/ocrs_amd/csrc/kernels_rec.hip
@@ -219,11 +219,12 @@
 
 constexpr int RG_BM = 128, RG_BK = 16, RG_LDA = RG_BM + 1;
 constexpr int CONV_WAVES = 4;
-template <int BN, int TW, int PH, int PW, bool FLAT, int SPLIT = 0>
+template <int BN, int TW, int PH, int PW, bool SEQ, bool FLAT, int SPLIT = 0>
 __global__ void __launch_bounds__(256, SPLIT == 3 ? 2 : SPLIT == 2 ? 3 : CONV_WAVES)
 conv3x3_ragged_kernel(const float* __restrict__ X, RaggedView rv, int cin, const float* __restrict__ Bw,
                       const float* __restrict__ bias, int cout, int relu, float* __restrict__ Y,
-                      const int64_t* __restrict__ out_poff) {
+                      const int64_t* __restrict__ out_poff, const int32_t* __restrict__ seq_pos,
+                      const int32_t* __restrict__ seq_off) {
     extern __shared__ __attribute__((aligned(16))) float lds[];
     constexpr int NTW = BN / 64;
     constexpr int TH = RG_BM / TW;
@@ -410,8 +411,51 @@
     }
 
     const int Ho = H / PH, Wo = W / PW;
-    float* __restrict__ C = Y + (out_poff[g] + (int64_t)img * Ho * Wo) * cout;
+    float* __restrict__ C = SEQ ? nullptr : Y + (out_poff[g] + (int64_t)img * Ho * Wo) * cout;
     auto act = [&](float v) { return relu ? (v > 0.0f ? v : 0.0f) : v; };
+    if constexpr (SEQ) {
+        static_assert(BN == 128 && TW == 16 && PH == 2 && PW == 1 && FLAT && SPLIT == 0, "the sequence epilogue's one shape");
+        constexpr int HS = 136;
+        static_assert(16 * HS <= 2 * RG_BK * RG_LDA + 2 * RG_BK * BN, "the hand-off must fit the operand tiles");
+        float* hand = lds;
+        auto pooled = [&](int i, int t, int jx) {
+            float m = act(acc[i][t][jx]);
+            const float v = act(acc[i][t][jx + 8]);
+            return v > m ? v : m;
+        };
+        int xrow[8];
+        if (wm == 1) {
+#pragma unroll
+            for (int jx = 0; jx < 8; jx++) {
+                int x = x0 + (jx & 3) + 8 * (jx >> 2) + 4 * half, ir = 0;
+#pragma unroll
+                for (int k = 0; k < 3; k++) { const bool nx = x >= Wp; x -= nx ? Wp : 0; ir += nx; }
+                const bool ok = x < W && ir < span;
+                xrow[jx] = ok ? seq_off[x] + seq_pos[rv.loff[g] + img + ir] : -1;
+            }
+        } else {
+#pragma unroll
+            for (int t = 0; t < NTW; t++)
+#pragma unroll
+                for (int jx = 0; jx < 8; jx++)
+                    hand[((jx & 3) + 8 * (jx >> 2) + 4 * half) * HS + wn * (BN / 2) + t * 32 + l31] = (0.0f + pooled(0, t, jx)) + pooled(1, t, jx);
+        }
+        __syncthreads();
+        if (wm == 1) {
+            const float inv = 1.0f / (float)(H / PH);
+#pragma unroll
+            for (int t = 0; t < NTW; t++) {
+                const int col = n0 + wn * (BN / 2) + t * 32 + l31;
+#pragma unroll
+                for (int jx = 0; jx < 8; jx++) {
+                    if (xrow[jx] < 0) continue;
+                    const float s2 = hand[((jx & 3) + 8 * (jx >> 2) + 4 * half) * HS + wn * (BN / 2) + t * 32 + l31];
+                    Y[(int64_t)xrow[jx] * cout + col] = ((s2 + pooled(0, t, jx)) + pooled(1, t, jx)) * inv;
+                }
+            }
+        }
+        return;
+    }
     if (PH == 1 && PW == 1 && n0 + BN <= cout && (cout & 3) == 0 && (((uintptr_t)Y) & 15) == 0) {
         constexpr int WN = BN / 2, LPR = WN / 4, RPI = 64 / LPR, NIT = 32 / RPI;
         static_assert(SPLIT != 0 || 4 * 32 * WN <= 2 * RG_BK * RG_LDA + 2 * RG_BK * BN, "staging must fit the operand tiles");
@@ -916,6 +960,20 @@
         }
 }
 
+bool conv3x3_pool_avg_seq_ragged(const float* x, const RaggedView& rv, int cin, const float* wt, const float* bias, int cout,
+                                 int relu, const int32_t* d_pos, const int32_t* d_off, float* y, hipStream_t s) {
+    if (option(OPT_REC_TAIL) & REC_TAIL_SEQ) {} else return false;
+    if ((cin % (2 * RG_BK)) != 0 || (cout % 128) != 0 || !relu || rv.tw != 16 || rv.H != 8) return false;
+    if (option(OPT_NUMERICS) != 0) return false;
+    if (!(option(OPT_CONV_FLAT) != 0 && rv.min_w >= 11 && rv.max_tile_px_ * std::max(cin, cout) * (int64_t)sizeof(float) < (int64_t)1 << 30))
+        return false;
+    if (!x || rv.ntiles2d_flat <= 0) return true;
+    const size_t lds = (size_t)(2 * RG_BK * RG_LDA + 2 * RG_BK * 128) * sizeof(float);
+    hipLaunchKernelGGL((conv3x3_ragged_kernel<128, 16, 2, 1, true, true>), dim3(rv.ntiles2d_flat, cout / 128), dim3(256), lds, s, x, rv,
+                       cin, wt, bias, cout, relu, y, nullptr, d_pos, d_off);
+    return true;
+}
+
 bool conv3x3_ragged(const float* x, const RaggedView& rv, int cin, const float* wt, const float* bias, int cout, int relu,
                     int ph, int pw, float* y, const RaggedView& out, hipStream_t s, const uint16_t* wsplit) {
     if ((cin % (2 * RG_BK)) != 0 || (cout % 4) != 0 || cout < 64) return false;
@@ -936,9 +994,9 @@
     const dim3 grid(ntiles, (cout + (n64 ? 63 : 127)) / (n64 ? 64 : 128));
 #define OCRS_LAUNCH_SPLIT(TW_, PH_, PW_, FLAT_, NP_, SLOT_)                                                              \
     if (flat == FLAT_ && (numerics == 2 ? 2 : 3) == NP_) {                                                              \
-        allow_dynamic_lds(reinterpret_cast<const void*>(&conv3x3_ragged_kernel<128, TW_, PH_, PW_, FLAT_, NP_>), ok_[SLOT_]);   \
-        hipLaunchKernelGGL((conv3x3_ragged_kernel<128, TW_, PH_, PW_, FLAT_, NP_>), grid, dim3(256), lds, s, x, rv, cin, ws_, bias, \
-                           cout, relu, y, out.poff);                                                                    \
+        allow_dynamic_lds(reinterpret_cast<const void*>(&conv3x3_ragged_kernel<128, TW_, PH_, PW_, false, FLAT_, NP_>), ok_[SLOT_]);   \
+        hipLaunchKernelGGL((conv3x3_ragged_kernel<128, TW_, PH_, PW_, false, FLAT_, NP_>), grid, dim3(256), lds, s, x, rv, cin, ws_, bias, \
+                           cout, relu, y, out.poff, nullptr, nullptr);                                                  \
     }
 #define OCRS_LAUNCH_CONV(BN_, TW_, PH_, PW_)                                                                            \
     do {                                                                                                                \
@@ -947,10 +1005,10 @@
             static std::atomic<uint64_t> ok_[4] = {};                                                                    \
             OCRS_LAUNCH_SPLIT(TW_, PH_, PW_, true, 3, 0) OCRS_LAUNCH_SPLIT(TW_, PH_, PW_, false, 3, 1)                     \
             OCRS_LAUNCH_SPLIT(TW_, PH_, PW_, true, 2, 2) OCRS_LAUNCH_SPLIT(TW_, PH_, PW_, false, 2, 3)                     \
-        } else if (flat) hipLaunchKernelGGL((conv3x3_ragged_kernel<BN_, TW_, PH_, PW_, true>), grid, dim3(256), lds, s, x, rv, \
-                                     cin, wt, bias, cout, relu, y, out.poff);                                           \
-        else hipLaunchKernelGGL((conv3x3_ragged_kernel<BN_, TW_, PH_, PW_, false>), grid, dim3(256), lds, s, x, rv,     \
-                                cin, wt, bias, cout, relu, y, out.poff);                                                \
+        } else if (flat) hipLaunchKernelGGL((conv3x3_ragged_kernel<BN_, TW_, PH_, PW_, false, true>), grid, dim3(256), lds, s, x, rv, \
+                                     cin, wt, bias, cout, relu, y, out.poff, nullptr, nullptr);                         \
+        else hipLaunchKernelGGL((conv3x3_ragged_kernel<BN_, TW_, PH_, PW_, false, false>), grid, dim3(256), lds, s, x, rv, \
+                                cin, wt, bias, cout, relu, y, out.poff, nullptr, nullptr);                              \
     } while (0)
 #define OCRS_DISPATCH_POOL(BN_, TW_)                              \
     do {                                                          \
diff --git a/ocrs_amd/csrc/model.cpp b/ocrs_amd/csrc/model.cpp
--- a/ocrs_amd/csrc/model.cpp
+++ b/ocrs_amd/csrc/model.cpp
@@ -213,6 +213,22 @@
         m->tapes.emplace_back(both.size() * sizeof(uint16_t));
         OCRS_HIP(hipMemcpy(m->tapes.back().p, both.data(), both.size() * sizeof(uint16_t), hipMemcpyHostToDevice));
         op.wsplit = m->tapes.back().as<uint16_t>();
+    }
+    for (uint32_t i = 0; i + 1 < hd.n_ops; i++) {
+        GraphOp& op = m->ops[i];
+        const GraphOp& nx = m->ops[i + 1];
+        if (m->kind != 1 || op.type != OP_LINEAR || op.relu || op.cout < 1 || op.cout > 128 || (op.cin % 32) != 0 || fops[i].n_w < 2 ||
+            nx.type != OP_LOGSOFTMAX || nx.in0 != op.out || i + 2 != hd.n_ops)
+            continue;
+        std::vector<float> pad((size_t)(op.cin + 1) * 128, 0.0f);
+        const float* w = slab.data() + fops[i].w[0].off;
+        const float* b = slab.data() + fops[i].w[1].off;
+        for (int k = 0; k < op.cin; k++) std::copy(w + (size_t)k * op.cout, w + (size_t)(k + 1) * op.cout, pad.begin() + (size_t)k * 128);
+        std::copy(b, b + op.cout, pad.begin() + (size_t)op.cin * 128);
+        m->tapes.emplace_back(pad.size() * sizeof(float));
+        OCRS_HIP(hipMemcpy(m->tapes.back().p, pad.data(), pad.size() * sizeof(float), hipMemcpyHostToDevice));
+        op.aux0 = m->tapes.back().as<float>();
+        op.aux1 = op.aux0 + (size_t)op.cin * 128;
     }
     for (size_t i = 0; i + 1 < m->ops.size(); i++) {
         GraphOp& a = m->ops[i];
@@ -899,6 +915,7 @@
         return i >= first;
     };
     int at = ts;
+    float* seq_done = nullptr;
     for (int i = 0; i < ts; i++) {
         const GraphOp& op = ops[i];
         const k::RaggedView vin = view(i);
@@ -943,6 +960,16 @@
             const bool fuse = i + 1 < ts && ops[i + 1].type == OP_MAXPOOL && ops[i + 1].kh == 2 &&
                               (ops[i + 1].kw == 1 || ops[i + 1].kw == 2) && vin.H % 2 == 0;
             const int ph = fuse ? 2 : 1, pw = fuse ? ops[i + 1].kw : 1;
+            if (fuse && pw == 1 && i + 3 == ts && ops[i + 2].type == OP_AVGPOOL && ops[i + 2].kw == 1 && ops[i + 2].kh * 2 == vin.H &&
+                (!range || (first <= i && last >= ts)) &&
+                k::conv3x3_pool_avg_seq_ragged(nullptr, vin, op.cin, nullptr, nullptr, op.cout, op.relu, nullptr, nullptr, nullptr, st)) {
+                seq_done = ws.alloc_n<float>((size_t)plan.R * op.cout);
+                timed(KC_GEMM_CONV3X3, 2.0 * vin.pixels * 9.0 * op.cin * op.cout,
+                      4.0 * (vin.pixels * op.cin + (double)plan.R * op.cout) + 4.0 * op.wcount[0],
+                      [&] { k::conv3x3_pool_avg_seq_ragged(cur, vin, op.cin, op.w[0], op.w[1], op.cout, op.relu, groups[0].d_pos, plan.d_off, seq_done, st); });
+                curC = op.cout;
+                break;
+            }
             const k::RaggedView vout = view(fuse ? i + 2 : i + 1);
             if ((run = launches(i, fuse ? i + 1 : i))) {
                 ybytes = (size_t)vout.pixels * op.cout * sizeof(float);
@@ -973,8 +1000,9 @@
         }
         if (i >= last) { at = i; break; }
     }
-    float* X = nullptr;
-    if (at < ts) {
+    float* X = seq_done;
+    if (X) {
+    } else if (at < ts) {
         X = ws.alloc_n<float>(prev_bytes / sizeof(float));
         OCRS_HIP(hipMemcpyAsync(X, prev_buf, prev_bytes, hipMemcpyDeviceToDevice, st));
     } else {
@@ -1217,6 +1245,20 @@
         } else if (op.type == OP_LINEAR) {
             if (op.cin != curC) fail(OCRS_ERR_RUN_FAILED, "model run failed: Linear input size %d != %d", op.cin, curC);
             int tok = timers ? timers->begin(ST_REC_HEAD, st, 0) : -1;
+            if ((option(OPT_REC_TAIL) & REC_TAIL_HEAD) && op.aux0 && i + 1 <= last && ops[i + 1].type == OP_LOGSOFTMAX && d_labels) {
+                float* lp = (d_logp || range) ? ws.alloc_n<float>((size_t)R * op.cout) : nullptr;
+                bool ok = false;
+                timed(KC_GEMM_LINEAR, 2.0 * R * (double)op.cout * op.cin, 4.0 * ((double)R * (op.cin + (lp ? op.cout : 0) + 1)) + 4.0 * op.wcount[0],
+                      [&] { ok = k::linear_log_softmax_argmax(cur, op.cin, op.aux0, op.aux1, R, op.cin, op.cout, d_excluded, lp, d_labels, d_maxlp, st); });
+                if (ok) {
+                    if (tok >= 0) timers->end(tok, st);
+                    if (d_logp) *d_logp = lp;
+                    classes = curC = op.cout;
+                    if (range) cur = lp;
+                    i++;
+                    continue;
+                }
+            }
             float* y = ws.alloc_n<float>((size_t)R * op.cout);
             k::GemmDesc d{};
             d.A = cur; d.lda = op.cin; d.B = op.w[0]; d.ldb = op.cout; d.bias = op.w[1];
```

After: 274.9, median of 5. About the same (+1.1%).
